# sp-uhh/sgmse

Measured on AMD Instinct MI355X. Metric: utterances/sec, SGMSE+ NCSN++ PC N=30 (reverse_diffusion + ALD, 60 NFE), 16 kHz 4 s utterances, higher is better.
Workload: dtype f32 (fp16x2-split products, fp32 accumulate); 1 GPU; BASELINE configs[1]: ncsnpp (65.6M params) PC sampler N=30, batch=32 x 4 s @16 kHz per GPU, hipGraph-captured step; batch_per_gpu=32, F=256, T=512, nfe=60, sampler=pc, parallelism=utterance-sharded x1 (weights broadcast once over RCCL)

## Files before the change

sgmse_amd/csrc/conv_launch.h:

```cpp
#pragma once
#include "conv_route.h"
#include "kernels_conv.h"
#include "kernels_conv_pipe.h"
#include "kernels_conv1x1.h"
#include "kernels_conv_split.h"
#include "kernels_conv_wino.h"
#include "kernels_conv_wino43.h"
#include "kernels_conv_wino2d.h"
#include "kernels_conv_thin.h"

#ifndef SGMSE_CONV_SPLIT_DEFAULT
#define SGMSE_CONV_SPLIT_DEFAULT 2
#endif
#ifndef SGMSE_CONV_PIPE_DEFAULT
#define SGMSE_CONV_PIPE_DEFAULT 1
#endif

namespace sgmse {

inline int conv_variant() {
  static int v = [] { const char* e = getenv("SGMSE_CONV_VARIANT"); return e ? atoi(e) : 0; }();
  return v;
}

inline int conv_grid_tiles(const ConvArgs& a, int rows) {
  const int ty = (a.H + rows - 1) / rows;
  return a.rag_cols ? ty * a.rag_ncols : a.B * ty * ((a.W + 31) / 32);
}

template <int KS, int WC, int FC, int FP>
inline void launch_conv_mfma_t(const ConvArgs& a, drt::stream_t st, int variant, int ksplit = 1) {
  using T = ConvTile<KS, WC, FC, FP>;
  const int tiles = conv_grid_tiles(a, T::ROWS);
  dim3 grid(tiles, (a.Cout + T::CO_T - 1) / T::CO_T, ksplit);
  if (variant < 0) variant = conv_variant();
  const bool vec = (a.rag_w ? a.rag_vec_ok != 0 : a.W % 4 == 0) && !(variant & 2) && (reinterpret_cast<uintptr_t>(a.src1) % 16 == 0) &&
                   (a.src2 == nullptr || reinterpret_cast<uintptr_t>(a.src2) % 16 == 0);
  const bool pref = !(variant & 1);
  if constexpr (FC * FP == 8) {
    const bool pipe = ((variant & 4) != 0) != (SGMSE_CONV_PIPE_DEFAULT != 0);
    if (vec && pipe) { DRT_LAUNCH((conv_mfma_pipe_kernel<KS, WC, FC, FP>), grid, dim3(256), st, a); return; }
  }
  if constexpr (KS == 1 && FC * FP == 8) {
    if (!vec) { launch_conv_mfma_t<KS, WC, FC, FP / 2>(a, st, variant, ksplit); return; }
    if (pref) DRT_LAUNCH((conv_mfma_kernel<KS, WC, FC, FP, 1, 1>), grid, dim3(256), st, a);
    else DRT_LAUNCH((conv_mfma_kernel<KS, WC, FC, FP, 0, 1>), grid, dim3(256), st, a);
  } else {
    if (vec && pref) DRT_LAUNCH((conv_mfma_kernel<KS, WC, FC, FP, 1, 1>), grid, dim3(256), st, a);
    else if (vec) DRT_LAUNCH((conv_mfma_kernel<KS, WC, FC, FP, 0, 1>), grid, dim3(256), st, a);
    else if (pref) DRT_LAUNCH((conv_mfma_kernel<KS, WC, FC, FP, 1, 0>), grid, dim3(256), st, a);
    else DRT_LAUNCH((conv_mfma_kernel<KS, WC, FC, FP, 0, 0>), grid, dim3(256), st, a);
  }
  if constexpr (FC * FP <= 2) {
    if (ksplit > 1) DRT_LAUNCH((conv_splitk_reduce_kernel<KS, WC, FC, FP>), dim3(grid.x, grid.y, 1), dim3(256), st, a, ksplit);
  }
}

inline void launch_conv_mfma(const ConvArgs& a, int ks, const ConvPlan& pl, drt::stream_t st, int variant = -1, int ksplit = 1) {
  const int v = variant < 0 ? conv_variant() : variant;
  if (ks == 1 && pl.co_t == 128 && (v & 8)) {
    const int kc = (v & 16) ? 64 : 32;
    const int Cin = a.C1 + a.C2;
    if (Cin % kc == 0 && (a.src2 == nullptr || a.C1 % kc == 0)) {
      const int tiles = conv_grid_tiles(a, 4);
      dim3 grid(tiles, a.Cout / 128, 1);
      if (kc == 64) DRT_LAUNCH((conv1x1_stream_kernel<1, 64>), grid, dim3(256), st, a);
      else DRT_LAUNCH((conv1x1_stream_kernel<1, 32>), grid, dim3(256), st, a);
      return;
    }
  }
#define SGMSE_CONV_CASE(KS_, CO_, ROWS_, WC_, FC_, FP_) \
  if (ks == KS_ && pl.co_t == CO_ && pl.rows == ROWS_) { launch_conv_mfma_t<KS_, WC_, FC_, FP_>(a, st, variant, ksplit); return; }
  SGMSE_CONV_CASE(3, 128, 8, 2, 2, 4)
  SGMSE_CONV_CASE(3, 64, 8, 2, 1, 4)
  SGMSE_CONV_CASE(3, 32, 8, 1, 1, 2)
  SGMSE_CONV_CASE(3, 128, 4, 2, 2, 2)
  SGMSE_CONV_CASE(3, 64, 4, 2, 1, 2)
  SGMSE_CONV_CASE(3, 32, 4, 1, 1, 1)
  SGMSE_CONV_CASE(1, 128, 8, 2, 2, 4)
  SGMSE_CONV_CASE(1, 64, 8, 2, 1, 4)
  SGMSE_CONV_CASE(1, 32, 8, 1, 1, 2)
  SGMSE_CONV_CASE(1, 128, 4, 2, 2, 2)
  SGMSE_CONV_CASE(1, 64, 4, 2, 1, 2)
  SGMSE_CONV_CASE(1, 32, 4, 1, 1, 1)
#undef SGMSE_CONV_CASE
}

static_assert(ConvThinGeom::KC == kConvThinKC, "conv_thin_eligible (conv_route.h) assumes the thin kernel's stage depth");

template <class S, int SHAPE>
inline void launch_conv3x3_split_t(const ConvArgs& a, dim3 grid, drt::stream_t st) {
  const bool act = a.in_scale && a.in_act;
  if constexpr (SHAPE != 1 && S::SCALED) {
    if (a.sc_w) {
      DRT_LAUNCH((conv3x3_split_kernel<S, SHAPE, 1, 0, 1>), grid, dim3(256), st, a);
      return;
    }
  }
  if (act) DRT_LAUNCH((conv3x3_split_kernel<S, SHAPE, 1>), grid, dim3(256), st, a);
  else DRT_LAUNCH((conv3x3_split_kernel<S, SHAPE, 0>), grid, dim3(256), st, a);
}
#ifndef SGMSE_CONV1X1_RAW_VEC
#define SGMSE_CONV1X1_RAW_VEC 1
#endif
template <class S>
inline void launch_conv1x1_split_t(const ConvArgs& a, dim3 grid, drt::stream_t st) {
  if (a.in_scale) { DRT_LAUNCH((conv1x1_split_kernel<S, 1, 0>), grid, dim3(256), st, a); return; }
  const bool vec = SGMSE_CONV1X1_RAW_VEC && (a.rag_w ? a.rag_vec_ok != 0 : a.W % 4 == 0) && reinterpret_cast<uintptr_t>(a.src1) % 16 == 0 &&
                   (a.src2 == nullptr || reinterpret_cast<uintptr_t>(a.src2) % 16 == 0);
  if (vec) DRT_LAUNCH((conv1x1_split_kernel<S, 0, 1>), grid, dim3(256), st, a);
  else DRT_LAUNCH((conv1x1_split_kernel<S, 0, 0>), grid, dim3(256), st, a);
}
inline void launch_conv_split(const ConvArgs& a, int ks, int mode, drt::stream_t st, bool rows4 = false, int abl = 0, int ksplit = 1) {
  const int tiles = conv_grid_tiles(a, 8);
  if (ks == 3 && a.Cout > 32 && rows4 && a.kchunk_stages > 0 && mode == 2) {
    const dim3 grid(conv_grid_tiles(a, 4), a.Cout / 128, ksplit);
    if (a.in_scale && a.in_act) DRT_LAUNCH((conv3x3_split_kernel<SplitH2, 2, 1, 0, 0, 1>), grid, dim3(256), st, a);
    else DRT_LAUNCH((conv3x3_split_kernel<SplitH2, 2, 0, 0, 0, 1>), grid, dim3(256), st, a);
    if (ksplit > 1) DRT_LAUNCH((conv_splitk_reduce_kernel<3, 4, 1, 4, true>), dim3(grid.x, grid.y, 1), dim3(256), st, a, ksplit);
    return;
  }
  if (ks == 3 && a.Cout > 32 && rows4) {
    const dim3 grid(conv_grid_tiles(a, 4), a.Cout / 128, 1);
    if (mode == 2) launch_conv3x3_split_t<SplitH2, 2>(a, grid, st); else launch_conv3x3_split_t<SplitB3, 2>(a, grid, st);
    return;
  }
  if (ks == 3 && a.Cout <= 32) {
    if (mode == 2) launch_conv3x3_split_t<SplitH2, 1>(a, dim3(tiles, 1, 1), st); else launch_conv3x3_split_t<SplitB3, 1>(a, dim3(tiles, 1, 1), st);
    return;
  }
  if (ks == 1) {
    if (mode == 2) launch_conv1x1_split_t<SplitH2>(a, dim3(tiles, a.Cout / 128, 1), st);
    else launch_conv1x1_split_t<SplitB3>(a, dim3(tiles, a.Cout / 128, 1), st);
    return;
  }
  const dim3 grid(tiles, a.Cout / 128, 1);
  if (abl && mode == 2) {
#define SGMSE_ABL_CASE(V) if (abl == V) { DRT_LAUNCH((conv3x3_split_kernel<SplitH2, 0, 1, V>), grid, dim3(256), st, a); return; }
#ifdef SGMSE_ABLATION_FULL
    SGMSE_ABL_CASE(8) SGMSE_ABL_CASE(59) SGMSE_ABL_CASE(64)
    SGMSE_ABL_CASE(3) SGMSE_ABL_CASE(4) SGMSE_ABL_CASE(24) SGMSE_ABL_CASE(56)
    SGMSE_ABL_CASE(1) SGMSE_ABL_CASE(2) SGMSE_ABL_CASE(67) SGMSE_ABL_CASE(72) SGMSE_ABL_CASE(128) SGMSE_ABL_CASE(256) SGMSE_ABL_CASE(512)
#endif
#undef SGMSE_ABL_CASE
  }
  if (mode == 2) launch_conv3x3_split_t<SplitH2, 0>(a, grid, st); else launch_conv3x3_split_t<SplitB3, 0>(a, grid, st);
}

inline bool conv_wino43_aligned(const ConvArgs& a) {
  return reinterpret_cast<uintptr_t>(a.src1) % 16 == 0 && (a.src2 == nullptr || reinterpret_cast<uintptr_t>(a.src2) % 16 == 0);
}
template <int ROWS>
inline void launch_conv_wino_rows(WinoForm form, const ConvArgs& a, drt::stream_t st) {
  const dim3 grid(conv_grid_tiles(a, ROWS), a.Cout / 128, 1);
  const bool act = a.in_scale && a.in_act;
  if (form == WinoForm::F43) {
    if (act) DRT_LAUNCH((conv3x3_wino43_kernel<ROWS, 1>), grid, dim3(512), st, a);
    else DRT_LAUNCH((conv3x3_wino43_kernel<ROWS, 0>), grid, dim3(512), st, a);
  } else {
    if (a.sc_w) DRT_LAUNCH((conv3x3_wino_kernel<ROWS, 1, 1>), grid, dim3(512), st, a);
    else if (act) DRT_LAUNCH((conv3x3_wino_kernel<ROWS, 1, 0>), grid, dim3(512), st, a);
    else DRT_LAUNCH((conv3x3_wino_kernel<ROWS, 0, 0>), grid, dim3(512), st, a);
  }
}
inline void launch_conv_wino(WinoForm form, const ConvArgs& a, drt::stream_t st, bool rows4, bool trace = false, int abl = 0) {
  if (form == WinoForm::F2x2) {
    const dim3 grid(conv_grid_tiles(a, 4), a.Cout / 128, 1);
    if (abl == 8) DRT_LAUNCH((conv3x3_wino2d_kernel<1, 8>), grid, dim3(512), st, a);
    else if (abl == 16) DRT_LAUNCH((conv3x3_wino2d_kernel<1, 16>), grid, dim3(512), st, a);
    else if (a.in_scale && a.in_act) DRT_LAUNCH((conv3x3_wino2d_kernel<1>), grid, dim3(512), st, a);
    else DRT_LAUNCH((conv3x3_wino2d_kernel<0>), grid, dim3(512), st, a);
    return;
  }
#ifdef SGMSE_ABLATION_FULL
  const dim3 grid8(conv_grid_tiles(a, 8), a.Cout / 128, 1);
  if (form == WinoForm::F43) {
    if (trace) { DRT_LAUNCH((conv3x3_wino43_kernel<8, 1, 1>), grid8, dim3(512), st, a); return; }
  } else {
#define SGMSE_WABL_CASE(V) if (abl == V) { DRT_LAUNCH((conv3x3_wino_kernel<8, 1, 0, 0, V>), grid8, dim3(512), st, a); return; }
    SGMSE_WABL_CASE(1) SGMSE_WABL_CASE(2) SGMSE_WABL_CASE(4) SGMSE_WABL_CASE(8) SGMSE_WABL_CASE(16) SGMSE_WABL_CASE(24) SGMSE_WABL_CASE(3) SGMSE_WABL_CASE(32) SGMSE_WABL_CASE(20)
#undef SGMSE_WABL_CASE
    if (trace) { DRT_LAUNCH((conv3x3_wino_kernel<8, 1, 0, 1>), grid8, dim3(512), st, a); return; }
  }
#endif
  (void)abl; (void)trace;
  if (rows4) launch_conv_wino_rows<4>(form, a, st); else launch_conv_wino_rows<8>(form, a, st);
}

inline void launch_conv_thin(const ConvArgs& a, drt::stream_t st) {
  const dim3 grid(conv_thin_grid_tiles(a, (a.W + ConvThinGeom::TW - 1) / ConvThinGeom::TW), 1, 1);
  if (a.in_scale && a.in_act) DRT_LAUNCH((conv3x3_thin_kernel<1>), grid, dim3(256), st, a);
  else DRT_LAUNCH((conv3x3_thin_kernel<0>), grid, dim3(256), st, a);
}

inline void launch_conv_direct(const ConvArgs& a, int ks, drt::stream_t st) {
  const int HW = a.H * a.W;
  if (a.Cout <= 4) {
    dim3 grid((HW + 255) / 256, 1, a.B);
    if (ks == 3) DRT_LAUNCH((conv_direct_kernel<3, 4>), grid, dim3(256), st, a);
    else DRT_LAUNCH((conv_direct_kernel<1, 4>), grid, dim3(256), st, a);
  } else {
    dim3 grid((HW + 255) / 256, (a.Cout + 15) / 16, a.B);
    if (ks == 3) DRT_LAUNCH((conv_direct_kernel<3, 16>), grid, dim3(256), st, a);
    else DRT_LAUNCH((conv_direct_kernel<1, 16>), grid, dim3(256), st, a);
  }
}

}
```

sgmse_amd/csrc/engine.h:

```cpp
#pragma once
#include <algorithm>
#include <map>
#include <string>
#include <vector>
#include <cstdio>
#include <stdexcept>

#include <deque>
#include <sgmse_devrt.h>
#include "dev_memory.h"
#include "kernels_conv.h"
#include "conv_launch.h"
#include "kernels_norm_fir.h"
#include "kernels_attn_misc.h"
#include "kernels_ode.h"
#include "ode_control.h"
#include "kernels_stft.h"
#include "../../include/sgmse_hip.h"

namespace sgmse {

struct NetCfg {
  int variant = 0;
  int nf = 128;
// ... 661 lines not shown
    frames_next_.insert(frames_next_.end(), total, total + n);
  }
  void take_noise_frames(const std::string& who, int B, int T, const float2* noise) {
    std::vector<int> g;
    g.swap(frames_next_);
    geom_call_.clear();
    if ((int)g.size() != 2 * B) return;
    std::string bad;
    if (noise) bad = who + ": a noise geometry (sgmse_set_noise_frames) applies to in-kernel noise, not to replayed noise";
    for (int b = 0; b < B && bad.empty(); ++b) {
      const int Tb = ragged() ? rag_T_[b] : T;
      const long long first = g[b], total = g[B + b];
      if (first < 0 || first + Tb > total)
        bad = who + ": utterance " + std::to_string(b) + ": noise frames [" + std::to_string(first) + ", " + std::to_string(first + Tb) +
              ") do not lie inside the recording's [0, " + std::to_string(total) + ")";
      geom_call_.insert(geom_call_.end(), {g[b], g[B + b], Tb});
    }
    if (!bad.empty()) { geom_call_.clear(); streams_next_.clear(); throw EngineArgError(bad); }
  }
  void set_ragged_frames(const int* frames, int n) { set_frames(frames, n); }
  int last_nfe() const { return nfe_; }
  int graph_captures() const { return graph_captures_; }
  int graph_updates() const { return graph_updates_; }
  int split_mode() const { return split_mode_; }
  bool winograd() const { return split_mode_ == 2 && wino_; }
  size_t arena_bytes() const { return arena_buf_.capacity(); }

  DevBuf input_bounds(const float* x1, int C1, const float* x2, int C2, int B, int HW) {
    const size_t per = (size_t)B * kAmaxSpread;
    DevBuf buf = fresh(2 * per * 4);
    float* out = buf.as<float>();
    SG_CHECK(drt::memset_dev(out, 0, 2 * per * 4, stream_));
    for (int b = 0; b < B; ++b) {
      const size_t n1 = (size_t)C1 * HW;
      DRT_LAUNCH(absmax_kernel, dim3((unsigned)std::min<size_t>((n1 + 255) / 256, 1024)), dim3(256), stream_, x1 + b * n1, n1,
                 out + (size_t)b * kAmaxSpread);
      if (x2) {
        const size_t n2 = (size_t)C2 * HW;
        DRT_LAUNCH(absmax_kernel, dim3((unsigned)std::min<size_t>((n2 + 255) / 256, 1024)), dim3(256), stream_, x2 + b * n2, n2,
                   out + per + (size_t)b * kAmaxSpread);
      }
    }
    return buf;
  }

  DevBuf producer_bound(const float* in_scale, const float* in_shift, int C, const float* amax1, const float* amax2, int B) {
    DevBuf buf = fresh((size_t)B * kAmaxSpread * 4);
    float* out = buf.as<float>();
    DRT_LAUNCH(xform_bound_kernel, dim3(B), dim3(64), stream_, in_scale, in_shift, C, amax1, amax2, out);
    return buf;
  }

  struct ConvPack { enum Kind { Mfma, Thin, Split, Wino } kind; int smode = 0; WinoForm form = WinoForm::F23; int co_t = 0; };
  struct StandaloneConv { ConvArgs a{}; DevBuf packed, bounds, xbound; };
  StandaloneConv standalone_conv(const ConvArgs& a0, const ConvPack& f, const float* w_oihw, int ks) {
    StandaloneConv s;
    ConvArgs& a = s.a = a0;
    const int Cin = a.C1 + a.C2;
    switch (f.kind) {
      case ConvPack::Mfma: s.packed = pack_mfma(oihw_sources(w_oihw, ks, Cin, a.Cout), f.co_t); break;
      case ConvPack::Thin: s.packed = pack_thin(w_oihw, Cin, a.Cout); break;
      case ConvPack::Split: s.packed = pack_split(w_oihw, ks, Cin, a.Cout, f.smode, &a.co_scale); break;
      case ConvPack::Wino: s.packed = pack_wino(f.form, w_oihw, Cin, a.Cout, &a.co_scale); break;
    }
    a.w = s.packed.as<float>();
    if (f.kind == ConvPack::Wino || (f.kind == ConvPack::Split && f.smode == 2)) {
      s.bounds = input_bounds(a.src1, a.C1, a.src2, a.C2, a.B, a.H * a.W);
      const float* am1 = s.bounds.as<float>();
      const float* am2 = a.src2 ? am1 + (size_t)a.B * kAmaxSpread : nullptr;
      if (ks == 1 && a.in_scale == nullptr) bind_bounds(a, 1, nullptr, am1, am2);
      else {
        s.xbound = producer_bound(a.in_scale, a.in_shift, Cin, am1, am2, a.B);
        bind_bounds(a, ks, s.xbound.as<float>(), s.xbound.as<float>(), nullptr);
      }
    }
    return s;
  }
  static void bind_bounds(ConvArgs& ca, int ks, const float* xbound, const float* amax1, const float* amax2) {
    if (ks == 3) ca.xbound = xbound;
    else { ca.amax1 = amax1; ca.amax2 = amax2; }
  }

  enum ForceConv { FC_AUTO = 0, FC_DIRECT = 1, FC_SPLIT_B3 = 2, FC_SPLIT_H2 = 3, FC_WINO = 4, FC_WINO_4ROW = 5, FC_THIN = 6, FC_WINO2D = 7,
                   FC_WINO43 = 8, FC_WINO43_4ROW = 9 };
  void op_conv2d(const float* x, const float* w_oihw, const float* bias, const float* res, float* out, int B, int Cin,
                 int Cout, int H, int W, int ks, float out_scale, int force_direct, const float* in_scale,
                 const float* in_shift, int in_act, const float* x2, int C2) {
    ConvArgs a{};
    a.src1 = x; a.src2 = x2; a.C1 = Cin - C2; a.C2 = C2; a.bias = bias; a.res = res; a.out_scale = out_scale; a.out = out;
    a.Cout = Cout; a.B = B; a.H = H; a.W = W; a.in_scale = in_scale; a.in_shift = in_shift; a.in_act = in_act;
    ConvPlan pl = choose_conv_plan(ks, Cin, Cout, H, W);
    const bool wino = force_direct == FC_WINO || force_direct == FC_WINO_4ROW || force_direct == FC_WINO2D || force_direct == FC_WINO43 || force_direct == FC_WINO43_4ROW;
    StandaloneConv s;
    if (force_direct == FC_THIN) {
      SG_REQUIRE(conv_thin_eligible(ks, a.C1, C2, Cout), "op_conv2d: shape is not eligible for the thin-output kernel");
      s = standalone_conv(a, ConvPack{ConvPack::Thin}, w_oihw, ks);
      launch_conv_thin(s.a, stream_);
      SG_CHECK(drt::stream_sync(stream_));
    } else if (wino || force_direct == FC_SPLIT_B3 || force_direct == FC_SPLIT_H2) {
      const WinoForm form = force_direct == FC_WINO2D ? WinoForm::F2x2 : force_direct >= FC_WINO43 ? WinoForm::F43 : WinoForm::F23;
      const int smode = wino ? 2 : force_direct - 1;
      if (!wino) SG_REQUIRE(conv_split_eligible(ks, a.C1, C2, Cout) || conv_thin_split_eligible(ks, a.C1, C2, Cout), "op_conv2d: shape is not eligible for the split kernels");
      else if (form == WinoForm::F43) SG_REQUIRE(ks == 3 && conv_wino43_eligible(a.C1, C2, Cout, W) && conv_wino43_aligned(a), "op_conv2d: shape is not eligible for the Winograd F(4,3) kernel");
      else SG_REQUIRE(ks == 3 && conv_wino_eligible(a.C1, C2, Cout, W), form == WinoForm::F2x2 ? "op_conv2d: shape is not eligible for the 2-D Winograd kernel" : "op_conv2d: shape is not eligible for the Winograd kernel");
      s = standalone_conv(a, wino ? ConvPack{ConvPack::Wino, smode, form} : ConvPack{ConvPack::Split, smode}, w_oihw, ks);
      if (wino) launch_conv_wino(form, s.a, stream_, force_direct == FC_WINO_4ROW || force_direct == FC_WINO43_4ROW);
      else launch_conv_split(s.a, ks, smode, stream_);
      SG_CHECK(drt::stream_sync(stream_));
    } else if (pl.mfma && !force_direct && (C2 == 0 || a.C1 % ((ks == 3) ? 8 : 32) == 0)) {
      s = standalone_conv(a, ConvPack{ConvPack::Mfma, 0, WinoForm::F23, pl.co_t}, w_oihw, ks);
      launch_conv_mfma(s.a, ks, pl, stream_);
      SG_CHECK(drt::stream_sync(stream_));
    } else {
      a.w = w_oihw;
      launch_conv_direct(a, ks, stream_);
    }
    check_launch();
  }

  void op_groupnorm(const float* x, const float* gamma, const float* beta, float* out, int B, int C, int H, int W, int act,
                    const float* x2, int C2) {
    const int HW = H * W, C1 = C - C2;
    const DevBuf stats_buf = fresh((size_t)B * C * 2 * 4), sc_buf = fresh((size_t)B * C * 4), sh_buf = fresh((size_t)B * C * 4);
    float *stats = stats_buf.as<float>(), *sc = sc_buf.as<float>(), *sh = sh_buf.as<float>();
    float* stats2 = stats + (size_t)B * C1 * 2;
    DRT_LAUNCH(gn_chan_stats_kernel, dim3(B * C1), dim3(256), stream_, x, (const float*)nullptr, C1, 0, HW, stats, Rag{nullptr, nullptr, nullptr}, 0);
    if (C2) DRT_LAUNCH(gn_chan_stats_kernel, dim3(B * C2), dim3(256), stream_, x2, (const float*)nullptr, C2, 0, HW, stats2, Rag{nullptr, nullptr, nullptr}, 0);
    const int G = std::min(C / 4, 32);
    const GnFin f{stats, stats2, nullptr, nullptr, gamma, beta, sc, sh, nullptr, Rag{nullptr, nullptr, nullptr}, C1, 1, 1, C2, 1, 1, G, HW, 0, 1e-6f};
    DRT_LAUNCH(gn_finalize_kernel, dim3(G, B), dim3(256), stream_, f);
    DRT_LAUNCH(gn_apply_kernel, dim3((HW + 1023) / 1024, B * C), dim3(256), stream_, x, x2, C1, C2, HW, (const float*)sc,
               (const float*)sh, act, out);
    SG_CHECK(drt::stream_sync(stream_));
    check_launch();
  }

  void op_fir(const float* x, float* out, int BC, int H, int W, int up, const float* in_scale, const float* in_shift, int in_act,
              float* out_raw) {
    FirArgs fa{x, out, in_scale, in_shift, in_act, BC, H, W, out_raw, 1, Rag{nullptr, nullptr, nullptr}};
    launch_fir(fa, up);
    check_launch();
  }

  void op_upfirdn2d(int dtype, const void* x, const void* kern, void* out, int BC, int H, int W, int kh, int kw, int up_x, int up_y,
                    int down_x, int down_y, int px0, int px1, int py0, int py1) {
    UpfirdnArgs a{x, kern, out, BC, H, W, kh, kw, up_x, up_y, down_x, down_y, px0, px1, py0, py1, 0, 0};
    a.Ho = (H * up_y + py0 + py1 - kh) / down_y + 1;
    a.Wo = (W * up_x + px0 + px1 - kw) / down_x + 1;
    SG_REQUIRE(a.Ho > 0 && a.Wo > 0, "upfirdn2d: empty output");
    const dim3 grid((a.Ho * a.Wo + 255) / 256, BC);
    if (dtype == 0) DRT_LAUNCH(upfirdn2d_generic_kernel<UpfirdnF32>, grid, dim3(256), stream_, a);
    else if (dtype == 1) DRT_LAUNCH(upfirdn2d_generic_kernel<UpfirdnF64>, grid, dim3(256), stream_, a);
    else DRT_LAUNCH(upfirdn2d_generic_kernel<UpfirdnF16>, grid, dim3(256), stream_, a);
    check_launch();
  }

  void op_attention(const float* qkv, float* out, int B, int C, int S) {
    AttnArgs a{qkv, out, B, C, S, 1.0f / sqrtf((float)C), Rag{nullptr, nullptr, nullptr}, 0};
    SG_REQUIRE(launch_attn_core(a, stream_), "attention: C must be one of " + attn_widths_text());
    check_launch();
  }

  void op_stft(const float* sig, const float* window, float2* spec, int B, int L, int n_fft, int hop) {
    SG_REQUIRE(n_fft <= kMaxNfft && n_fft >= 2 && hop >= 1 && L > n_fft / 2, "stft: unsupported geometry");
    const float2* tw = twiddle(n_fft);
    StftArgs a{sig, window, tw, spec, L, n_fft, hop, n_fft / 2 + 1, (L + 2 * (n_fft / 2) - n_fft) / hop + 1};
    DRT_LAUNCH(stft_kernel, dim3(a.K, B), dim3(256), stream_, a);
    check_launch();
  }

  void op_istft(const float2* spec, const float* window, float* out, int B, int K, int n_fft, int hop, int length) {
    SG_REQUIRE(n_fft <= kMaxNfft && n_fft >= 2 && hop >= 1, "istft: unsupported geometry");
    SG_REQUIRE(K >= 1 && length >= 1 && length + n_fft / 2 <= n_fft + hop * (K - 1), "istft: length exceeds the overlap-add span");
    const float2* tw = twiddle(n_fft);
    IstftArgs a{spec, window, tw, out, n_fft, hop, n_fft / 2 + 1, K, length};
    DRT_LAUNCH(istft_kernel, dim3((length + 255) / 256, B), dim3(256), stream_, a);
    check_launch();
  }

  void op_spec_xform(const float2* in, float2* out, size_t n, int type, float factor, float exponent, int inverse) {
    SpecXformArgs a{in, out, n, type, factor, exponent, inverse};
    DRT_LAUNCH(spec_xform_kernel, dim3((unsigned)((n + 255) / 256)), dim3(256), stream_, a);
    check_launch();
  }

  const int* upload_windows(const int* start, const int* frames, int n) {
    const size_t nb = (size_t)3 * n * sizeof(int);
    grow(win_tab_, nb);
    int* h = reinterpret_cast<int*>(stage_.acquire(nb));
    int col = 0;
    for (int j = 0; j < n; ++j) { h[j] = start[j]; h[n + j] = frames[j]; h[2 * n + j] = col; col += frames[j]; }
    SG_CHECK(drt::memcpy_h2d(win_tab_, h, nb, stream_));
    stage_.commit(stream_);
    return win_tab_.get();
  }

  void op_spec_split(const float2* spec, float2* windows, int F, int K, const int* start, const int* frames, int n, int type, float factor,
                     float exponent) {
    SG_REQUIRE(n <= 65535 && F <= 65535, "spec_split: more than 65535 windows or rows");
    SpecWinArgs a{spec, windows, upload_windows(start, frames, n), F, K, n, type, factor, exponent};
    const int tmax = *std::max_element(frames, frames + n);
    DRT_LAUNCH(spec_split_kernel, dim3((tmax + 255) / 256, F, n), dim3(256), stream_, a);
    check_launch();
  }

  void op_spec_merge(const float2* windows, float2* spec, int F, int K, const int* start, const int* frames, int n, int type, float factor,
                     float exponent) {
    SG_REQUIRE(F <= 65535, "spec_merge: more than 65535 rows");
    SpecWinArgs a{windows, spec, upload_windows(start, frames, n), F, K, n, type, factor, exponent};
    DRT_LAUNCH(spec_merge_kernel, dim3((K + 255) / 256, F), dim3(256), stream_, a);
    check_launch();
  }

  void sync() { SG_CHECK(drt::stream_sync(stream_)); }

  float bench_conv(int ks, int B, int Cin, int Cout, int H, int W, int variant, int iters, int fused) {
    ConvPlan pl = choose_conv_plan(ks, Cin, Cout, H, W);
    SG_REQUIRE(pl.mfma, "bench_conv: shape is not MFMA-eligible");
    if (variant >= 0 && (variant & 512)) { pl.rows = 4; variant &= ~512; }
    int ablate = 0, abl_split = 0;
    bool split_rows4 = false, wino43 = false;
    if (variant >= 0) {
      split_rows4 = (variant >> 23) & 1;
      wino43 = (variant >> 22) & 1;
      abl_split = (variant >> 12) & 1023;
      if (!(variant & (64 | 128))) { ablate = abl_split & 15; abl_split = 0; }
      variant &= 4095;
    }
    const bool wino = variant >= 0 && (variant & 1024);
    const bool wino2d = variant >= 0 && (variant & 2048) && !wino;
    const int smode = variant < 0 ? 0 : ((variant & 128) ? 2 : ((variant & 64) ? 1 : 0));
    const bool b3 = smode != 0 && !wino && !wino2d;
    SG_REQUIRE(!(wino || wino2d) || (ks == 3 && conv_wino_eligible(Cin, 0, Cout, W)), "bench_conv: shape is not eligible for the Winograd kernel");
    SG_REQUIRE(!b3 || conv_split_eligible(ks, Cin, 0, Cout), "bench_conv: shape is not eligible for the split kernels");
    wino43 = wino43 && wino;
    SG_REQUIRE(!wino43 || conv_wino43_eligible(Cin, 0, Cout, W), "bench_conv: shape is not eligible for the Winograd F(4,3) kernel");
    const WinoForm wform = wino2d ? WinoForm::F2x2 : wino43 ? WinoForm::F43 : WinoForm::F23;
    const size_t nx = (size_t)B * Cin * H * W, no = (size_t)B * Cout * H * W, nw = (size_t)Cout * Cin * ks * ks;
    const DevBuf x_buf = fresh(nx * 4), o_buf = fresh(no * 4), r_buf = fresh(no * 4), w_buf = fresh(nw * 4), sc_buf = fresh((size_t)B * Cin * 8);
    float *x = x_buf.as<float>(), *o = o_buf.as<float>(), *r = r_buf.as<float>(), *w = w_buf.as<float>(), *sc = sc_buf.as<float>();
    auto fill = [&](float* d, size_t n, uint32_t seed) {
      DRT_LAUNCH(fill_random_kernel, dim3((unsigned)((n + 255) / 256)), dim3(256), stream_, d, n, seed);
    };
    fill(x, nx, 1); fill(r, no, 2); fill(w, nw, 3); fill(sc, (size_t)B * Cin * 2, 4);
    ConvArgs a0{};
    a0.src1 = x; a0.C1 = Cin; a0.out = o; a0.Cout = Cout; a0.B = B; a0.H = H; a0.W = W; a0.out_scale = 1.f;
    a0.ablate = ablate;
    if (fused) { a0.in_scale = sc; a0.in_shift = sc + (size_t)B * Cin; a0.in_act = 1; a0.res = r; a0.bias = w; a0.out_scale = 0.70710678f; }
    if (b3 && smode == 2 && ks == 1) { a0.in_scale = nullptr; a0.in_shift = nullptr; a0.in_act = 0; }
    EventTimer timer;
    StandaloneConv s = standalone_conv(a0, b3 ? ConvPack{ConvPack::Split, smode} : (wino || wino2d) ? ConvPack{ConvPack::Wino, 2, wform}
                                                                               : ConvPack{ConvPack::Mfma, 0, WinoForm::F23, pl.co_t}, w, ks);
    ConvArgs& a = s.a;
    DevBuf trace_buf;
    unsigned long long* trace_dev = nullptr;
    const size_t n_wg = (size_t)B * ((H + 7) / 8) * ((W + 31) / 32) * ((Cout + 127) / 128);
    if (abl_split & 64) {
      trace_buf = fresh(n_wg * 256);
      trace_dev = trace_buf.as<unsigned long long>();
      SG_CHECK(drt::memset_dev(trace_dev, 0, n_wg * 256, stream_));
      a.trace = trace_dev;
    }
    auto go = [&]() {
      if (wino || wino2d) launch_conv_wino(wform, a, stream_, split_rows4, (abl_split & 64) != 0, abl_split & 63);
      else if (b3) launch_conv_split(a, ks, smode, stream_, split_rows4, abl_split);
      else launch_conv_mfma(a, ks, pl, stream_, variant);
    };
    for (int i = 0; i < 2; ++i) go();
    timer.start(stream_);
    for (int i = 0; i < iters; ++i) go();
    const float ms = timer.stop_ms(stream_) / (float)iters;
    check_launch();
    if (trace_dev) {
      const size_t words = wino ? 32 : 16;
      std::vector<unsigned long long> h(n_wg * words);
      SG_CHECK(drt::memcpy_d2h(h.data(), trace_dev, n_wg * words * 8, stream_));
      SG_CHECK(drt::stream_sync(stream_));
      if (const char* path = getenv("SGMSE_TRACE_OUT")) { if (FILE* f = fopen(path, "wb")) { fwrite(h.data(), 8, h.size(), f); fclose(f); } }
    }
    return ms;
  }

  float calib_stream(int mode, int bytes_per_lane, size_t total_bytes) {
    SG_REQUIRE((bytes_per_lane == 8 || bytes_per_lane == 16) && (mode == 0 || mode == 1) && total_bytes >= 4096, "calib_stream: bad arguments");
    const DevBuf scratch = fresh(total_bytes + 256);
    float* buf = scratch.as<float>();
    SG_CHECK(drt::memset_dev(buf, 0, total_bytes + 256, stream_));
    const size_t nvec = total_bytes / (size_t)bytes_per_lane;
    EventTimer timer;
    timer.start(stream_);
    const dim3 g(256 * 16), b(256);
    float* sink = buf + total_bytes / 4;
    if (bytes_per_lane == 8) { if (mode) DRT_LAUNCH((calib_stream_kernel<2, 1>), g, b, stream_, buf, nvec, sink); else DRT_LAUNCH((calib_stream_kernel<2, 0>), g, b, stream_, buf, nvec, sink); }
    else { if (mode) DRT_LAUNCH((calib_stream_kernel<4, 1>), g, b, stream_, buf, nvec, sink); else DRT_LAUNCH((calib_stream_kernel<4, 0>), g, b, stream_, buf, nvec, sink); }
    const float ms = timer.stop_ms(stream_);
    check_launch();
    return ms;
  }

  enum { TC_CONV3_BIG = 0, TC_CONV3, TC_CONV1, TC_DIRECT, TC_GN, TC_FIR, TC_ATTN, TC_MISC, TC_COUNT };
  void profile_forward(const float2* xy, const float* t_dev, float2* out, int B, int F, int T, float* ms_out, double* work_out,
                       int* launches_out) {
    prof_ = true;
    for (int i = 0; i < TC_COUNT; ++i) { prof_ms_[i] = 0.f; prof_flops_[i] = 0.0; prof_n_[i] = 0; }
    prof_used_ = 0;
    forward_xy(xy, t_dev, out, B, F, T);
    prof_ = false;
    SG_CHECK(drt::stream_sync(stream_));
    for (size_t i = 0; i < prof_used_; ++i) {
      ProfRec& r = prof_recs_[i];
      if (r.cls < 0) continue;
      const float ms = drt::event_elapsed_ms(*r.a.get(), *r.b.get());
      prof_ms_[r.cls] += ms;
      prof_flops_[r.cls] += r.work;
      prof_n_[r.cls] += r.launches;
      if (prof_dump_ && r.note[0]) fprintf(stderr, "[sgmse-prof] %s %.4f ms %.1f Gwork/s\n", r.note, ms, r.work / ms * 1e-6);
    }
    for (int i = 0; i < TC_COUNT; ++i) { ms_out[i] = prof_ms_[i]; work_out[i] = prof_flops_[i]; launches_out[i] = prof_n_[i]; }
  }

 private:
  bool grow(DevBuf& b, size_t bytes) { return b.ensure(bytes, stream_, poison_); }
  void renew(DevBuf& b, size_t bytes) { b.renew(bytes, stream_, poison_); }
  DevBuf fresh(size_t bytes) { DevBuf b; grow(b, bytes); return b; }
  template <class T = float> T* keep(DevBuf b) { wset_.push_back(std::move(b)); return wset_.back().as<T>(); }
  void release_weights() {
    if (wset_.empty()) return;
    drt::stream_sync(stream_);
    wset_.clear();
  }
// ... 333 lines not shown
    SG_REQUIRE(tmax == T, "ragged batch: T must be the largest frame count");
    rag_.clear();
    for (int l = 0; l < L; ++l) {
      const int H = F >> l;
      std::vector<int> w(B), cols(B + 1, 0);
      std::vector<long long> off(B + 1, 0), soff(B + 1, 0);
      for (int b = 0; b < B; ++b) {
        w[b] = rag_T_[b] >> l;
        off[b + 1] = off[b] + (long long)H * w[b];
        soff[b + 1] = soff[b] + (long long)H * ((w[b] + 31) / 32);
        cols[b + 1] = cols[b] + (w[b] + 31) / 32;
      }
      RagLevel r;
      r.pix = (size_t)off[B]; r.ncols = cols[B];
      grow(r.w, (size_t)B * 4); grow(r.off, (size_t)(B + 1) * 8); grow(r.soff, (size_t)(B + 1) * 8); grow(r.cols, (size_t)(B + 1) * 4);
      SG_CHECK(drt::memcpy_h2d(r.w, w.data(), (size_t)B * 4, stream_));
      SG_CHECK(drt::memcpy_h2d(r.off, off.data(), (size_t)(B + 1) * 8, stream_));
      SG_CHECK(drt::memcpy_h2d(r.soff, soff.data(), (size_t)(B + 1) * 8, stream_));
      SG_CHECK(drt::memcpy_h2d(r.cols, cols.data(), (size_t)(B + 1) * 4, stream_));
      SG_CHECK(drt::stream_sync(stream_));
      rag_.push_back(std::move(r));
    }
    rag_built_ = true;
  }
  std::vector<int> rag_T_;
  struct RagLevel { DevArray<int> w; DevArray<long long> off, soff; DevArray<int> cols; size_t pix = 0; int ncols = 0; };
  std::vector<RagLevel> rag_;
  bool rag_built_ = false;
  int cur_F_ = 0;
  void drop(Tensor& t) { arena_.release(t.p); t.p = nullptr; if (t.st) { arena_.release(t.st); t.st = nullptr; } }

  void gn_coeffs(const Tensor& a, const Tensor* b, const float* gamma, const float* beta, float** sc, float** sh,
                 const float** bound = nullptr) {
    const int C = a.C + (b ? b->C : 0), HW = a.H * a.W;
    float* bslot = bound ? next_amax() : nullptr;
    if (bound) *bound = bslot;
    const float* st[2] = {a.st, b ? b->st : nullptr};
    int nsub[2] = {a.nsub, b ? b->nsub : 0};
    int srows[2] = {a.srows, b ? b->srows : 1};
    float* tmp[2] = {nullptr, nullptr};
    const Tensor* src[2] = {&a, b};
    for (int k = 0; k < 2; ++k) {
      if (!src[k] || st[k]) continue;
      tmp[k] = arena_.alloc((size_t)B_ * src[k]->C * 2);
      st[k] = tmp[k]; nsub[k] = 1; srows[k] = 1;
      if (!dry_) {
        tock();
        DRT_LAUNCH(gn_chan_stats_kernel, dim3(B_ * src[k]->C), dim3(256), stream_, (const float*)src[k]->p, (const float*)nullptr,
                   src[k]->C, 0, HW, tmp[k], rag_of(a.H), a.H);
        if (noting()) snprintf(prof_note_, sizeof prof_note_, "gn_chan_stats C=%d @%dx%dx%d", src[k]->C, B_, a.H, a.W);
        tick(TC_GN, 4.0 * B_ * (double)src[k]->C * HW, 1);
      }
    }
    *sc = arena_.alloc((size_t)B_ * C);
    *sh = arena_.alloc((size_t)B_ * C);
    if (!dry_) {
      tock();
      const int G = std::min(C / 4, 32);
      const GnFin f{st[0], st[1], a.amax, b ? b->amax : nullptr, gamma, beta, *sc, *sh, bslot, rag_of(a.H),
                    a.C, nsub[0], srows[0], b ? b->C : 0, nsub[1], srows[1], G, HW, a.H, 1e-6f};
      DRT_LAUNCH(gn_finalize_kernel, dim3(G, B_), dim3(256), stream_, f);
      if (noting()) snprintf(prof_note_, sizeof prof_note_, "gn_finalize C=%d nsub=%d @%dx%dx%d", C, nsub[0], B_, a.H, a.W);
      tick(TC_GN, 8.0 * B_ * ((double)a.C * nsub[0] + (b ? (double)b->C * nsub[1] : 0.0)), 1);
    }
    for (int k = 0; k < 2; ++k) if (tmp[k]) arena_.release(tmp[k]);
  }

  struct Shortcut { const ConvW* w; const Tensor* a; const Tensor* b; };
  bool shortcut_foldable(const ConvW& c2, const Tensor& a, const Tensor* b) const {
    return fold_shortcut_ && c2.packed_split && c2.split_mode == 2 && c2.ks == 1 && conv_split_eligible(1, a.C, b ? b->C : 0, c2.cout) &&
           a.amax && (!b || b->amax);
  }

  ConvRoute route_of(const ConvW& w, int C1, int C2, int H, int W, const ConvCall& call) const {
    const ConvLayer layer{w.ks, C1, C2, w.cout, w.co_t, w.packed != nullptr, w.packed32 != nullptr, w.packed_thin != nullptr,
                          w.packed_split != nullptr, w.packed_wino != nullptr, w.split_mode, w.wino_form};
    const ConvKnobs knobs{tile_min_blocks_, split_min_tiles_, wino_min_tiles_, wino_, fuse_gn_stats_, chunk_max_tiles_, coarse_splitk_div_,
                          coarse_chunked_, coarse_split_};
    return conv_route(layer, ConvLevel{H, W, dec_W(H), level_of(H)}, call, B_, knobs);
  }

  Tensor conv(const ConvW& w, const Tensor& a, const Tensor* b, const Xform& xf, const float* bias, const float* bias2,
              const float* res, float out_scale, const FwdCtl& ctl, bool emit_stats = false, const Shortcut* sc = nullptr) {
    const int C2 = b ? b->C : 0, Cin = a.C + C2;
    SG_REQUIRE(Cin == w.cin, "conv: channel mismatch");
    Tensor o = new_tensor(w.cout, a.H, a.W);
    const ConvRoute rt = route_of(w, a.C, C2, a.H, a.W, ConvCall{xf.bound != nullptr, a.amax && (!b || b->amax), xf.scale != nullptr, emit_stats,
                                                                 bias2 != nullptr, sc != nullptr});
    const ConvFamily fam = rt.family;
    SG_REQUIRE(fam != ConvFamily::Wino23 || (a.W % 2 == 0 && rag_all_mult(a.H, 2)), "conv: odd width on a Winograd level");
    SG_REQUIRE(fam != ConvFamily::Wino43 || (a.W % 4 == 0 && rag_all_mult(a.H, 4)), "conv: width not a multiple of 4 on a Winograd F(4,3) level");
    SG_REQUIRE(!sc || (rt.accepts_shortcut && xf.act && !res), "conv: shortcut fold on an ineligible launch");
    float* partial = rt.ksplit > 1 ? arena_.alloc((size_t)rt.ksplit * w.cout * pix_total(a.H, a.W)) : nullptr;
    if (emit_stats && fuse_gn_stats_ && fam != ConvFamily::Direct) {
      o.srows = rt.srows;
      SG_REQUIRE(o.srows == 1 || !ragged() || a.H % 4 == 0, "ragged batch: 4-row statistics sub-tiles need H % 4 == 0");
      o.nsub = conv_plan_nsub(a.H, a.W, o.srows);
      o.st = arena_.alloc((size_t)B_ * w.cout * o.nsub * 2);
    } else if (emit_stats && fuse_gn_stats_) {
      o.nsub = 1;
      o.st = arena_.alloc((size_t)B_ * w.cout * 2);
    }
    o.amax = next_amax();
    if (dry_) { if (partial) arena_.release(partial); return o; }
    ConvArgs ca{};
    ca.xcd_map = conv_xcd_map_ ? 1 : 0;
    ca.stats_out = o.st; ca.stats_nsub = o.nsub; ca.stats_rows = o.srows;
    ca.amax_out = o.amax;
    ca.src1 = a.p; ca.src2 = b ? b->p : nullptr; ca.C1 = a.C; ca.C2 = C2;
    ca.bias = bias; ca.bias2 = bias2; ca.bias2_bstride = ctl.bias_bstride; ca.bias2_sstride = ctl.bias_sstride;
    ca.step_ptr = bias2 ? ctl.bias_step : nullptr;
    ca.in_scale = xf.scale; ca.in_shift = xf.shift; ca.in_act = xf.act;
    ca.res = res; ca.out_scale = out_scale; ca.out = o.p; ca.Cout = w.cout; ca.B = B_; ca.H = a.H; ca.W = a.W;
    ca.kchunk_stages = rt.kchunk; ca.partial = partial;
    if (ragged()) {
      const Rag rg = rag_of(a.H);
      ca.rag_w = rg.w; ca.rag_off = rg.off; ca.rag_soff = rg.soff; ca.rag_slab = (long long)w.cout * (long long)pix_total(a.H, a.W);
      ca.rag_vec_ok = rag_all_mult(a.H, 4) ? 1 : 0;
      if (rag_prefix_) { const RagLevel& r = rag_.at(level_of(a.H)); ca.rag_cols = r.cols; ca.rag_ncols = r.ncols; }
    }
    double fl = 2.0 * B_ * (double)w.cout * Cin * w.ks * w.ks * a.H * a.W;
    if (sc) {
      const int Cs = sc->a->C + (sc->b ? sc->b->C : 0);
      SG_REQUIRE(Cs == sc->w->cin && sc->w->cout == w.cout && sc->a->H == a.H && sc->a->W == a.W, "conv: shortcut shape mismatch");
      ca.sc_src1 = sc->a->p; ca.sc_src2 = sc->b ? sc->b->p : nullptr; ca.sc_C1 = sc->a->C; ca.sc_C2 = sc->b ? sc->b->C : 0;
      ca.sc_w = sc->w->packed_split; ca.sc_scale = sc->w->split_scale; ca.sc_bias = sc->w->bias;
      ca.sc_amax1 = sc->a->amax; ca.sc_amax2 = sc->b ? sc->b->amax : nullptr;
      fl += 2.0 * B_ * (double)w.cout * Cs * a.H * a.W;
    }
    tock();
    const char* gn = xf.scale ? " +gn" : "";
    const char* rs = res ? " +res" : "";
    const char* ex = ca.rag_cols ? " existing-tiles" : "";
    auto note_split = [&](const char* name) {
      if (!noting()) return;
      char scn[24] = "";
      if (sc) snprintf(scn, sizeof scn, " +shortcut(%d)", ca.sc_C1 + ca.sc_C2);
      snprintf(prof_note_, sizeof prof_note_, "conv3x3-%s %d->%d @%dx%dx%d%s%s%s%s", name, Cin, w.cout, B_, a.H, a.W, rs, gn, scn, ex);
    };
    int cls = w.ks == 3 ? (w.cout >= 128 ? TC_CONV3_BIG : TC_CONV3) : TC_CONV1;
    switch (fam) {
      case ConvFamily::Thin:
        ca.w = w.packed_thin; ca.stats_out = nullptr;
        launch_conv_thin(ca, stream_);
        if (noting()) snprintf(prof_note_, sizeof prof_note_, "conv3x3-thin %d->%d @%dx%dx%d%s%s", Cin, w.cout, B_, a.H, a.W, rs, gn);
        cls = TC_CONV3;
        break;
      case ConvFamily::Wino43:
        SG_REQUIRE(conv_wino43_aligned(ca), "conv: unaligned source on a Winograd F(4,3) level");
        [[fallthrough]];
      case ConvFamily::Wino23:
        ca.w = w.packed_wino; ca.co_scale = w.wino_scale;
        bind_bounds(ca, w.ks, xf.bound, a.amax, b ? b->amax : nullptr);
        launch_conv_wino(w.wino_form, ca, stream_, rt.rows4);
        note_split(fam == ConvFamily::Wino43 ? "wino43" : "wino");
        break;
      case ConvFamily::Split:
      case ConvFamily::SplitCoarse:
        ca.w = w.packed_split; ca.co_scale = w.split_scale;
        if (w.split_mode == 2) bind_bounds(ca, w.ks, xf.bound, a.amax, b ? b->amax : nullptr);
        launch_conv_split(ca, w.ks, w.split_mode, stream_, rt.rows4, 0, rt.ksplit);
        note_split("split");
        break;
      case ConvFamily::Mfma:
        ca.w = (rt.co_t == w.co_t) ? w.packed : w.packed32;
        launch_conv_mfma(ca, w.ks, ConvPlan{rt.co_t, rt.rows, true}, stream_, -1, rt.ksplit);
        if (noting())
          snprintf(prof_note_, sizeof prof_note_, "conv%dx%d %d->%d @%dx%dx%d tile %dco x %drows%s%s%s%s", w.ks, w.ks, Cin, w.cout, B_, a.H, a.W,
                   rt.co_t, rt.rows, rs, gn, rt.ksplit > 1 ? " split-K" : "", ex);
        cls = w.ks == 3 ? ((split_mode_ == 0 && rt.co_t == 128 && rt.rows == 8) ? TC_CONV3_BIG : TC_CONV3) : TC_CONV1;
        break;
      case ConvFamily::Direct:
        ca.w = w.oihw; ca.stats_out = nullptr;
        launch_conv_direct(ca, w.ks, stream_);
        if (noting()) snprintf(prof_note_, sizeof prof_note_, "conv-direct%dx%d %d->%d @%dx%dx%d", w.ks, w.ks, Cin, w.cout, B_, a.H, a.W);
        cls = TC_DIRECT;
        break;
    }
    tick(cls, fl);
    if (partial) arena_.release(partial);
    if (fam == ConvFamily::Direct && o.st) {
      tock();
      DRT_LAUNCH(gn_chan_stats_kernel, dim3(B_ * w.cout), dim3(256), stream_, (const float*)o.p, (const float*)nullptr, w.cout, 0,
                 a.H * a.W, o.st, rag_of(a.H), a.H);
      if (noting()) snprintf(prof_note_, sizeof prof_note_, "gn_chan_stats(direct) C=%d @%dx%dx%d", w.cout, B_, a.H, a.W);
      tick(TC_GN, 4.0 * B_ * (double)w.cout * a.H * a.W, 1);
    }
    return o;
  }

  void launch_fir(const FirArgs& fa, bool up, bool by_level = false) {
    const int H = fa.H, W = fa.W, BC = fa.BC;
// ... 99 lines not shown
    Tensor out = conv(w.proj, o, nullptr, Xform{}, w.proj.bias, nullptr, x.p, 0.70710678118654752440f, ctl, true);
    drop(o);
    return out;
  }

  bool side_enabled() const { return side_stream_on_ && B_ <= side_max_batch_; }
  bool side_active() const { return side_enabled() && !prof_ && !dry_ && !drt::is_emulator(); }
  drt::event_t* side_event() {
    if (side_ev_next_ == side_ev_.size()) side_ev_.emplace_back(Event::Order);
    return side_ev_[side_ev_next_++].get();
  }
  void side_begin() {
    SG_REQUIRE(!side_open_, "side stream: nested section");
    side_open_ = true;
    if (!side_enabled()) return;
    if (!side_pending_) arena_.defer_begin();
    if (!side_active()) return;
    if (!side_stream_ready_) { SG_CHECK(drt::stream_create(&side_stream_)); side_stream_ready_ = true; }
    drt::event_t* e = side_event();
    SG_CHECK(drt::event_record(e, stream_));
    SG_CHECK(drt::stream_wait_event(side_stream_, e));
    std::swap(stream_, side_stream_);
    side_swapped_ = true;
  }
  void side_end() {
    SG_REQUIRE(side_open_, "side stream: end without begin");
    side_open_ = false;
    if (!side_enabled()) return;
    side_pending_ = true;
    if (!side_swapped_) return;
    drt::event_t* e = side_event();
    SG_CHECK(drt::event_record(e, stream_));
    std::swap(stream_, side_stream_);
    side_swapped_ = false;
    side_join_ev_ = e;
  }
  void side_join() {
    if (!side_pending_) return;
    side_pending_ = false;
    if (side_join_ev_) { SG_CHECK(drt::stream_wait_event(stream_, side_join_ev_)); side_join_ev_ = nullptr; }
    arena_.defer_end();
  }
  drt::stream_t side_stream_{}; bool side_stream_ready_ = false, side_open_ = false, side_pending_ = false, side_swapped_ = false;
  std::deque<Event> side_ev_; size_t side_ev_next_ = 0; drt::event_t* side_join_ev_ = nullptr;
  bool side_stream_on_ = true; int side_max_batch_ = 8;

  void run_forward(const float2* x, long long xbs, const float2* y, long long ybs, float2* out, int B, int F, int T,
                   const FwdCtl& ctl_in) {
    side_ev_next_ = 0; side_open_ = side_pending_ = false; side_join_ev_ = nullptr;
    try { run_forward_main(x, xbs, y, ybs, out, B, F, T, ctl_in); }
    catch (...) {
      if (side_swapped_) { std::swap(stream_, side_stream_); side_swapped_ = false; }
      side_open_ = side_pending_ = false; side_join_ev_ = nullptr;
      arena_.reset();
      throw;
    }
  }
  void run_forward_main(const float2* x, long long xbs, const float2* y, long long ybs, float2* out, int B, int F, int T,
                        const FwdCtl& ctl_in) {
    FwdCtl ctl = ctl_in;
    ctl.bias_step = ctl.step_ptr;
    if (!dry_ && ctl.step_ptr && ctl.bias_table && ctl.bias_bstride == 0 && tot_temb_ > 0) {
      DRT_LAUNCH(bias_select_kernel, dim3((tot_temb_ + 255) / 256), dim3(256), stream_, ctl.bias_table, ctl.bias_sstride, ctl.step_ptr,
                 bias_cur_.get(), tot_temb_);
      ctl.bias_table = bias_cur_; ctl.bias_sstride = 0; ctl.bias_step = nullptr;
    }
    B_ = B;
    cur_F_ = F;
    amax_next_ = 0;
    lds_poison_count_ = 0;
    if (!dry_ && poison_ && arena_buf_.capacity()) SG_CHECK(drt::memset_dev(arena_buf_.as<char>(), 0xFF, arena_buf_.capacity(), stream_));
    if (!dry_ && amax_pool_) {
      const int n = amax_slots_ * B * kAmaxSpread;
      DRT_LAUNCH(zero_floats_kernel, dim3((n + 255) / 256), dim3(256), stream_, amax_pool_.get(), n);
    }
    const NetCfg& c = cfg_;
    const int L = c.n_levels;
    size_t mi = 3;
    auto next = [&]() -> const Mod& { SG_REQUIRE(mi < layout_.size(), "layout exhausted"); return layout_[mi++]; };
    const int FT = F * T;
    std::vector<Tensor> hs;
    Tensor xr = new_tensor(4, F, T);
    const bool entry8 = entry_mfma_ && entry8_.packed && layout_[mi].idx == entry8_idx_;
    Tensor xr8{};
    if (entry8) xr8 = new_tensor(entry8_.cin, F, T);
    if (!dry_) { tock(); const WrapCoef wc{ctl.coef, ctl.coef_bstride, ctl.coef_sstride, ctl.step_ptr, ctl.sign};
      DRT_LAUNCH(entry_kernel, dim3((FT + 255) / 256, B), dim3(256), stream_, x, xbs, y, ybs, xr.p, entry8 ? xr8.p : (float*)nullptr,
                 entry8 ? entry8_.cin : 0, FT, wc, rag_of(F), F, ctl.y_plane);
      tick(TC_MISC, (32.0 + (entry8 ? 4.0 * entry8_.cin : 0.0)) * B * FT); }
    {
      const Mod& m = next();
      const ConvW& w = entry8 ? entry8_ : conv_.at(m.idx);
      hs.push_back(conv(w, entry8 ? xr8 : xr, nullptr, Xform{}, w.bias, nullptr, nullptr, 1.f, ctl, true));
      if (entry8) drop(xr8);
    }
    Tensor pyr_in = xr;
    bool pyr_in_is_xr = true;
    for (int l = 0; l < L; ++l) {
      for (int rb = 0; rb < c.num_res_blocks; ++rb) {
        const Mod& m = next();
        Tensor h = res_block(m, hs.back(), nullptr, ctl);
        SG_REQUIRE(cfg_has_attn(c, h.H) == cfg_has_attn(c, c.image_size >> l),
                   "input height does not match the image_size the network was built for (attention placement, ncsnpp.py:308)");
        if (cfg_has_attn(c, h.H)) {
          const Mod& ma = next();
          Tensor h2 = attn_block(ma, h, ctl);
          drop(h);
          h = h2;
        }
        hs.push_back(h);
      }
      if (l != L - 1) {
        const Mod& m = next();
        Tensor h = res_block(m, hs.back(), nullptr, ctl);
        if (c.progressive_input == 1) {
          const Mod& mc = next();
          Tensor np = fir(pyr_in, false, Xform{});
          if (!pyr_in_is_xr) drop(pyr_in);
          pyr_in = np; pyr_in_is_xr = false;
          const ConvW& w = conv_.at(mc.idx);
          Tensor h2 = conv(w, pyr_in, nullptr, Xform{}, w.bias, nullptr, h.p, 1.f, ctl, true);
          drop(h);
          h = h2;
        }
        hs.push_back(h);
      }
    }
    if (!pyr_in_is_xr) drop(pyr_in);
    drop(xr);

    Tensor h = hs.back();
    {
      const Mod& m1 = next(); Tensor a = res_block(m1, h, nullptr, ctl);
      const Mod& m2 = next(); Tensor b2 = attn_block(m2, a, ctl); drop(a);
      const Mod& m3 = next(); h = res_block(m3, b2, nullptr, ctl); drop(b2);
    }
    Tensor pyramid; bool have_pyr = false;
    for (int l = L - 1; l >= 0; --l) {
      for (int rb = 0; rb < c.num_res_blocks + 1; ++rb) {
        const Mod& m = next();
        Tensor skip = hs.back(); hs.pop_back();
        Tensor o = res_block(m, h, &skip, ctl);
        drop(h); drop(skip);
        h = o;
      }
      SG_REQUIRE(cfg_has_attn(c, h.H) == cfg_has_attn(c, c.image_size >> l),
                 "input height does not match the image_size the network was built for (attention placement, ncsnpp.py:354)");
      if (cfg_has_attn(c, h.H)) {
        const Mod& ma = next();
        Tensor h2 = attn_block(ma, h, ctl);
        drop(h); h = h2;
      }
      if (c.progressive == 1) {
        const Mod& mg = next(); const Mod& mc = next();
        side_begin();
        float *sc, *sh;
        const float* bd;
        gn_coeffs(h, nullptr, gn_.at(mg.idx).first, gn_.at(mg.idx).second, &sc, &sh, &bd);
        const ConvW& w = conv_.at(mc.idx);
        Tensor up; bool have_up = false;
        if (have_pyr) { up = fir(pyramid, true, Xform{}); have_up = true; drop(pyramid); }
        pyramid = conv(w, h, nullptr, Xform{sc, sh, 1, bd}, w.bias, nullptr, have_up ? up.p : nullptr, 1.f, ctl);
        have_pyr = true;
        if (have_up) drop(up);
        arena_.release(sc); arena_.release(sh);
        side_end();
      }
      if (l != 0) {
        const Mod& m = next();
        Tensor o = res_block(m, h, nullptr, ctl);
        side_join();
        drop(h); h = o;
      }
    }
    side_join();
    SG_REQUIRE(hs.empty(), "skip stack not empty");
    Tensor h4;
// ... 12 lines not shown
    if (!dry_) {
      ExitArgs ea{h4.p, Wp("output_layer.weight"), Wp("output_layer.bias"), ctl.tvals, ctl.t_bstride, ctl.t_sstride, ctl.step_ptr,
                  c.variant == 1 ? 1 : 0, c.scale_by_sigma,
                  WrapCoef{ctl.coef, ctl.coef_bstride, ctl.coef_sstride, ctl.step_ptr, ctl.sign}, x, xbs, out, FT, rag_of(F), F};
      tock();
      DRT_LAUNCH(exit_kernel, dim3((FT + 255) / 256, B), dim3(256), stream_, ea);
      tick(TC_MISC, 24.0 * B * FT);
      check_launch();
    }
    drop(h4);
  }

  struct HostStage {
    PinnedArray<char> buf_; Event ev_; bool pending_ = false;
    char* acquire(size_t n) {
      if (pending_) { SG_CHECK(drt::event_sync(ev_.get())); pending_ = false; }
      buf_.ensure(std::max(n, size_t(1) << 16));
      return buf_;
    }
    void commit(drt::stream_t stream) {
      ev_.create();
      SG_CHECK(drt::event_record(ev_.get(), stream));
      pending_ = true;
    }
  } stage_;
  const unsigned long long* upload_tables(const std::vector<float>& tab, const std::vector<float>& tv, const std::vector<float>& cf,
                                          unsigned long long seed, int B) {
    SG_REQUIRE(B + 1 <= kMaxStreams, "batch too large for the noise-stream table");
    grow(seed_dev_, (size_t)kMaxStreams * (8 + 12) + 8);
    const size_t nb_geom = geom_call_.empty() ? 0 : ((size_t)3 * B * 4 + 7) / 8 * 8;
    const size_t nb_seed = ((size_t)B + 2) * 8 + nb_geom, nb_tab = tab.size() * 4, nb_tv = tv.size() * 4, nb_cf = cf.size() * 4;
    char* q = stage_.acquire(nb_seed + nb_tab + nb_tv + nb_cf);
    unsigned long long* hs = reinterpret_cast<unsigned long long*>(q);
    hs[0] = seed;
    const bool given = (int)streams_next_.size() == B;
    for (int b = 0; b < B; ++b) hs[1 + b] = given ? streams_next_[b] : (unsigned long long)b;
    streams_next_.clear();
    hs[1 + B] = nb_geom ? 1ull : 0ull;
    if (nb_geom) { hs[1 + B + nb_geom / 8] = 0; memcpy(hs + 2 + B, geom_call_.data(), (size_t)3 * B * 4); }
    geom_call_.clear();
    q += nb_seed;
    memcpy(q, tab.data(), nb_tab); memcpy(q + nb_tab, tv.data(), nb_tv);
    if (nb_cf) memcpy(q + nb_tab + nb_tv, cf.data(), nb_cf);
    SG_CHECK(drt::memcpy_h2d(seed_dev_, hs, nb_seed, stream_));
    SG_CHECK(drt::memcpy_h2d(step_table_, q, nb_tab, stream_));
    SG_CHECK(drt::memcpy_h2d(tsteps_, q + nb_tab, nb_tv, stream_));
    if (nb_cf) SG_CHECK(drt::memcpy_h2d(coef_table_, q + nb_tab + nb_tv, nb_cf, stream_));
    stage_.commit(stream_);
    return seed_dev_.get();
  }
  static constexpr int kMaxStreams = 4096;
  std::vector<unsigned long long> streams_next_;
  std::vector<int> frames_next_;
  std::vector<int> geom_call_;
  DevArray<unsigned long long> seed_dev_;
  DevArray<int> win_tab_;
  int graph_captures_ = 0;

  int device_;
  drt::stream_t stream_;
  NetCfg cfg_;
  std::vector<Mod> layout_;
  std::map<std::string, const float*> W_;
  std::map<int, ResW> res_;
  std::map<int, AttnW> attn_;
  std::map<int, ConvW> conv_;
  std::map<int, std::pair<const float*, const float*>> gn_;
  DenseDesc* dense_descs_ = nullptr; int n_dense_ = 0; int tot_temb_ = 0;
  bool weights_ready_ = false;
  std::vector<DevBuf> wset_;
  std::map<int, DevArray<float2>> twiddles_;

  Arena arena_; DevBuf arena_buf_;
  bool dry_ = false;
  void read_knobs() {
    auto flag = [](const char* name, bool dflt) { const char* e = getenv(name); return e ? e[0] == '1' : dflt; };
    const char* e = getenv("SGMSE_CONV_SPLIT");
    split_mode_ = e ? atoi(e) : SGMSE_CONV_SPLIT_DEFAULT;
    SG_REQUIRE(split_mode_ >= 0 && split_mode_ <= 2, "SGMSE_CONV_SPLIT must be 0, 1 or 2");
    wino_ = flag("SGMSE_WINO", true);
    wino43_ = flag("SGMSE_WINO43", true);
    rag_prefix_ = flag("SGMSE_RAGGED_PREFIX", true);
    conv_xcd_map_ = flag("SGMSE_CONV_XCD_MAP", true);
    debug_sync_ = flag("SGMSE_DEBUG_SYNC", false);
    prof_dump_ = flag("SGMSE_PROFILE_DUMP", false);
    e = getenv("SGMSE_TILE_MIN_BLOCKS");
    tile_min_blocks_ = e ? atol(e) : 512L;
    e = getenv("SGMSE_SPLIT_MIN_TILES");
    split_min_tiles_ = e ? atol(e) : 8L;
    e = getenv("SGMSE_WINO_MIN_TILES");
    wino_min_tiles_ = e ? atol(e) : 32L;
    fuse_gn_stats_ = flag("SGMSE_FUSE_GN_STATS", true);
    lds_poison_ = flag("SGMSE_POISON_LDS", false);
    e = getenv("SGMSE_POISON_LDS_AT");
    lds_poison_at_ = e ? atoi(e) : -1;
    lds_poison_upto_ = flag("SGMSE_POISON_LDS_UPTO", false);
    side_stream_on_ = flag("SGMSE_SIDE_STREAM", true);
    e = getenv("SGMSE_SIDE_MAX_BATCH");
    side_max_batch_ = e ? atoi(e) : 8;
    e = getenv("SGMSE_NOFOLD_LEVELS");
    nofold_levels_ = e ? atoi(e) : 0;
    poison_ = flag("SGMSE_POISON", false);
  }
  DevArray<float> amax_pool_; int amax_slots_ = 0, amax_next_ = 0;
  float* next_amax() {
    const int i = amax_next_++;
    if (dry_) return reinterpret_cast<float*>(uintptr_t(1) << 43) + (size_t)i * kAmaxSpread;
    SG_REQUIRE(amax_pool_ && i < amax_slots_, "range-bound pool smaller than the forward needs");
    return amax_pool_ + (size_t)i * B_ * kAmaxSpread;
  }
  long tile_min_blocks_ = 512, split_min_tiles_ = 8;
  static constexpr bool coarse_chunked_ = true, fold_shortcut_ = true, coarse_split_ = true, entry_mfma_ = true;
  ConvW entry8_{}; int entry8_idx_ = -1;
  bool poison_ = false, debug_sync_ = false, conv_xcd_map_ = true, rag_prefix_ = true, wino_ = true, wino43_ = true;
  long wino_min_tiles_ = 32;
  int nofold_levels_ = 0;
  bool lds_poison_ = false, lds_poison_upto_ = false; int lds_poison_at_ = -1, lds_poison_count_ = 0; DevArray<unsigned> lds_sink_;
  static constexpr long coarse_splitk_div_ = 4, chunk_max_tiles_ = 8;
  int split_mode_ = SGMSE_CONV_SPLIT_DEFAULT;
  bool prof_dump_ = false;
  char prof_note_[160] = {0};
  static constexpr bool fir_scalar_ = false;
  bool fuse_gn_stats_ = true;
  int B_ = 0, shape_B_ = 0, shape_F_ = 0, shape_T_ = 0;
  DevArray<float2> sx_, sxm_, sscore_, sy_;
  DevArray<int> step_ctr_;
  DevArray<float> lang_partial_, lang_scal_;
  DevArray<float> bias_cur_, temb_act_, bias_table_, step_table_, tsteps_, coef_table_; int temb_rows_ = 0;
  drt::graph_t graph_{}; bool graph_valid_ = false; GraphKey graph_key_{};
  int nfe_ = 0;
  DevArray<float2> ode_k_[7], ode_xs_;
  static constexpr int kOdeEachMaxB = 1024;
  DevArray<double> ode_table_, ode_partial_, ode_result_; PinnedArray<double> ode_host_;
  std::vector<OdeControl> ode_ctl_; int ode_rounds_ = 0, ode_wasted_ = 0;
  bool prof_ = false; std::vector<ProfRec> prof_recs_; size_t prof_used_ = 0; float prof_ms_[TC_COUNT]; double prof_flops_[TC_COUNT]; int prof_n_[TC_COUNT];
};

}
```

sgmse_amd/csrc/kernels_attn_misc.h:

```cpp
#pragma once
#include <string>
#include <sgmse_devrt.h>
#include "kernels_conv.h"
#include "kernels_norm_fir.h"

namespace sgmse {

struct AttnArgs { const float* qkv; float* out; int B, C, S; float scale; Rag rag; int H; };

template <int CF>
__global__ __launch_bounds__(256, 2) void attn_core_kernel(AttnArgs p) {
  constexpr int C = CF * 32;
  constexpr int FH = CF < 2 ? CF : 2;
  constexpr int NH = CF / FH;
  constexpr int VS = 33;
  __shared__ float s_q[C * 32];
  __shared__ float s_v[4][FH * 32 * VS];
  __shared__ float s_m[4][32];
  __shared__ float s_l[4][32];
  __shared__ float s_lt[32];
  const int tid = threadIdx.x, wave = tid >> 6, lane = tid & 63, l31 = lane & 31, kh = lane >> 5;
  const int b = blockIdx.y, s0 = blockIdx.x * 32;
  const int S = p.rag.w ? p.H * p.rag.w[b] : p.S;
  if (s0 >= S) return;
// ... 146 lines not shown
  return false;
}

inline std::string attn_widths_text() {
  std::string s;
#define SGMSE_ATTN_TXT(CF) s += (s.empty() ? "" : ", ") + std::to_string((CF) * 32);
  SGMSE_ATTN_WIDTHS(SGMSE_ATTN_TXT)
#undef SGMSE_ATTN_TXT
  return s;
}

inline bool launch_attn_core(const AttnArgs& a, drt::stream_t st) {
  dim3 grid((a.S + 31) / 32, a.B, 1);
  switch (a.C) {
#define SGMSE_ATTN_CASE(CF) case (CF) * 32: DRT_LAUNCH((attn_core_kernel<CF>), grid, dim3(256), st, a); return true;
    SGMSE_ATTN_WIDTHS(SGMSE_ATTN_CASE)
#undef SGMSE_ATTN_CASE
    default: return false;
  }
}

struct TembArgs {
  const float* t; int nt;
  const float* Wf; const float* w1; const float* b1; const float* w2; const float* b2;
  int nf;
  float* act_out;
};

__global__ __launch_bounds__(256) void temb_mlp_kernel(TembArgs p) {
  __shared__ float s_emb[512];
  __shared__ float s_h[1024];
  const int row = blockIdx.x, nf = p.nf, ne = 2 * nf, nh = 4 * nf;
  const float logt = (float)log((double)p.t[row]);
  for (int i = threadIdx.x; i < nf; i += 256) {
    float pr = logt * p.Wf[i];
    pr = pr * 2.0f;
    pr = pr * 3.14159265358979323846f;
    s_emb[i] = (float)sin((double)pr);
    s_emb[nf + i] = (float)cos((double)pr);
  }
  __syncthreads();
  for (int o = threadIdx.x; o < nh; o += 256) {
    float acc = 0.f;
    const float* wr = p.w1 + (size_t)o * ne;
    for (int i = 0; i < ne; ++i) acc = fmaf(wr[i], s_emb[i], acc);
    s_h[o] = silu_precise_f(acc + p.b1[o]);
  }
  __syncthreads();
  for (int o = threadIdx.x; o < nh; o += 256) {
    float acc = 0.f;
    const float* wr = p.w2 + (size_t)o * nh;
    for (int i = 0; i < nh; ++i) acc = fmaf(wr[i], s_h[i], acc);
    p.act_out[(size_t)row * nh + o] = silu_precise_f(acc + p.b2[o]);
  }
}

struct DenseDesc { const float* W; const float* b; const float* cb; int cout; int off; };

__global__ __launch_bounds__(256) void temb_dense_kernel(const DenseDesc* descs, const float* act, int nh, float* table,
                                                         int row_stride) {
  __shared__ float s_a[1024];
  const DenseDesc d = descs[blockIdx.x];
  const int row = blockIdx.y;
  for (int i = threadIdx.x; i < nh; i += 256) s_a[i] = act[(size_t)row * nh + i];
  __syncthreads();
  for (int co = threadIdx.x; co < d.cout; co += 256) {
    float acc = 0.f;
    const float* wr = d.W + (size_t)co * nh;
    for (int i = 0; i < nh; ++i) acc = fmaf(wr[i], s_a[i], acc);
    table[(size_t)row * row_stride + d.off + co] = acc + d.b[co] + d.cb[co];
  }
}

struct WrapCoef { const float* coef; int bstride, sstride; const int* step_ptr; float sign; };

__device__ __forceinline__ void wrap_coef(const WrapCoef& w, int b, float* gamma, float* alpha, float* beta) {
  if (!w.coef) { *gamma = 1.f; *alpha = 0.f; *beta = w.sign; return; }
  const int step = w.step_ptr ? *w.step_ptr : 0;
  const float* r = w.coef + ((size_t)step * w.sstride + (size_t)b * w.bstride) * 4;
  *gamma = r[0]; *alpha = r[1]; *beta = r[2];
}

__global__ __launch_bounds__(256) void entry_kernel(const float2* x, long long xbs, const float2* y, long long ybs,
                                                    float* xr, float* xr8, int C8, int FT, WrapCoef w, Rag rag, int F, int y_plane) {
  const int i = blockIdx.x * 256 + threadIdx.x;
  const int b = blockIdx.y;
  size_t xo = (size_t)b * xbs, yo = (size_t)b * ybs, po = (size_t)b * FT;
  if (rag.w) {
    FT = F * rag.w[b];
    xo = (size_t)rag.off[b] * xbs; yo = (size_t)rag.off[b] * ybs + (size_t)y_plane * FT; po = (size_t)rag.off[b];
  }
  if (i >= FT) return;
  float g, al, be;
  wrap_coef(w, b, &g, &al, &be);
  const float2 xv = x[xo + i], yv = y[yo + i];
  float* o = xr + po * 4 + i;
  const float v0 = g * xv.x, v1 = g * xv.y, v2 = g * yv.x, v3 = g * yv.y;
  o[0] = v0; o[FT] = v1; o[2 * (size_t)FT] = v2; o[3 * (size_t)FT] = v3;
  if (xr8) {
    float* q = xr8 + po * C8 + i;
    q[0] = v0; q[FT] = v1; q[2 * (size_t)FT] = v2; q[3 * (size_t)FT] = v3;
    for (int k = 4; k < C8; ++k) q[(size_t)k * FT] = 0.f;
  }
}

struct ExitArgs {
  const float* h4; const float* ow; const float* ob;
  const float* tvals; int t_bstride, t_sstride; const int* step_ptr;
  int conv_first, scale_by_t;
  WrapCoef w; const float2* xt; long long xt_bs;
  float2* out; int FT;
  Rag rag; int F;
};

__global__ __launch_bounds__(256) void exit_kernel(ExitArgs p) {
  const int i = blockIdx.x * 256 + threadIdx.x;
  const int b = blockIdx.y;
  int FT = p.FT;
  size_t po = (size_t)b * FT, xo = (size_t)b * p.xt_bs;
  if (p.rag.w) { FT = p.F * p.rag.w[b]; po = (size_t)p.rag.off[b]; xo = po * p.xt_bs; }
  if (i >= FT) return;
  const int step = p.step_ptr ? *p.step_ptr : 0;
  const float t = p.scale_by_t ? p.tvals[(size_t)step * p.t_sstride + (size_t)b * p.t_bstride] : 1.f;
  const float* h = p.h4 + po * 4 + i;
  float hv[4];
#pragma unroll
  for (int c = 0; c < 4; ++c) hv[c] = h[(size_t)c * FT];
  if (p.scale_by_t && !p.conv_first) {
#pragma unroll
    for (int c = 0; c < 4; ++c) hv[c] = hv[c] / t;
  }
  float o[2];
#pragma unroll
  for (int k = 0; k < 2; ++k) {
    float acc = 0.f;
#pragma unroll
    for (int c = 0; c < 4; ++c) acc = fmaf(p.ow[k * 4 + c], hv[c], acc);
    o[k] = acc + p.ob[k];
  }
  if (p.scale_by_t && p.conv_first) { o[0] = o[0] / t; o[1] = o[1] / t; }
  float g, al, be;
  wrap_coef(p.w, b, &g, &al, &be);
  float2 r = make_float2(be * o[0], be * o[1]);
  if (al != 0.f) { const float2 xv = p.xt[xo + i]; r.x += al * xv.x; r.y += al * xv.y; }
  p.out[po + i] = r;
}

enum { SC_T = 0, SC_DT = 1, SC_ALD_EPS = 2, SC_ALD_NOISE = 3, SC_G = 4, SC_G2 = 5, SC_STRIDE = 8 };

__device__ __forceinline__ void philox_round(uint32_t& c0, uint32_t& c1, uint32_t& c2, uint32_t& c3, uint32_t k0, uint32_t k1) {
  const uint64_t p0 = (uint64_t)0xD2511F53u * c0, p1 = (uint64_t)0xCD9E8D57u * c2;
  const uint32_t n0 = (uint32_t)(p1 >> 32) ^ c1 ^ k0, n1 = (uint32_t)p1;
  const uint32_t n2 = (uint32_t)(p0 >> 32) ^ c3 ^ k1, n3 = (uint32_t)p0;
  c0 = n0; c1 = n1; c2 = n2; c3 = n3;
}

__device__ __forceinline__ float2 philox_cnormal(unsigned long long seed, unsigned long long idx, uint32_t draw, unsigned long long stream64 = 0) {
  const uint32_t stream = (uint32_t)stream64, shi = (uint32_t)(stream64 >> 32);
  uint32_t c0 = (uint32_t)idx, c1 = (uint32_t)(idx >> 32) ^ (stream * 0x9E3779B9u), c2 = draw, c3 = 0x5367534du ^ stream;
  uint32_t k0 = (uint32_t)seed ^ (shi * 0x85EBCA6Bu), k1 = (uint32_t)(seed >> 32) ^ shi;
#pragma unroll
  for (int r = 0; r < 10; ++r) { philox_round(c0, c1, c2, c3, k0, k1); k0 += 0x9E3779B9u; k1 += 0xBB67AE85u; }
  const float u1 = ((float)(c0 >> 8) + 0.5f) * (1.0f / 16777216.0f);
  const float u2 = ((float)(c1 >> 8) + 0.5f) * (1.0f / 16777216.0f);
  const float rad = sqrtf(-logf(u1));
  float sn, cs;
  sincosf(6.283185307179586f * u2, &sn, &cs);
  return make_float2(rad * cs, rad * sn);
}

struct SamplerArgs {
  float2* x; float2* x_mean; const float2* y; const float2* score;
  const float2* noise;
  const unsigned long long* seed;
  const float* table; const int* step_ptr;
  int draw_base, draw_per_step;
  float theta, score_w;
  int add_noise;
  float std1;
  int n;
  float snr; int B; int per;
  float* partial;
  float* lang;
  const long long* rag_off;
};

// ... 186 lines not shown
```

sgmse_amd/csrc/kernels_conv.h:

```cpp
#pragma once
#include <sgmse_devrt.h>
#include <type_traits>

namespace sgmse {

struct Rag { const int* w; const long long* off; const long long* soff; };

struct ConvArgs {
  const float* src1; const float* src2;
  int C1, C2;
  const float* w;
  const float* bias;
  const float* bias2;
  int bias2_bstride, bias2_sstride;
  const int* step_ptr;
  const float* in_scale; const float* in_shift;
  int in_act;
  const float* res;
  const float* acc_scale;
  const float* co_scale;
  float out_scale;
  float* out;
  int Cout, B, H, W;
  float* stats_out;
  int stats_nsub;
  int stats_rows;
  float* amax_out;
  const float* amax1; const float* amax2;
  const float* xbound;
  int ablate;
  const float* sc_src1; const float* sc_src2; int sc_C1, sc_C2;
  const float* sc_w; const float* sc_scale; const float* sc_bias; const float* sc_amax1; const float* sc_amax2;
  int kchunk_stages;
  float* partial;
  const int* rag_w; const long long* rag_off; const long long* rag_soff; long long rag_slab;
  int rag_vec_ok;
  unsigned long long* trace;
  int xcd_map;
  const int* rag_cols; int rag_ncols;
};
__device__ __forceinline__ int conv_xcd_tile(int t, int nt, int on) { return (on && (nt & 7) == 0) ? (t & 7) * (nt >> 3) + (t >> 3) : t; }
__device__ __forceinline__ void conv_tile_of(const ConvArgs& p, int t, int nt, int tiles_xg, int tiles_y, int& b, int& ty, int& tx) {
  int bid = conv_xcd_tile(t, nt, p.xcd_map);
  if (p.rag_cols) {
    int lo = 0, hi = p.B;
    while (hi - lo > 1) { const int mid = (lo + hi) >> 1; if (p.rag_cols[mid] * tiles_y <= bid) lo = mid; else hi = mid; }
    const int c0 = p.rag_cols[lo], nx = p.rag_cols[lo + 1] - c0, r = bid - c0 * tiles_y;
    b = lo; ty = r / nx; tx = r - ty * nx;
  } else {
    tx = bid % tiles_xg; bid /= tiles_xg;
    ty = bid % tiles_y;
    b = bid / tiles_y;
  }
}

#ifndef SGMSE_SPLITK_FRAGMENT_MAJOR
#define SGMSE_SPLITK_FRAGMENT_MAJOR 1
#endif
constexpr int kAmaxSpread = 64;

__device__ __forceinline__ bool conv_ragged_adjust(ConvArgs& p, int b, int tx) {
  const int Wb = p.rag_w[b];
  if (tx * 32 >= Wb) return false;
  const long long d = p.rag_off[b] - (long long)b * p.H * Wb;
  p.W = Wb;
  p.src1 += d * p.C1;
  if (p.src2) p.src2 += d * p.C2;
  p.out += d * p.Cout;
  if (p.res) p.res += d * p.Cout;
  if (p.sc_src1) p.sc_src1 += d * p.sc_C1;
  if (p.sc_src2) p.sc_src2 += d * p.sc_C2;
  if (p.partial) p.partial += d * p.Cout;
  if (p.stats_out) {
    const int rps = p.stats_rows == 4 ? 4 : 1;
    const int nsub = (p.H / rps) * ((Wb + 31) >> 5);
    p.stats_out += (p.rag_soff[b] / rps - (long long)b * nsub) * p.Cout * 2;
    p.stats_nsub = nsub;
  }
  return true;
}
__device__ __forceinline__ size_t conv_partial_slab(const ConvArgs& p, int H, int W) {
  return p.rag_w ? (size_t)p.rag_slab : (size_t)p.B * p.Cout * H * W;
}

__device__ __forceinline__ float amax_read(const float* amax, int b) {
  float m = amax[b * kAmaxSpread + (threadIdx.x & (kAmaxSpread - 1))];
#pragma unroll
  for (int o = 32; o >= 1; o >>= 1) m = fmaxf(m, __shfl_xor(m, o));
  return m;
}

__device__ __forceinline__ float h2_weight_scale(float absmax) {
  if (!(absmax > 0.f)) return 1.f;
  const int e = (int)((__builtin_bit_cast(uint32_t, absmax) >> 23) & 0xff) - 127;
  int k = 13 - e;
  k = k > 100 ? 100 : (k < -100 ? -100 : k);
  return __builtin_bit_cast(float, (uint32_t)(k + 127) << 23);
}

struct GnFin {
  const float* st1; const float* st2; const float* amax1; const float* amax2;
  const float* gamma; const float* beta; float* scale; float* shift; float* bound_out;
  Rag rag;
  int C1, nsub1, rps1, C2, nsub2, rps2, G, HW, H;
  float eps;
};

__device__ __forceinline__ void gn_sum_pairs(const float* base, int n, int slot, double& s, double& q) {
  if ((reinterpret_cast<uintptr_t>(base) & 15) == 0 && (n & 1) == 0) {
    const float4* b4 = reinterpret_cast<const float4*>(base);
#pragma unroll 4
    for (int i = slot; i < n / 2; i += 256) {
      const float4 v = b4[i];
      s += (double)v.x + (double)v.z; q += (double)v.y + (double)v.w;
    }
  } else {
    for (int i = slot; i < n; i += 256) { s += (double)base[2 * i]; q += (double)base[2 * i + 1]; }
  }
}

struct GnGroupSpan { const float* p1; int n1; const float* p2; int n2; int HW; };
__device__ __forceinline__ GnGroupSpan gn_group_span(const GnFin& f, int b, int g) {
  const int cpg = (f.C1 + f.C2) / f.G;
  const int c_lo = g * cpg, c_hi = c_lo + cpg;
  int nsub1 = f.nsub1, nsub2 = f.nsub2, HW = f.HW;
  size_t sb1 = (size_t)b * nsub1, sb2 = (size_t)b * nsub2;
  if (f.rag.w) {
    const int w = f.rag.w[b], ns = f.H * ((w + 31) >> 5);
    HW = f.H * w;
    if (nsub1 > 1) { nsub1 = ns / f.rps1; sb1 = (size_t)(f.rag.soff[b] / f.rps1); }
    if (nsub2 > 1) { nsub2 = ns / f.rps2; sb2 = (size_t)(f.rag.soff[b] / f.rps2); }
  }
  GnGroupSpan sp{nullptr, 0, nullptr, 0, HW};
  const int a_hi = c_hi < f.C1 ? c_hi : f.C1;
  if (c_lo < a_hi) { sp.p1 = f.st1 + (sb1 * f.C1 + (size_t)c_lo * nsub1) * 2; sp.n1 = (a_hi - c_lo) * nsub1; }
  const int b_lo = c_lo > f.C1 ? c_lo : f.C1;
  if (b_lo < c_hi) { sp.p2 = f.st2 + (sb2 * f.C2 + (size_t)(b_lo - f.C1) * nsub2) * 2; sp.n2 = (c_hi - b_lo) * nsub2; }
  return sp;
}

__device__ __forceinline__ void gn_group_coeffs(const GnFin& f, int b, int g, int lane, double s_tot, double q_tot, int HW) {
  const int C = f.C1 + f.C2, cpg = C / f.G, c_lo = g * cpg;
  float am = -1.f;
  if (f.bound_out && f.amax1 && (f.C2 == 0 || f.amax2)) {
    am = amax_read(f.amax1, b);
    if (f.C2) am = fmaxf(am, amax_read(f.amax2, b));
  }
  float bnd = 0.f;
  if (lane < cpg) {
// ... 242 lines not shown
    for (int i = 0; i < FC; ++i)
#pragma unroll
      for (int j = 0; j < FP; ++j) {
        const int y = ty * ROWS + wp * FP + j;
        unsigned off[16];
#pragma unroll
        for (int r = 0; r < 16; ++r) {
          const int co = co_blk * CO_T + (wc * FC + i) * 32 + 4 * kh + (r & 3) + 8 * (r >> 2);
          const bool ok = co < p.Cout && y < H && x < W;
          off[r] = ok ? (unsigned)((((size_t)b * p.Cout + co) * H + y) * W + x) : 0u;
        }
        f32x16 v[8];
#pragma unroll
        for (int z = 0; z < 8; ++z) {
          const float* pz = p.partial + (size_t)(z < nchunks ? z : 0) * slab;
#pragma unroll
          for (int r = 0; r < 16; ++r) v[z][r] = pz[off[r]];
        }
        __builtin_amdgcn_sched_barrier(0);
#pragma unroll
        for (int r = 0; r < 16; ++r) acc[i][j][r] = v[0][r];
#pragma unroll
        for (int z = 1; z < 8; ++z) {
          if (z < nchunks) {
#pragma unroll
            for (int r = 0; r < 16; ++r) acc[i][j][r] = acc[i][j][r] + v[z][r];
          }
        }
        __builtin_amdgcn_sched_barrier(0);
      }
  } else
  for (int z = 0; z < nchunks; ++z) {
    const float* pz = p.partial + (size_t)z * slab;
    f32x16 v[FC][FP];
#pragma unroll
    for (int i = 0; i < FC; ++i)
#pragma unroll
      for (int j = 0; j < FP; ++j) {
        const int y = ty * ROWS + wp * FP + j;
#pragma unroll
        for (int r = 0; r < 16; ++r) {
          const int co = co_blk * CO_T + (wc * FC + i) * 32 + 4 * kh + (r & 3) + 8 * (r >> 2);
          const bool ok = co < p.Cout && y < H && x < W;
          v[i][j][r] = pz[ok ? ((size_t)(b * p.Cout + co) * H + y) * W + x : 0];
        }
      }
    __builtin_amdgcn_sched_barrier(0);
#pragma unroll
    for (int i = 0; i < FC; ++i)
#pragma unroll
      for (int j = 0; j < FP; ++j)
#pragma unroll
        for (int r = 0; r < 16; ++r) acc[i][j][r] = z == 0 ? v[i][j][r] : acc[i][j][r] + v[i][j][r];
    __builtin_amdgcn_sched_barrier(0);
  }
#pragma unroll
  for (int i = 0; i < FC; ++i)
#pragma unroll
    for (int j = 0; j < FP; ++j) {
      const int y = ty * ROWS + wp * FP + j;
#pragma unroll
      for (int r = 0; r < 16; ++r) {
        const int co = co_blk * CO_T + (wc * FC + i) * 32 + 4 * kh + (r & 3) + 8 * (r >> 2);
        if (!(co < p.Cout && y < H && x < W)) acc[i][j][r] = 0.f;
      }
    }
}

template <int KS, int WC, int FC, int FP, int PREF, int VEC>
__global__ __launch_bounds__(256, 2) void conv_mfma_kernel(ConvArgs p) {
  using T = ConvTile<KS, WC, FC, FP, VEC>;
  constexpr int CO_T = T::CO_T, ROWS = T::ROWS, KC = T::KC, HALO = T::HALO, RS = T::RS, PLANE = T::PLANE,
                TAPS = T::TAPS, NI = VEC ? 1 : T::NI, NW4 = T::NW4, NV = VEC ? T::NV : 1, TROWS = T::TROWS;
  __shared__ float s_in[T::IN_ELEMS];
  __shared__ float s_w[T::W_ELEMS];
  __shared__ float s_sc[512];
  __shared__ float s_sh[512];

  const int tid = threadIdx.x;
  const int Cin = p.C1 + p.C2;
  const int tiles_xg = (p.W + 31) >> 5;
  const int tiles_y = (p.H + ROWS - 1) / ROWS;
  int b, ty, tx;
  conv_tile_of(p, (int)blockIdx.x, (int)gridDim.x, tiles_xg, tiles_y, b, ty, tx);
  if (p.rag_w) { if (!conv_ragged_adjust(p, b, tx)) return; }
  const int tiles_x = (p.W + 31) >> 5;
  const int x0 = tx * 32, y0 = ty * ROWS;
  const int co_blk = blockIdx.y;
  const int H = p.H, W = p.W;
  const bool xform = p.in_scale != nullptr;

  for (int c = tid; c < Cin; c += 256) {
    s_sc[c] = xform ? p.in_scale[b * Cin + c] : 1.f;
    s_sh[c] = xform ? p.in_shift[b * Cin + c] : 0.f;
  }
  const bool act = xform && p.in_act;

  const int wave = tid >> 6, lane = tid & 63, l31 = lane & 31, kh = lane >> 5;
  const int wc = wave % WC, wp = wave / WC;
  const int a_off = kh * TAPS * CO_T + wc * FC * 32 + l31;
  const int b_off = kh * PLANE + (wp * FP) * RS + l31 + T::XOFF;

  f32x16 acc[FC][FP];
#pragma unroll
  for (int i = 0; i < FC; ++i)
#pragma unroll
    for (int j = 0; j < FP; ++j)
#pragma unroll
      for (int r = 0; r < 16; ++r) acc[i][j][r] = 0.f;

  float rin[NI];
  f32x4 rv[NV];
  f32x4 rw[NW4];
  unsigned okmask = 0;
  int goff[NI];
  int goff_v[NV];
  int loff_v[NV];
  int loff_h = 0;

  const float* wbase = p.w + (size_t)co_blk * Cin * TAPS * CO_T;
  const size_t HW = (size_t)H * W;

  if constexpr (!VEC) {
#pragma unroll
    for (int i = 0; i < NI; ++i) {
      int e = tid + 256 * i;
      e = e < T::IN_ELEMS ? e : T::IN_ELEMS - 1;
      const int c = e / PLANE;
      const int rem = e - c * PLANE;
      const int r = rem / RS;
      const int x = rem - r * RS;
      const int gy = y0 - HALO + r, gx = x0 - HALO + x;
      const bool ok = gy >= 0 && gy < H && gx >= 0 && gx < W;
      okmask |= (ok ? 1u : 0u) << i;
      goff[i] = ok ? gy * W + gx : 0;
    }
  } else {
#pragma unroll
    for (int i = 0; i < NV; ++i) {
      int it = tid + 256 * i;
      it = it < T::NVI ? it : T::NVI - 1;
      const int c = it / (TROWS * 8);
      const int rem = it - c * (TROWS * 8);
      const int r = rem >> 3, q = rem & 7;
      const int gy = y0 - HALO + r, gx = x0 + 4 * q;
      const bool ok = gy >= 0 && gy < H && gx < W;
      okmask |= (ok ? 1u : 0u) << i;
      goff_v[i] = ok ? gy * W + gx : 0;
      loff_v[i] = c * PLANE + r * RS + (HALO ? 4 : 0) + 4 * q;
    }
    if (HALO) {
      const int it = tid < T::NHI ? tid : T::NHI - 1;
      const int c = it / (TROWS * 2);
      const int rem = it - c * (TROWS * 2);
      const int r = rem >> 1, side = rem & 1;
      const int gy = y0 - HALO + r, gx = side ? x0 + 32 : x0 - 1;
      const bool ok = gy >= 0 && gy < H && gx >= 0 && gx < W;
      okmask |= (ok ? 1u : 0u) << 31;
      goff[0] = ok ? gy * W + gx : 0;
      loff_h = c * PLANE + r * RS + (side ? 36 : 3);
    }
  }

  auto plane_of = [&](int cg) -> const float* {
    return (cg < p.C1) ? p.src1 + (size_t)(b * p.C1 + cg) * HW : p.src2 + (size_t)(b * p.C2 + (cg - p.C1)) * HW;
  };

  auto load_stage = [&](int c0) {
    if constexpr (!VEC) {
#pragma unroll
      for (int i = 0; i < NI; ++i) {
        int e = tid + 256 * i;
        e = e < T::IN_ELEMS ? e : T::IN_ELEMS - 1;
        rin[i] = plane_of(c0 + e / PLANE)[goff[i]];
      }
    } else {
#pragma unroll
      for (int i = 0; i < NV; ++i) {
        int it = tid + 256 * i;
        it = it < T::NVI ? it : T::NVI - 1;
        rv[i] = *reinterpret_cast<const f32x4*>(plane_of(c0 + it / (TROWS * 8)) + goff_v[i]);
      }
      if (HALO) {
        const int it = tid < T::NHI ? tid : T::NHI - 1;
        rin[0] = plane_of(c0 + it / (TROWS * 2))[goff[0]];
      }
    }
    const f32x4* wsrc = reinterpret_cast<const f32x4*>(wbase + (size_t)c0 * TAPS * CO_T);
#pragma unroll
    for (int i = 0; i < NW4; ++i) {
      int idx = tid + 256 * i;
      idx = idx < T::W_ELEMS / 4 ? idx : T::W_ELEMS / 4 - 1;
      rw[i] = wsrc[idx];
    }
  };

  auto xf1 = [&](float v, float sc, float sh, bool ok) -> float {
    v = v * sc + sh;
    const float sv = silu_f(v);
    v = act ? sv : v;
    return ok ? v : 0.f;
  };

  auto store_stage = [&](int c0) {
    if constexpr (!VEC) {
#pragma unroll
      for (int i = 0; i < NI; ++i) {
        int e = tid + 256 * i;
        e = e < T::IN_ELEMS ? e : T::IN_ELEMS - 1;
        const int cg = c0 + e / PLANE;
        s_in[e] = xf1(rin[i], s_sc[cg], s_sh[cg], (okmask >> i) & 1u);
      }
    } else {
#pragma unroll
      for (int i = 0; i < NV; ++i) {
        int it = tid + 256 * i;
        it = it < T::NVI ? it : T::NVI - 1;
        const int cg = c0 + it / (TROWS * 8);
        const float sc = s_sc[cg], sh = s_sh[cg];
        const bool ok = (okmask >> i) & 1u;
        f32x4 o;
        o[0] = xf1(rv[i][0], sc, sh, ok); o[1] = xf1(rv[i][1], sc, sh, ok);
        o[2] = xf1(rv[i][2], sc, sh, ok); o[3] = xf1(rv[i][3], sc, sh, ok);
        *reinterpret_cast<f32x4*>(s_in + loff_v[i]) = o;
      }
      if (HALO) {
        const int it = tid < T::NHI ? tid : T::NHI - 1;
        const int cg = c0 + it / (TROWS * 2);
        s_in[loff_h] = xf1(rin[0], s_sc[cg], s_sh[cg], (okmask >> 31) & 1u);
      }
    }
    f32x4* wdst = reinterpret_cast<f32x4*>(s_w);
#pragma unroll
    for (int i = 0; i < NW4; ++i) {
      int idx = tid + 256 * i;
      idx = idx < T::W_ELEMS / 4 ? idx : T::W_ELEMS / 4 - 1;
      wdst[idx] = rw[i];
    }
  };

  auto compute = [&]() {
    const float* sw = s_w + a_off;
    const float* si = s_in + b_off;
    if constexpr (PREF) {
      constexpr int NS = (KC / 2) * TAPS;
      float a[2][FC], bb[2][FP];
      auto ld = [&](int s2, int slot) {
        const int cp = s2 / TAPS, tap = s2 % TAPS, dy = tap / KS, dx = tap % KS;
// ... 22 lines not shown
#pragma unroll 1
      for (int cp = 0; cp < KC / 2; ++cp) {
#pragma unroll
        for (int tap = 0; tap < TAPS; ++tap) {
          const int dy = tap / KS, dx = tap % KS;
          float a[FC], bb[FP];
#pragma unroll
          for (int i = 0; i < FC; ++i) a[i] = sw[i * 32 + (cp * 2 * TAPS + tap) * CO_T];
#pragma unroll
          for (int j = 0; j < FP; ++j) bb[j] = si[j * RS + cp * 2 * PLANE + dy * RS + dx];
#pragma unroll
          for (int i = 0; i < FC; ++i)
#pragma unroll
            for (int j = 0; j < FP; ++j)
              acc[i][j] = __builtin_amdgcn_mfma_f32_32x32x2f32(a[i], bb[j], acc[i][j], 0, 0, 0);
        }
      }
    }
  };

  const int nstages = Cin / KC;
  const bool abl_stage = p.ablate & 4, abl_bar = p.ablate & 8;
  if constexpr (FC * FP <= 2) {
    const int cs = p.kchunk_stages > 0 ? p.kchunk_stages : nstages;
    const bool splitk = gridDim.z > 1;
    const int ci0 = splitk ? (int)blockIdx.z * cs : 0;
    const int ci1 = splitk ? (ci0 + cs < nstages ? ci0 + cs : nstages) : nstages;
    f32x16 tot[FC][FP];
    bool first = true;
    load_stage(ci0 * KC);
    __syncthreads();
    for (int ci = ci0; ci < ci1; ++ci) {
      store_stage(ci * KC);
      __syncthreads();
      if (ci + 1 < ci1) load_stage((ci + 1) * KC);
      compute();
      __syncthreads();
      if (p.kchunk_stages > 0 && !splitk && ((ci + 1) % cs == 0 || ci + 1 == ci1)) {
#pragma unroll
        for (int i = 0; i < FC; ++i)
#pragma unroll
          for (int j = 0; j < FP; ++j)
#pragma unroll
            for (int r = 0; r < 16; ++r) { tot[i][j][r] = first ? acc[i][j][r] : tot[i][j][r] + acc[i][j][r]; acc[i][j][r] = 0.f; }
        first = false;
      }
    }
    if (p.kchunk_stages > 0 && !splitk) {
#pragma unroll
      for (int i = 0; i < FC; ++i)
#pragma unroll
        for (int j = 0; j < FP; ++j) acc[i][j] = tot[i][j];
    }
    if (splitk) {
      ConvArgs q = p;
      q.out = p.partial + (size_t)blockIdx.z * conv_partial_slab(p, H, W);
      q.bias = nullptr; q.bias2 = nullptr; q.res = nullptr; q.acc_scale = nullptr; q.out_scale = 1.f; q.stats_out = nullptr; q.amax_out = nullptr;
      conv_epilogue<T, FC, FP, WC>(q, acc, b, co_blk, tx, ty, tiles_x, wc, wp, l31, kh);
      return;
    }
  } else {
    load_stage(0);
    __syncthreads();
    for (int ci = 0; ci < nstages; ++ci) {
      if (!abl_stage || ci == 0) store_stage(ci * KC);
      if (!abl_bar) __syncthreads();
      if (ci + 1 < nstages && !abl_stage) load_stage((ci + 1) * KC);
      compute();
      if (!abl_bar) __syncthreads();
    }
  }

  conv_epilogue<T, FC, FP, WC>(p, acc, b, co_blk, tx, ty, tiles_x, wc, wp, l31, kh);
}

template <int KS, int WC, int FC, int FP, bool STAT4 = false>
__global__ __launch_bounds__(256) void conv_splitk_reduce_kernel(ConvArgs p, int nchunks) {
  using T = ConvTile<KS, WC, FC, FP, 1>;
  constexpr int ROWS = T::ROWS, CO_T = T::CO_T;
  const int tid = threadIdx.x;
  const int tiles_xg = (p.W + 31) >> 5;
  const int tiles_y = (p.H + ROWS - 1) / ROWS;
  int b, ty, tx;
  conv_tile_of(p, (int)blockIdx.x, (int)gridDim.x, tiles_xg, tiles_y, b, ty, tx);
  if (p.rag_w) { if (!conv_ragged_adjust(p, b, tx)) return; }
  const int H = p.H, W = p.W;
  const int tiles_x = (W + 31) >> 5;
  const int co_blk = blockIdx.y;
  const int wave = tid >> 6, lane = tid & 63, l31 = lane & 31, kh = lane >> 5;
  const int wc = wave % WC, wp = wave / WC;
  f32x16 acc[FC][FP];
  conv_splitk_sum<T, FC, FP, WC>(p, nchunks, b, co_blk, tx, ty, wc, wp, l31, kh, acc);
  float as_mul = 1.0f;
  if (p.xbound) as_mul = 1.0f / h2_weight_scale(amax_read(p.xbound, b));
  conv_epilogue<T, FC, FP, WC, 0, false, STAT4, STAT4>(p, acc, b, co_blk, tx, ty, tiles_x, wc, wp, l31, kh, as_mul);
}

template <int KS, int CG>
__global__ __launch_bounds__(256) void conv_direct_kernel(ConvArgs p) {
  constexpr int TAPS = KS * KS, HALO = KS / 2;
  const int b = blockIdx.z;
  if (p.rag_w) conv_ragged_adjust(p, b, 0);
  const int H = p.H, W = p.W, HW = H * W;
  const int pix = blockIdx.x * 256 + threadIdx.x;
  const int co0 = blockIdx.y * CG;
  const int Cin = p.C1 + p.C2;
  const bool inb = pix < HW;
  const int y = inb ? pix / W : 0, x = inb ? pix - (pix / W) * W : 0;
  float acc[CG];
#pragma unroll
  for (int g = 0; g < CG; ++g) acc[g] = 0.f;
  const bool xform = p.in_scale != nullptr;
  constexpr int CB = 4;
  int offs[TAPS];
  bool oks[TAPS];
#pragma unroll
  for (int t = 0; t < TAPS; ++t) {
    const int gy = y + t / KS - HALO, gx = x + t % KS - HALO;
    oks[t] = inb && gy >= 0 && gy < H && gx >= 0 && gx < W;
    const int gyc = gy < 0 ? 0 : (gy >= H ? H - 1 : gy), gxc = gx < 0 ? 0 : (gx >= W ? W - 1 : gx);
    offs[t] = gyc * W + gxc;
  }
  for (int c0 = 0; c0 < Cin; c0 += CB) {
    float v[CB][TAPS];
#pragma unroll
    for (int cc = 0; cc < CB; ++cc) {
      const int c = c0 + cc < Cin ? c0 + cc : Cin - 1;
      const float* plane = (c < p.C1) ? p.src1 + (size_t)(b * p.C1 + c) * HW : p.src2 + (size_t)(b * p.C2 + (c - p.C1)) * HW;
#pragma unroll
      for (int t = 0; t < TAPS; ++t) v[cc][t] = plane[offs[t]];
    }
    __builtin_amdgcn_sched_barrier(0);
#pragma unroll
    for (int cc = 0; cc < CB; ++cc) {
      const int c = c0 + cc;
      if (c < Cin) {
        if (xform) {
          const float sc = p.in_scale[b * Cin + c], sh = p.in_shift[b * Cin + c];
#pragma unroll
          for (int t = 0; t < TAPS; ++t) { float u = v[cc][t] * sc + sh; if (p.in_act) u = silu_f(u); v[cc][t] = u; }
        }
#pragma unroll
        for (int t = 0; t < TAPS; ++t) v[cc][t] = oks[t] ? v[cc][t] : 0.f;
#pragma unroll
        for (int g = 0; g < CG; ++g) {
          const int co = co0 + g;
          if (co < p.Cout) {
            const float* wr = p.w + ((size_t)co * Cin + c) * TAPS;
#pragma unroll
            for (int t = 0; t < TAPS; ++t) acc[g] = fmaf(wr[t], v[cc][t], acc[g]);
          }
        }
      }
    }
  }
  const float* b2 = nullptr;
  if (p.bias2) {
    const int step = p.step_ptr ? *p.step_ptr : 0;
    b2 = p.bias2 + (size_t)step * p.bias2_sstride + (size_t)b * p.bias2_bstride;
  }
  float vmax = 0.f;
  float rr[CG];
  if (p.res) {
#pragma unroll
    for (int g = 0; g < CG; ++g) {
      const int co = co0 + g < p.Cout ? co0 + g : p.Cout - 1;
      rr[g] = p.res[(size_t)(b * p.Cout + co) * HW + (inb ? pix : 0)];
    }
  } else {
#pragma unroll
    for (int g = 0; g < CG; ++g) rr[g] = 0.f;
// ... 49 lines not shown
```

sgmse_amd/csrc/kernels_conv1x1.h:

```cpp
#pragma once
#include "kernels_conv.h"

namespace sgmse {

template <int FP, int KC>
__global__ __launch_bounds__(256, 2) void conv1x1_stream_kernel(ConvArgs p) {
  constexpr int FC = 4, NSTEP = KC / 2, CO_T = 128;
  using T = ConvTile<1, 1, FC, FP, 1>;
  static_assert(T::CO_T == CO_T && T::ROWS == 4 * FP, "tile");
  __shared__ float s_w0[KC * CO_T];
  __shared__ float s_w1[KC * CO_T];
  __shared__ float s_sc[512];
  __shared__ float s_sh[512];

  const int tid = threadIdx.x;
  const int Cin = p.C1 + p.C2;
  const int tiles_xg = (p.W + 31) >> 5;
  const int tiles_y = (p.H + T::ROWS - 1) / T::ROWS;
  int b, ty, tx;
  conv_tile_of(p, (int)blockIdx.x, (int)gridDim.x, tiles_xg, tiles_y, b, ty, tx);
  if (p.rag_w) { if (!conv_ragged_adjust(p, b, tx)) return; }
  const int H = p.H, W = p.W;
  const int tiles_x = (W + 31) >> 5;
  const int co_blk = blockIdx.y;
  const bool xform = p.in_scale != nullptr;
  for (int c = tid; c < Cin; c += 256) {
    s_sc[c] = xform ? p.in_scale[b * Cin + c] : 1.f;
    s_sh[c] = xform ? p.in_shift[b * Cin + c] : 0.f;
  }
  const bool act = xform && p.in_act;

  const int wave = tid >> 6, lane = tid & 63, l31 = lane & 31, kh = lane >> 5;
  const size_t HW = (size_t)H * W;
  int poff[FP];
#pragma unroll
  for (int j = 0; j < FP; ++j) {
    int y = ty * T::ROWS + wave * FP + j, x = tx * 32 + l31;
    y = y < H ? y : H - 1;
    x = x < W ? x : W - 1;
    poff[j] = y * W + x;
  }

  f32x16 acc[FC][FP];
#pragma unroll
  for (int i = 0; i < FC; ++i)
#pragma unroll
    for (int j = 0; j < FP; ++j)
#pragma unroll
      for (int r = 0; r < 16; ++r) acc[i][j][r] = 0.f;

  const float* wbase = p.w + (size_t)co_blk * Cin * CO_T;
  constexpr int NW4 = KC * CO_T / 4 / 256;
  float xb[NSTEP][FP], xn[NSTEP][FP];
  f32x4 rw[NW4];

  auto load_x = [&](int c0, float (&dst)[NSTEP][FP]) {
    const bool first = c0 < p.C1;
    const float* base = first ? p.src1 + ((size_t)b * p.C1 + c0 + kh) * HW : p.src2 + ((size_t)b * p.C2 + (c0 - p.C1) + kh) * HW;
#pragma unroll
    for (int s = 0; s < NSTEP; ++s)
#pragma unroll
      for (int j = 0; j < FP; ++j) dst[s][j] = base[(size_t)(2 * s) * HW + poff[j]];
  };
  auto load_w = [&](int c0) {
#pragma unroll
    for (int i = 0; i < NW4; ++i) rw[i] = *reinterpret_cast<const f32x4*>(wbase + (size_t)c0 * CO_T + 4 * (tid + 256 * i));
  };
  auto store_w = [&](float* sw) {
#pragma unroll
    for (int i = 0; i < NW4; ++i) *reinterpret_cast<f32x4*>(sw + 4 * (tid + 256 * i)) = rw[i];
  };
  auto compute = [&](const float* sw, int c0) {
    float a[2][FC];
    auto lda = [&](int s, int slot) {
#pragma unroll
      for (int i = 0; i < FC; ++i) a[slot][i] = sw[(2 * s + kh) * CO_T + i * 32 + l31];
    };
    lda(0, 0);
#pragma unroll
    for (int s = 0; s < NSTEP; ++s) {
      if (s + 1 < NSTEP) lda(s + 1, (s + 1) & 1);
      const float sc = s_sc[c0 + 2 * s + kh], sh = s_sh[c0 + 2 * s + kh];
      float bb[FP];
#pragma unroll
      for (int j = 0; j < FP; ++j) {
        float t = xb[s][j] * sc + sh;
        bb[j] = act ? silu_f(t) : t;
      }
#pragma unroll
      for (int i = 0; i < FC; ++i)
#pragma unroll
        for (int j = 0; j < FP; ++j)
          acc[i][j] = __builtin_amdgcn_mfma_f32_32x32x2f32(a[s & 1][i], bb[j], acc[i][j], 0, 0, 0);
    }
  };

  const int nchunk = Cin / KC;
  load_x(0, xb);
  load_w(0);
  store_w(s_w0);
  __syncthreads();
#pragma unroll 1
  for (int ci = 0; ci < nchunk; ci += 2) {
    const int cn = (ci + 1 < nchunk ? ci + 1 : ci) * KC;
    load_x(cn, xn);
    load_w(cn);
    compute(s_w0, ci * KC);
// ... 24 lines not shown
```

sgmse_amd/csrc/kernels_conv_pipe.h:

```cpp
#pragma once
#include "kernels_conv.h"

namespace sgmse {

template <int KS, int WC, int FC, int FP>
__global__ __launch_bounds__(256, 2) void conv_mfma_pipe_kernel(ConvArgs p) {
  using T = ConvTile<KS, WC, FC, FP, 1>;
  constexpr int CO_T = T::CO_T, ROWS = T::ROWS, HALO = T::HALO, RS = T::RS, PLANE = T::PLANE, TAPS = T::TAPS, TROWS = T::TROWS;
  constexpr int KH = T::KC / 2;
  constexpr int IN_ELEMS = KH * PLANE, W_ELEMS = KH * TAPS * CO_T;
  constexpr int NVI = KH * TROWS * 8, NV = (NVI + 255) / 256;
  constexpr int NHI = KH * TROWS * 2 * HALO;
  constexpr int NW4 = (W_ELEMS / 4 + 255) / 256;
  constexpr int NTASK = NV + (HALO ? 1 : 0) + NW4;
  constexpr int NS = (KH / 2) * TAPS;
  static_assert(NTASK <= NS - 1, "not enough MFMA groups to hide the staging tasks");
  static_assert(NHI <= 256, "halo items must fit one per thread");

  __shared__ float s_in0[IN_ELEMS];
  __shared__ float s_in1[IN_ELEMS];
  __shared__ float s_w0[W_ELEMS];
  __shared__ float s_w1[W_ELEMS];
  __shared__ float s_sc[512];
  __shared__ float s_sh[512];

  const int tid = threadIdx.x;
  const int Cin = p.C1 + p.C2;
  const int tiles_xg = (p.W + 31) >> 5;
  const int tiles_y = (p.H + ROWS - 1) / ROWS;
  int b, ty, tx;
  conv_tile_of(p, (int)blockIdx.x, (int)gridDim.x, tiles_xg, tiles_y, b, ty, tx);
  if (p.rag_w) { if (!conv_ragged_adjust(p, b, tx)) return; }
  const int tiles_x = (p.W + 31) >> 5;
  const int x0 = tx * 32, y0 = ty * ROWS;
  const int co_blk = blockIdx.y;
  const int H = p.H, W = p.W;
  const bool xform = p.in_scale != nullptr;
  for (int c = tid; c < Cin; c += 256) {
    s_sc[c] = xform ? p.in_scale[b * Cin + c] : 1.f;
    s_sh[c] = xform ? p.in_shift[b * Cin + c] : 0.f;
  }
  const bool act = xform && p.in_act;

  const int wave = tid >> 6, lane = tid & 63, l31 = lane & 31, kh = lane >> 5;
  const int wc = wave % WC, wp = wave / WC;
  const int a_off = kh * TAPS * CO_T + wc * FC * 32 + l31;
  const int b_off = kh * PLANE + (wp * FP) * RS + l31 + T::XOFF;

  f32x16 acc[FC][FP];
#pragma unroll
  for (int i = 0; i < FC; ++i)
#pragma unroll
    for (int j = 0; j < FP; ++j)
#pragma unroll
      for (int r = 0; r < 16; ++r) acc[i][j][r] = 0.f;

  f32x4 rv[NV];
  f32x4 rw[NW4];
  float rh = 0.f;
  unsigned okmask = 0;
  int goff_v[NV], loff_v[NV], cv[NV];
  int goff_h = 0, loff_h = 0, ch = 0;
#pragma unroll
  for (int i = 0; i < NV; ++i) {
    int it = tid + 256 * i;
    it = it < NVI ? it : NVI - 1;
    const int c = it / (TROWS * 8);
    const int rem = it - c * (TROWS * 8);
    const int r = rem >> 3, q = rem & 7;
    const int gy = y0 - HALO + r, gx = x0 + 4 * q;
    const bool ok = gy >= 0 && gy < H && gx < W;
    okmask |= (ok ? 1u : 0u) << i;
    goff_v[i] = ok ? gy * W + gx : 0;
    loff_v[i] = c * PLANE + r * RS + (HALO ? 4 : 0) + 4 * q;
    cv[i] = c;
  }
  if (HALO) {
    const int it = tid < NHI ? tid : NHI - 1;
    const int c = it / (TROWS * 2);
    const int rem = it - c * (TROWS * 2);
    const int r = rem >> 1, side = rem & 1;
    const int gy = y0 - HALO + r, gx = side ? x0 + 32 : x0 - 1;
    const bool ok = gy >= 0 && gy < H && gx >= 0 && gx < W;
    okmask |= (ok ? 1u : 0u) << 31;
    goff_h = ok ? gy * W + gx : 0;
    loff_h = c * PLANE + r * RS + (side ? 36 : 3);
    ch = c;
  }
  const float* wbase = p.w + (size_t)co_blk * Cin * TAPS * CO_T;
  const size_t HW = (size_t)H * W;
  const int nst = Cin / KH;

  auto plane_of = [&](int cg) -> const float* {
    return (cg < p.C1) ? p.src1 + (size_t)(b * p.C1 + cg) * HW : p.src2 + (size_t)(b * p.C2 + (cg - p.C1)) * HW;
  };
  auto xf1 = [&](float v, float sc, float sh, bool ok) -> float {
    v = v * sc + sh;
    const float sv = silu_f(v);
    v = act ? sv : v;
    return ok ? v : 0.f;
  };

  constexpr int NPART = 4;
  f32x4 tmp_o;
  auto task_part = [&](auto itc, auto partc, auto nbc, int st_store, int st_load) {
    constexpr int IT = decltype(itc)::value, PART = decltype(partc)::value, NB = decltype(nbc)::value;
    float* din = NB ? s_in1 : s_in0;
    float* dw = NB ? s_w1 : s_w0;
    if constexpr (IT < NV) {
      const int cg = st_store * KH + cv[IT];
      const bool ok = (okmask >> IT) & 1u;
      if constexpr (PART == 0) { const float sc = s_sc[cg], sh = s_sh[cg]; tmp_o[0] = xf1(rv[IT][0], sc, sh, ok); tmp_o[1] = xf1(rv[IT][1], sc, sh, ok); }
      if constexpr (PART == 1) { const float sc = s_sc[cg], sh = s_sh[cg]; tmp_o[2] = xf1(rv[IT][2], sc, sh, ok); tmp_o[3] = xf1(rv[IT][3], sc, sh, ok); }
      if constexpr (PART == 2) *reinterpret_cast<f32x4*>(din + loff_v[IT]) = tmp_o;
      if constexpr (PART == 3) rv[IT] = *reinterpret_cast<const f32x4*>(plane_of(st_load * KH + cv[IT]) + goff_v[IT]);
    } else if constexpr (HALO && IT == NV) {
      const int cg = st_store * KH + ch;
      if constexpr (PART == 0) din[loff_h] = xf1(rh, s_sc[cg], s_sh[cg], (okmask >> 31) & 1u);
      if constexpr (PART == 2) rh = plane_of(st_load * KH + ch)[goff_h];
    } else {
      constexpr int WI = IT - NV - (HALO ? 1 : 0);
      int idx = tid + 256 * WI;
      idx = idx < W_ELEMS / 4 ? idx : W_ELEMS / 4 - 1;
      if constexpr (PART == 0) reinterpret_cast<f32x4*>(dw)[idx] = rw[WI];
      if constexpr (PART == 2) rw[WI] = reinterpret_cast<const f32x4*>(wbase + (size_t)st_load * KH * TAPS * CO_T)[idx];
    }
  };
  auto task = [&](auto itc, auto nbc, int st_store, int st_load) {
    task_part(itc, std::integral_constant<int, 0>{}, nbc, st_store, st_load);
    task_part(itc, std::integral_constant<int, 1>{}, nbc, st_store, st_load);
    task_part(itc, std::integral_constant<int, 2>{}, nbc, st_store, st_load);
    task_part(itc, std::integral_constant<int, 3>{}, nbc, st_store, st_load);
  };

  auto stage = [&](auto cbc, int st_store, int st_load) {
    constexpr int CB = decltype(cbc)::value;
    using NBc = std::integral_constant<int, CB ^ 1>;
    const float* sw = (CB ? s_w1 : s_w0) + a_off;
    const float* si = (CB ? s_in1 : s_in0) + b_off;
    float a[2][FC], bb[2][FP];
    auto ld = [&](int s2, int slot) {
      const int cp = s2 / TAPS, tap = s2 % TAPS, dy = tap / KS, dx = tap % KS;
#pragma unroll
      for (int i = 0; i < FC; ++i) a[slot][i] = sw[i * 32 + (cp * 2 * TAPS + tap) * CO_T];
#pragma unroll
      for (int j = 0; j < FP; ++j) bb[slot][j] = si[j * RS + cp * 2 * PLANE + dy * RS + dx];
    };
    ld(0, 0);
    constexpr int NM = FC * FP, SL = (NM + NPART - 1) / NPART;
    auto group = [&](auto sc2) {
      constexpr int S2 = decltype(sc2)::value;
      if (S2 + 1 < NS) ld(S2 + 1, (S2 + 1) & 1);
      auto slice = [&](auto qc) {
        constexpr int Q = decltype(qc)::value;
#pragma unroll
        for (int m = Q * SL; m < (Q + 1) * SL && m < NM; ++m) {
          const int i = m / FP, j = m % FP;
          acc[i][j] = __builtin_amdgcn_mfma_f32_32x32x2f32(a[S2 & 1][i], bb[S2 & 1][j], acc[i][j], 0, 0, 0);
        }
        if constexpr (S2 >= 1 && S2 - 1 < NTASK) task_part(std::integral_constant<int, S2 - 1>{}, qc, NBc{}, st_store, st_load);
        __builtin_amdgcn_sched_barrier(0);
      };
      slice(std::integral_constant<int, 0>{});
      slice(std::integral_constant<int, 1>{});
      slice(std::integral_constant<int, 2>{});
      slice(std::integral_constant<int, 3>{});
    };
    auto run = [&](auto self, auto sc2) -> void {
      constexpr int S2 = decltype(sc2)::value;
      if constexpr (S2 < NS) { group(sc2); self(self, std::integral_constant<int, S2 + 1>{}); }
    };
    run(run, std::integral_constant<int, 0>{});
  };

  using B0 = std::integral_constant<int, 0>;
  using B1 = std::integral_constant<int, 1>;
  auto clampst = [&](int s) { return s < nst ? s : nst - 1; };
// ... 37 lines not shown
```

sgmse_amd/csrc/kernels_conv_split.h:

```cpp
#pragma once
#include "kernels_conv.h"

#ifndef SGMSE_SPLIT_FENCE
#define SGMSE_SPLIT_FENCE 0
#endif

namespace sgmse {

struct SplitB3 {
  static constexpr int NS = 3;
  static constexpr int NP = 6;
  static constexpr int PX_V = 7;
  static constexpr bool SCALED = false;
  __device__ static constexpr int pa(int k) { return k == 0 ? 2 : (k == 2 || k == 3) ? 1 : 0; }
  __device__ static constexpr int pb(int k) { return k == 1 ? 2 : (k == 2 || k == 4) ? 1 : 0; }
  __device__ static __forceinline__ void split(float x, uint32_t (&t)[3]) {
    const uint32_t xb = __builtin_bit_cast(uint32_t, x);
    const uint32_t hi = xb & 0xffff0000u;
    const float r1 = x - __builtin_bit_cast(float, hi);
    const uint32_t mid = __builtin_bit_cast(uint32_t, r1) & 0xffff0000u;
    const float r2 = r1 - __builtin_bit_cast(float, mid);
    t[0] = hi >> 16; t[1] = mid >> 16; t[2] = __builtin_bit_cast(uint32_t, r2) >> 16;
  }
  __device__ static __forceinline__ void split2(float x0, float x1, uint32_t (&d)[3]) {
// ... 46 lines not shown
  for (size_t i = (size_t)blockIdx.x * 256 + threadIdx.x; i < n; i += (size_t)gridDim.x * 256) m = fmaxf(m, fabsf(x[i]));
#pragma unroll
  for (int o = 32; o >= 1; o >>= 1) m = fmaxf(m, __shfl_xor(m, o));
  if ((threadIdx.x & 63) == 0) drt_atomic_max_nonneg(out, m);
}

template <class S>
__global__ __launch_bounds__(256) void pack_weights_split_kernel(PackSplitArgs p) {
  const size_t e = (size_t)blockIdx.x * 256 + threadIdx.x;
  if (e >= p.total) return;
  const int lane = (int)(e & 63);
  size_t r = e >> 6;
  const int w = (int)(r & 3); r >>= 2;
  const int split = (int)(r % S::NS); r /= S::NS;
  const int tap = (int)(r % p.taps); r /= p.taps;
  const int nst = p.cin / 16;
  const int st = (int)(r % nst);
  const int blk = (int)(r / nst);
  const int co = blk * 128 + w * 32 + (lane & 31);
  const int c0 = st * 16 + 8 * (lane >> 5);
  const float wscale = (S::SCALED && co < p.cout) ? p.co_scale[co] : 1.f;
  u32x4 o;
#pragma unroll
  for (int q = 0; q < 4; ++q) {
    uint32_t part[2];
#pragma unroll
    for (int h = 0; h < 2; ++h) {
      const int c = c0 + 2 * q + h;
      const float v = (co < p.cout ? p.src[((size_t)co * p.cin + c) * p.taps + tap] : 0.f) * wscale;
      uint32_t t[S::NS];
      S::split(v, t);
      uint32_t sel = t[0];
#pragma unroll
      for (int s = 1; s < S::NS; ++s) sel = split == s ? t[s] : sel;
      part[h] = sel;
    }
    o[q] = part[0] | (part[1] << 16);
  }
  reinterpret_cast<u32x4*>(p.dst)[e] = o;
}

template <class S>
inline size_t packed_split_frags(int cin, int cout, int taps = 9) { return (size_t)((cout + 127) / 128) * (cin / 16) * taps * S::NS * 4 * 64; }
template <class S>
inline size_t packed_split_bytes(int cin, int cout, int taps = 9) { return packed_split_frags<S>(cin, cout, taps) * 16 + (size_t)((cout + 127) / 128) * 128 * 8; }

template <class S, int SHAPE = 0, int ACT = 1, int ABL = 0, int SC = 0, int CHK = 0>
__global__ __launch_bounds__(256, 2) void conv3x3_split_kernel(ConvArgs p) {
  static_assert(!CHK || (SHAPE == 2 && !SC), "chunked accumulation exists for the plain 4-row shape");
  constexpr bool THIN = SHAPE == 1;
  constexpr int ROWS = SHAPE == 2 ? 4 : 8;
  using C = ConvSplitGeom<ROWS>;
  constexpr int WCW = THIN ? 1 : 4;
  constexpr int FCW = THIN ? 1 : 4 / WCW;
  constexpr int FPW = THIN ? 2 : ROWS / (4 / WCW);
  using T = ConvTile<3, WCW, FCW, FPW, 1>;
  static_assert(T::CO_T == (THIN ? 32 : 128) && T::ROWS == ROWS, "tile");
  constexpr int NS = S::NS, PX_V = S::PX_V;
  constexpr int EPJ = 8 / FPW;
  constexpr int STAGE_V = C::TROWS * C::TCOLS * PX_V;
  constexpr int DUMMY_V = STAGE_V;
  __shared__ u32x4 s_in0[STAGE_V + NS];
  __shared__ u32x4 s_in1[STAGE_V + NS];
  constexpr int NCO = S::SCALED ? 4 : 2;
  __shared__ float s_co[512 * NCO];

  const int tid = threadIdx.x;
  if constexpr (ABL & 512) {
    __shared__ u32x4 s_pad[3072];
    if (p.ablate == 12345) s_pad[tid] = u32x4{0u, 0u, 0u, 0u};
  }
  unsigned long long* trace = nullptr;
  if constexpr (ABL & 64) {
    if (tid == 0 && p.trace) {
      trace = p.trace + 16 * (size_t)(blockIdx.y * gridDim.x + blockIdx.x);
      trace[0] = (unsigned long long)drt_hw_id() | ((unsigned long long)drt_xcc_id() << 32);
      trace[1] = drt_clock();
    }
  }
  const int Cin = p.C1 + p.C2;
  const int tiles_xg = (p.W + 31) >> 5;
  const int tiles_y = (p.H + ROWS - 1) / ROWS;
  int b, ty, tx;
  conv_tile_of(p, (int)blockIdx.x, (int)gridDim.x, tiles_xg, tiles_y, b, ty, tx);
  if (p.rag_w) { if (!conv_ragged_adjust(p, b, tx)) return; }
  const int H = p.H, W = p.W;
  const int tiles_x = (W + 31) >> 5;
  const int co_blk = blockIdx.y;
  const int x0 = tx * 32, y0 = ty * ROWS;
  float xb_raw = 0.f;
  if constexpr (S::SCALED) { if (p.xbound) xb_raw = p.xbound[b * kAmaxSpread + (tid & (kAmaxSpread - 1))]; }
  float csc[2], csh[2];
#pragma unroll
  for (int k = 0; k < 2; ++k) {
    const int c = tid + 256 * k;
    const bool ld = p.in_scale != nullptr && c < Cin;
    csc[k] = ld ? p.in_scale[b * Cin + (c < Cin ? c : 0)] : 1.f;
    csh[k] = ld ? p.in_shift[b * Cin + (c < Cin ? c : 0)] : 0.f;
  }
  const unsigned HW = (unsigned)H * (unsigned)W;

  const int wave = tid >> 6, lane = tid & 63, l31 = lane & 31, kg = lane >> 5;

  unsigned it_boff[C::NIT];
  int it_loff[C::NIT], it_g[C::NIT];
#pragma unroll
  for (int i = 0; i < C::NIT; ++i) {
    int it = tid + 256 * i;
    it = it < C::NITEM ? it : C::NITEM - 1;
    const int g = it / (C::TROWS * C::TCOLS);
    const int rem = it - g * (C::TROWS * C::TCOLS);
    const int r = rem / C::TCOLS, c = rem - r * C::TCOLS;
    const int gy = y0 - 1 + r, gx = x0 - 1 + c;
    const bool ok = gy >= 0 && gy < H && gx >= 0 && gx < W;
    const int loff = (r * C::TCOLS + c) * PX_V + g * NS;
    if (!ok) {
#pragma unroll
      for (int s = 0; s < NS; ++s) { s_in0[loff + s] = u32x4{0u, 0u, 0u, 0u}; s_in1[loff + s] = u32x4{0u, 0u, 0u, 0u}; }
    }
    it_boff[i] = ((unsigned)(8 * g) * HW + (ok ? (unsigned)(gy * W + gx) : 0u)) * 4u;
    it_loff[i] = ok ? loff : DUMMY_V;
    it_g[i] = g;
  }

  float rin[C::NIT][8];
  auto load_item = [&](int i, int c0) {
    const bool first = c0 < p.C1;
    const float* base = first ? p.src1 + ((size_t)b * p.C1 + c0) * HW : p.src2 + ((size_t)b * p.C2 + (c0 - p.C1)) * HW;
#pragma unroll
    for (int e = 0; e < 8; ++e)
      rin[i][e] = *reinterpret_cast<const float*>(reinterpret_cast<const char*>(base + (size_t)e * HW) + it_boff[i]);
  };
  auto produce = [&](float x, int ch) -> float {
    float o, u;
    if constexpr (NCO == 4) {
      const f32x4 co = reinterpret_cast<const f32x4*>(s_co)[ch];
      o = x * co[0] + co[1];
      u = x * co[2] + co[3];
    } else {
      o = x * s_co[2 * ch] + s_co[2 * ch + 1];
      u = o * -1.4426950408889634f;
    }
    if constexpr (ACT == 1) {
      if constexpr (ABL & 4) o = o * u;
      else o = o * __builtin_amdgcn_rcpf(1.0f + drt_exp2(u));
    }
    if (S::SCALED) o = fminf(fmaxf(o, -65504.f), 65504.f);
    return o;
  };
  auto store_item = [&](int i, int c0, u32x4* sbuf) {
    u32x4 v[NS];
#pragma unroll
    for (int q = 0; q < 4; ++q) {
      const int ch = c0 + 8 * it_g[i] + 2 * q;
      uint32_t d[NS];
      S::split2(produce(rin[i][2 * q], ch), produce(rin[i][2 * q + 1], ch + 1), d);
#pragma unroll
      for (int s = 0; s < NS; ++s) v[s][q] = d[s];
    }
#pragma unroll
    for (int s = 0; s < NS; ++s) sbuf[it_loff[i] + s] = v[s];
  };

  u32x4 pk[NS];
  float ev = 0.f;
  auto stage_elem = [&](int i, int e, int c0, const float (&raw)[C::NIT][8]) {
    const float o = produce(raw[i][e], c0 + 8 * it_g[i] + e);
    if ((e & 1) == 0) { ev = o; return; }
    uint32_t d[NS];
    S::split2(ev, o, d);
#pragma unroll
// ... 255 lines not shown
  }
  if constexpr (ABL & 32) load_a(0, 2, ar[2]);
#pragma unroll 1
  for (int st = st0; st < st1; ++st) {
    const int stn = st + 1 < st1 ? st + 1 : st;
    const u32x4* cur = ((st - st0) & 1) ? s_in1 : s_in0;
    u32x4* nxt = ((st - st0) & 1) ? s_in0 : s_in1;
#pragma unroll
    for (int tap = 0; tap < 9; ++tap) {
      unsigned long long tc0 = 0;
      if constexpr (ABL & 64) tc0 = drt_clock();
      const int ntap = (tap + AD) % 9;
      const int nstg = tap + AD < 9 ? st : stn;
      if constexpr (!(ABL & 32)) load_a(nstg, ntap, ar[(tap + AD) % AR]);
      if constexpr (!(ABL & 8)) { if (tap < C::NIT) load_item(tap, stn * C::KC); }
      __builtin_amdgcn_sched_barrier(0);
      int item = (tap >= 4 && (tap & 1) == 0 && (tap - 4) / 2 < C::NIT) ? (tap - 4) / 2 : -1;
      if constexpr (ABL & 8) item = -1;
      compute_tap(cur, tap, ar[tap % AR], item, stn * C::KC, nxt, rin);
      if constexpr (ABL & 64) { __builtin_amdgcn_sched_barrier(0); tsum[tap] += drt_clock() - tc0; }
    }
    if constexpr (ABL & 64) {
      const unsigned long long tb = drt_clock();
      __syncthreads();
      tsum[9] += drt_clock() - tb;
    } else {
      __syncthreads();
    }
    if constexpr (CHK) {
      if (gridDim.z == 1 && ((st + 1) % p.kchunk_stages == 0 || st + 1 == st1)) {
#pragma unroll
        for (int i = 0; i < FCW; ++i)
#pragma unroll
          for (int j = 0; j < FPW; ++j)
#pragma unroll
            for (int r = 0; r < 16; ++r) { tot[i][j][r] = first_chunk ? acc[i][j][r] : tot[i][j][r] + acc[i][j][r]; acc[i][j][r] = 0.f; }
        first_chunk = false;
      }
    }
  }
  if constexpr (CHK) {
    if (gridDim.z == 1) {
#pragma unroll
      for (int i = 0; i < FCW; ++i)
#pragma unroll
        for (int j = 0; j < FPW; ++j) acc[i][j] = tot[i][j];
    } else {
      ConvArgs q = p;
      q.out = p.partial + (size_t)blockIdx.z * conv_partial_slab(p, H, W);
      q.bias = nullptr; q.bias2 = nullptr; q.res = nullptr; q.acc_scale = nullptr; q.co_scale = nullptr; q.out_scale = 1.f; q.stats_out = nullptr; q.amax_out = nullptr;
      conv_epilogue<T, FCW, FPW, WCW, 0, true>(q, acc, b, co_blk, tx, ty, tiles_x, wc, wp, l31, kg);
      return;
    }
  }
  if constexpr (ABL & 64) {
    if (trace) {
#pragma unroll
      for (int i = 0; i < 10; ++i) trace[5 + i] = tsum[i];
    }
  }

  if constexpr (ABL & 64) { if (trace) trace[3] = drt_clock(); }
  conv_epilogue<T, FCW, FPW, WCW, ABL & (3 | 128 | 256), !CHK, FPW % 4 == 0, S::SCALED>(p, acc, b, co_blk, tx, ty, tiles_x, wc, wp, l31, kg, inv_kx);
  if constexpr (ABL & 64) { if (trace) trace[4] = drt_clock(); }
}

template <class S, int XF = 1, int VEC = 0>
__global__ __launch_bounds__(256, 2) void conv1x1_split_kernel(ConvArgs p) {
  using T = ConvTile<1, 4, 1, 8, 1>;
  static_assert(T::CO_T == 128 && T::ROWS == 8, "tile");
  static_assert(!VEC || !XF, "16-byte staging exists for raw inputs only");
  constexpr int NS = S::NS, PX_V = S::PX_V, KC = 16, NIT = 2;
  constexpr int STAGE_V = 256 * PX_V;
  __shared__ u32x4 s_in0[STAGE_V];
  __shared__ u32x4 s_in1[STAGE_V];
  __shared__ float s_sc[XF ? 512 : 1];
  __shared__ float s_sh[XF ? 512 : 1];

  const int tid = threadIdx.x;
  const int Cin = p.C1 + p.C2;
  const int tiles_xg = (p.W + 31) >> 5;
  const int tiles_y = (p.H + 7) >> 3;
  int b, ty, tx;
  conv_tile_of(p, (int)blockIdx.x, (int)gridDim.x, tiles_xg, tiles_y, b, ty, tx);
  if (p.rag_w) { if (!conv_ragged_adjust(p, b, tx)) return; }
  const int H = p.H, W = p.W;
  const int tiles_x = (W + 31) >> 5;
  const int co_blk = blockIdx.y;
  const int x0 = tx * 32, y0 = ty * 8;
  float actf = 0.f;
  if constexpr (XF) {
    const bool xform = p.in_scale != nullptr;
    for (int c = tid; c < Cin; c += 256) {
      s_sc[c] = xform ? p.in_scale[b * Cin + c] : 1.f;
      s_sh[c] = xform ? p.in_shift[b * Cin + c] : 0.f;
    }
    actf = (xform && p.in_act) ? 1.f : 0.f;
  }
  const size_t HW = (size_t)H * W;
  const int wave = tid >> 6, lane = tid & 63, l31 = lane & 31, kg = lane >> 5;
  float xs = 1.f;
  if (S::SCALED) {
    float m = p.amax1 ? amax_read(p.amax1, b) : 0.f;
    if (p.amax2) m = fmaxf(m, amax_read(p.amax2, b));
    xs = h2_weight_scale(m);
  }

  int it_goff[NIT], it_loff[NIT], it_g[NIT];
  if constexpr (VEC) {
    const int cq = tid & 7, h = (tid >> 3) & 1, g = (tid >> 4) & 1, r = tid >> 5;
    int gy = y0 + r, gx = x0 + 4 * cq;
    gy = gy < H ? gy : H - 1; gx = gx < W ? gx : W - 4;
    it_goff[0] = gy * W + gx;
    it_loff[0] = ((r * 32 + 4 * cq) * PX_V + g * NS) * 2 + h;
    it_g[0] = 8 * g + 4 * h;
    it_goff[1] = it_loff[1] = it_g[1] = 0;
  } else {
#pragma unroll
    for (int i = 0; i < NIT; ++i) {
      const int it = tid + 256 * i;
      const int g = it >> 8, r = (it >> 5) & 7, c = it & 31;
      int gy = y0 + r, gx = x0 + c;
      gy = gy < H ? gy : H - 1; gx = gx < W ? gx : W - 1;
      it_goff[i] = gy * W + gx;
      it_loff[i] = (r * 32 + c) * PX_V + g * NS;
      it_g[i] = g;
    }
  }
  float rinA[NIT][8], rinB[NIT][8];
  auto load_items = [&](int c0, float (&dst)[NIT][8]) {
    const bool first = c0 < p.C1;
    const float* base = first ? p.src1 + ((size_t)b * p.C1 + c0) * HW : p.src2 + ((size_t)b * p.C2 + (c0 - p.C1)) * HW;
    if constexpr (VEC) {
#pragma unroll
      for (int e = 0; e < 4; ++e) {
        const f32x4 v = *reinterpret_cast<const f32x4*>(base + (size_t)(it_g[0] + e) * HW + it_goff[0]);
#pragma unroll
        for (int q = 0; q < 4; ++q) dst[e >> 1][4 * (e & 1) + q] = v[q];
      }
    } else {
#pragma unroll
      for (int i = 0; i < NIT; ++i)
#pragma unroll
        for (int e = 0; e < 8; ++e) dst[i][e] = base[(size_t)(8 * it_g[i] + e) * HW + it_goff[i]];
    }
  };
  u32x4 pk[NS];
  uint32_t ev[NS];
  auto stage_elem = [&](int i, int e, int c0, const float (&src)[NIT][8]) {
    float t = src[i][e];
    if constexpr (XF) {
      const int ch = c0 + 8 * it_g[i] + e;
      t = t * s_sc[ch] + s_sh[ch];
      const float sig = __builtin_amdgcn_rcpf(1.0f + __expf(-t));
      t *= actf * (sig - 1.0f) + 1.0f;
    }
    if (S::SCALED) t = fminf(fmaxf(t * xs, -65504.f), 65504.f);
    uint32_t t16[NS];
    S::split(t, t16);
#pragma unroll
    for (int s = 0; s < NS; ++s) {
      if ((e & 1) == 0) ev[s] = t16[s]; else pk[s][e >> 1] = ev[s] | (t16[s] << 16);
    }
  };
  auto flush_item = [&](int i, u32x4* sbuf) {
#pragma unroll
    for (int s = 0; s < NS; ++s) sbuf[it_loff[i] + s] = pk[s];
  };
  uint32_t hv[NS];
  auto stage_quad = [&](int k, const float (&src)[NIT][8], u32x4* sbuf) {
    const int q = k >> 1, cp = k & 1;
// ... 95 lines not shown
```

sgmse_amd/csrc/kernels_conv_wino.h:

```cpp
#pragma once
#include "kernels_conv_split.h"

#ifndef SGMSE_WINO_TAIL_STAGING
#define SGMSE_WINO_TAIL_STAGING 0
#endif

namespace sgmse {

template <int ROWS_>
struct WinoGeom {
  static constexpr int KC = 16, ROWS = ROWS_, TROWS = ROWS_ + 2, NF = ROWS_ / 2;
  static constexpr int PV = 17;
  static constexpr int ROW_V = 16 * PV;
  static constexpr int STAGE_V = TROWS * ROW_V;
  static constexpr int NSROW = 4 * TROWS;
  static constexpr int NPASS = (NSROW + 2) / 3;
  static constexpr int NIT = (NPASS + 7) / 8;
  static constexpr int CO_V = 512;
  static constexpr int NDIR = ROWS_ == 4 ? 1 : 2;
  static constexpr int XCH_V = 4 * NDIR * 2 * 16 * 64 / 2;
  static constexpr int LDS_V = (2 * STAGE_V + CO_V) > XCH_V ? (2 * STAGE_V + CO_V) : XCH_V;
};
template <int ROWS_>
struct WinoTile { static constexpr int CO_T = 128, ROWS = ROWS_; };
// ... 1 lines not shown
struct PackWinoArgs { const float* src; uint32_t* dst; int cin, cout; size_t total; };
inline size_t packed_wino_frags(int cin, int cout) { return (size_t)((cout + 127) / 128) * (cin / 16) * 12 * 2 * 4 * 64; }
inline size_t packed_wino_bytes(int cin, int cout) { return packed_wino_frags(cin, cout) * 16 + (size_t)((cout + 127) / 128) * 128 * 4; }

__device__ __forceinline__ float wino_co_absmax(const float* src, int cin, int co) {
  float m = 0.f;
  for (int i = 0; i < cin * 3; ++i) {
    const float* g = src + ((size_t)co * cin * 3 + i) * 3;
    const float g0 = g[0], g1 = g[1], g2 = g[2];
    m = fmaxf(m, fmaxf(fmaxf(fabsf(g0), fabsf(g2)), fmaxf(fabsf(0.5f * (g0 + g1 + g2)), fabsf(0.5f * (g0 - g1 + g2)))));
  }
  return m;
}
__global__ __launch_bounds__(256) void wino_co_scale_kernel(const float* src, int cin, int cout, int cout_pad, float* inv_scale, float* scale) {
  const int co = blockIdx.x * 256 + threadIdx.x;
  if (co >= cout_pad) return;
  const float s = co < cout ? h2_weight_scale(wino_co_absmax(src, cin, co)) : 1.f;
  scale[co] = s; inv_scale[co] = 1.f / s;
}
__global__ __launch_bounds__(256) void pack_weights_wino_kernel(PackWinoArgs p, const float* co_scale) {
  const size_t e = (size_t)blockIdx.x * 256 + threadIdx.x;
  if (e >= p.total) return;
  const int lane = (int)(e & 63);
  size_t r = e >> 6;
  const int cf = (int)(r & 3); r >>= 2;
  const int split = (int)(r & 1); r >>= 1;
  const int k = (int)(r & 3); r >>= 2;
  const int dy = (int)(r % 3); r /= 3;
  const int nst = p.cin / 16;
  const int st = (int)(r % nst);
  const int blk = (int)(r / nst);
  const int co = blk * 128 + cf * 32 + (lane & 31);
  const int c0 = st * 16 + 8 * (lane >> 5);
  const double ws = co < p.cout ? (double)co_scale[co] : 1.0;
  u32x4 o;
#pragma unroll
  for (int q = 0; q < 4; ++q) {
    uint32_t part[2];
#pragma unroll
    for (int h = 0; h < 2; ++h) {
      const int c = c0 + 2 * q + h;
      double u = 0.0;
      if (co < p.cout) {
        const float* g = p.src + (((size_t)co * p.cin + c) * 3 + dy) * 3;
        const double g0 = g[0], g1 = g[1], g2 = g[2];
        u = k == 0 ? g0 : k == 1 ? 0.5 * (g0 + g1 + g2) : k == 2 ? 0.5 * (g0 - g1 + g2) : g2;
      }
      u *= ws;
      const uint32_t hi = drt_f32_to_f16((float)u);
      const uint32_t lo = drt_f32_to_f16((float)(u - (double)drt_f16_to_f32(hi)));
      part[h] = split ? lo : hi;
    }
    o[q] = part[0] | (part[1] << 16);
  }
  reinterpret_cast<u32x4*>(p.dst)[e] = o;
}

template <int ROWS, int ACT, int SC, int TRACE = 0, int ABL = 0>
__global__ __launch_bounds__(512, 1) void conv3x3_wino_kernel(ConvArgs p) {
  using G = WinoGeom<ROWS>;
  using T = WinoTile<ROWS>;
  using S = SplitH2;
  constexpr int NF = G::NF, NIT = G::NIT, PV = G::PV, NS = 2;
  __shared__ u32x4 s_all[G::LDS_V];
  u32x4* const s_in0 = s_all;
  u32x4* const s_in1 = s_all + G::STAGE_V;
  f32x4* const s_co = reinterpret_cast<f32x4*>(s_all + 2 * G::STAGE_V);

  const int tid = threadIdx.x;
  const int wave = drt_uniform(tid >> 6), lane = tid & 63, l31 = lane & 31, kg = lane >> 5;
  const int cf = wave & 3, kh = wave >> 2;
  unsigned long long* trace = nullptr;
  if constexpr (TRACE) {
    if (tid == 0 && p.trace) {
      trace = p.trace + 32 * (size_t)(blockIdx.y * gridDim.x + blockIdx.x);
      trace[0] = (unsigned long long)drt_hw_id() | ((unsigned long long)drt_xcc_id() << 32);
      trace[1] = drt_clock();
    }
  }
  const int Cin = p.C1 + p.C2;
  const int tiles_xg = (p.W + 31) >> 5;
  const int tiles_y = (p.H + ROWS - 1) / ROWS;
  int b, ty, tx;
  conv_tile_of(p, (int)blockIdx.x, (int)gridDim.x, tiles_xg, tiles_y, b, ty, tx);
  if (p.rag_w) { if (!conv_ragged_adjust(p, b, tx)) return; }
  const int H = p.H, W = p.W;
  const int tiles_x = (W + 31) >> 5;
  const int co_blk = blockIdx.y;
  const int x0 = tx * 32, y0 = ty * ROWS;
  const unsigned HW = (unsigned)H * (unsigned)W;

  float xb_raw = 0.f;
  if (p.xbound) xb_raw = p.xbound[b * kAmaxSpread + (tid & (kAmaxSpread - 1))];
  const bool cld = p.in_scale != nullptr && tid < Cin;
  const float csc = cld ? p.in_scale[b * Cin + (tid < Cin ? tid : 0)] : 1.f;
  const float csh = cld ? p.in_shift[b * Cin + (tid < Cin ? tid : 0)] : 0.f;

  unsigned it_boff[NIT];
  int it_woff[NIT], it_q[NIT];
  bool it_ok[NIT], it_wr[NIT], it_run[NIT];
#pragma unroll
  for (int i = 0; i < NIT; ++i) {
    const int pass = wave + 8 * i;
    const int sub = lane / 18, j = lane - 18 * sub;
    const int rr = 3 * pass + sub;
    const bool live = sub < 3 && rr < G::NSROW;
    const int q = rr & 3, r = live ? rr >> 2 : 0;
    const int gy = y0 - 1 + r, gx = x0 - 2 + 2 * j;
    const bool ok = live && gy >= 0 && gy < H && gx >= 0 && gx < W;
    it_boff[i] = ((unsigned)(4 * q) * HW + (ok ? (unsigned)(gy * W + gx) : 0u)) * 4u;
    it_woff[i] = ((r * 16 + (j - 1)) * PV + (q >> 1) * NS) * 2 + (q & 1);
    it_q[i] = q; it_ok[i] = ok; it_wr[i] = live && j >= 1 && j <= 16;
    it_run[i] = 3 * pass < G::NSROW;
  }
  float rin[NIT][8];
  auto load_item = [&](int i, int c0) {
    const bool first = c0 < p.C1;
    const float* base = first ? p.src1 + ((size_t)b * p.C1 + c0) * HW : p.src2 + ((size_t)b * p.C2 + (c0 - p.C1)) * HW;
#pragma unroll
    for (int c = 0; c < 4; ++c) {
      const float2 v = *reinterpret_cast<const float2*>(reinterpret_cast<const char*>(base + (size_t)c * HW) + it_boff[i]);
      rin[i][2 * c] = v.x; rin[i][2 * c + 1] = v.y;
    }
  };
  float V[4][4];
  auto produce_co = [&](float x, const f32x4& co, bool ok) -> float {
    float o = x * co[0] + co[1];
    if constexpr (ACT == 1) {
      const float u = x * co[2] + co[3];
      if constexpr (ABL & 1) o = o * u; else o = o * __builtin_amdgcn_rcpf(1.0f + drt_exp2(u));
    }
    return ok ? o : 0.f;
  };
  auto stage_chan_co = [&](int i, int c, const f32x4& co) {
    const float e = produce_co(rin[i][2 * c], co, it_ok[i]), o = produce_co(rin[i][2 * c + 1], co, it_ok[i]);
    const float ol = (ABL & 2) ? e : drt_wave_shr1(o), er = (ABL & 2) ? o : drt_wave_shl1(e);
    V[0][c] = ol - o; V[1][c] = e + o; V[2][c] = o - e; V[3][c] = e - er;
  };
  auto stage_chan = [&](int i, int c, int c0) { stage_chan_co(i, c, s_co[c0 + 4 * it_q[i] + c]); };
  auto flush_k = [&](int i, int k, u32x4* sbuf) {
    if (it_wr[i] && (!(ABL & 4) || V[k][0] == 12345.678f)) {
      uint2* w = reinterpret_cast<uint2*>(sbuf) + it_woff[i];
      uint32_t d01[2], d23[2];
      S::split2(V[k][0], V[k][1], d01);
      S::split2(V[k][2], V[k][3], d23);
      if constexpr (ABL & 32) {
        if ((d01[0] ^ d23[1]) == 0x12345678u) w[k * 8] = make_uint2(d01[0] ^ d01[1], d23[0] ^ d23[1]);
      } else {
        w[k * 8] = make_uint2(d01[0], d23[0]);
        w[k * 8 + 2] = make_uint2(d01[1], d23[1]);
      }
    }
  };
  auto flush_item = [&](int i, u32x4* sbuf) {
#pragma unroll
    for (int k = 0; k < 4; ++k) flush_k(i, k, sbuf);
  };

  const int nst = Cin / G::KC;
  const float* cs_tab = p.co_scale + (size_t)co_blk * 128;
  float acc_raw[16];
  if constexpr (!SC) conv_acc_raw<T>(p, b, co_blk, cf, kg, acc_raw);
  auto load_cs = [&](float (&cs)[16]) {
#pragma unroll
    for (int r = 0; r < 16; ++r) cs[r] = cs_tab[cf * 32 + 4 * kg + (r & 3) + 8 * (r >> 2)];
  };
  float sc_m1 = 0.f, sc_m2 = 0.f;
  if constexpr (SC) {
    sc_m1 = p.sc_amax1[b * kAmaxSpread + (tid & (kAmaxSpread - 1))];
    if (p.sc_amax2) sc_m2 = p.sc_amax2[b * kAmaxSpread + (tid & (kAmaxSpread - 1))];
  } else {
// ... 370 lines not shown
```

sgmse_amd/csrc/kernels_conv_wino2d.h:

```cpp
#pragma once
#include "kernels_conv_wino.h"

namespace sgmse {

struct Wino2Geom {
  static constexpr int KC = 16, ROWS = 4, TROWS = 6;
  static constexpr int PV = 65;
  static constexpr int STAGE_V = 32 * PV;
  static constexpr int SCR_E = 68;
  static constexpr int SCR_F = TROWS * 16 * SCR_E;
  static constexpr int SCR_V = SCR_F / 4;
  static constexpr int CO_V = 512;
  static constexpr int XCH_V = 4 * 2 * 16 * 64 / 2;
  static constexpr int LDS_V = 2 * STAGE_V + 2 * SCR_V + CO_V;
  static_assert(XCH_V <= 2 * STAGE_V, "exchange buffer must fit the stage buffers");
};
struct Wino2Tile { static constexpr int CO_T = 128, ROWS = 4; };

__device__ __forceinline__ double wino2d_u(const float* g, int i, int j) {
  const double G[4][3] = {{1.0, 0.0, 0.0}, {0.5, 0.5, 0.5}, {0.5, -0.5, 0.5}, {0.0, 0.0, 1.0}};
  double u = 0.0;
#pragma unroll
  for (int a = 0; a < 3; ++a)
#pragma unroll
    for (int b = 0; b < 3; ++b) u += G[i][a] * (double)g[a * 3 + b] * G[j][b];
  return u;
}
inline size_t packed_wino2d_frags(int cin, int cout) { return (size_t)((cout + 127) / 128) * (cin / 16) * 16 * 2 * 4 * 64; }
inline size_t packed_wino2d_bytes(int cin, int cout) { return packed_wino2d_frags(cin, cout) * 16 + (size_t)((cout + 127) / 128) * 128 * 4; }

__global__ __launch_bounds__(256) void wino2d_co_scale_kernel(const float* src, int cin, int cout, int cout_pad, float* inv_scale, float* scale) {
  const int co = blockIdx.x * 256 + threadIdx.x;
  if (co >= cout_pad) return;
  float m = 0.f;
  if (co < cout) {
    for (int c = 0; c < cin; ++c) {
      const float* g = src + ((size_t)co * cin + c) * 9;
#pragma unroll
      for (int i = 0; i < 4; ++i)
#pragma unroll
        for (int j = 0; j < 4; ++j) m = fmaxf(m, fabsf((float)wino2d_u(g, i, j)) * 1.0000002f);
    }
  }
  const float s = co < cout ? h2_weight_scale(m) : 1.f;
  scale[co] = s; inv_scale[co] = 1.f / s;
}
__global__ __launch_bounds__(256) void pack_weights_wino2d_kernel(PackWinoArgs p, const float* co_scale) {
  const size_t e = (size_t)blockIdx.x * 256 + threadIdx.x;
  if (e >= p.total) return;
  const int lane = (int)(e & 63);
  size_t r = e >> 6;
  const int cf = (int)(r & 3); r >>= 2;
  const int split = (int)(r & 1); r >>= 1;
  const int comp = (int)(r & 15); r >>= 4;
  const int nst = p.cin / 16;
  const int st = (int)(r % nst);
  const int blk = (int)(r / nst);
  const int co = blk * 128 + cf * 32 + (lane & 31);
  const int c0 = st * 16 + 8 * (lane >> 5);
  const double ws = co < p.cout ? (double)co_scale[co] : 1.0;
  u32x4 o;
#pragma unroll
  for (int q = 0; q < 4; ++q) {
    uint32_t part[2];
#pragma unroll
    for (int h = 0; h < 2; ++h) {
      const int c = c0 + 2 * q + h;
      double u = 0.0;
      if (co < p.cout) u = wino2d_u(p.src + ((size_t)co * p.cin + c) * 9, comp >> 2, comp & 3);
      u *= ws;
      const uint32_t hi = drt_f32_to_f16((float)u);
      const uint32_t lo = drt_f32_to_f16((float)(u - (double)drt_f16_to_f32(hi)));
      part[h] = split ? lo : hi;
    }
    o[q] = part[0] | (part[1] << 16);
  }
  reinterpret_cast<u32x4*>(p.dst)[e] = o;
}

template <int ACT, int ABL = 0>
__global__ __launch_bounds__(512, 1) void conv3x3_wino2d_kernel(ConvArgs p) {
  using G = Wino2Geom;
  using T = Wino2Tile;
  using S = SplitH2;
  constexpr int PV = G::PV, NS = 2, ROWS = 4;
  __shared__ u32x4 s_all[G::LDS_V];
  u32x4* const s_st0 = s_all;
  u32x4* const s_st1 = s_all + G::STAGE_V;
  float* const s_scr0 = reinterpret_cast<float*>(s_all + 2 * G::STAGE_V);
  float* const s_scr1 = s_scr0 + G::SCR_F;
  f32x4* const s_co = reinterpret_cast<f32x4*>(s_all + 2 * G::STAGE_V + 2 * G::SCR_V);

  const int tid = threadIdx.x;
  const int wave = drt_uniform(tid >> 6), lane = tid & 63, l31 = lane & 31, kg = lane >> 5;
  const int cf = wave & 3, kh = wave >> 2;
  const int Cin = p.C1 + p.C2;
  const int tiles_xg = (p.W + 31) >> 5;
  const int tiles_y = (p.H + ROWS - 1) / ROWS;
  int b, ty, tx;
  conv_tile_of(p, (int)blockIdx.x, (int)gridDim.x, tiles_xg, tiles_y, b, ty, tx);
  if (p.rag_w) { if (!conv_ragged_adjust(p, b, tx)) return; }
  const int H = p.H, W = p.W;
  const int tiles_x = (W + 31) >> 5;
  const int co_blk = blockIdx.y;
  const int x0 = tx * 32, y0 = ty * ROWS;
  const unsigned HW = (unsigned)H * (unsigned)W;

  float xb_raw = 0.f;
  if (p.xbound) xb_raw = p.xbound[b * kAmaxSpread + (tid & (kAmaxSpread - 1))];
  const bool cld = p.in_scale != nullptr && tid < Cin;
  const float csc = cld ? p.in_scale[b * Cin + (tid < Cin ? tid : 0)] : 1.f;
  const float csh = cld ? p.in_shift[b * Cin + (tid < Cin ? tid : 0)] : 0.f;

  const int sub1 = lane / 18, j1 = lane - 18 * sub1;
  const int rr1 = 3 * wave + sub1;
  const bool live1 = sub1 < 3;
  const int q1 = rr1 & 3, r1 = live1 ? rr1 >> 2 : 0;
  const int gy1 = y0 - 1 + r1, gx1 = x0 - 2 + 2 * j1;
  const bool ok1 = live1 && gy1 >= 0 && gy1 < H && gx1 >= 0 && gx1 < W;
  const unsigned boff1 = ((unsigned)(4 * q1) * HW + (ok1 ? (unsigned)(gy1 * W + gx1) : 0u)) * 4u;
  const bool wr1 = live1 && j1 >= 1 && j1 <= 16;
  const int soff1 = (r1 * 16 + (wr1 ? j1 - 1 : 0)) * G::SCR_E + q1 * 4;
  float rin[8];
  auto load_raw = [&](int c0) {
    const bool first = c0 < p.C1;
    const float* base = first ? p.src1 + ((size_t)b * p.C1 + c0) * HW : p.src2 + ((size_t)b * p.C2 + (c0 - p.C1)) * HW;
#pragma unroll
    for (int c = 0; c < 4; ++c) {
      const float2 v = *reinterpret_cast<const float2*>(reinterpret_cast<const char*>(base + (size_t)c * HW) + boff1);
      rin[2 * c] = v.x; rin[2 * c + 1] = v.y;
    }
  };
  auto produce_co = [&](float x, const f32x4& co, bool ok) -> float {
    float o = x * co[0] + co[1];
    if constexpr (ACT == 1) {
      const float u = x * co[2] + co[3];
      o = o * __builtin_amdgcn_rcpf(1.0f + drt_exp2(u));
    }
    return ok ? o : 0.f;
  };
  float Hh[4][4];
  auto phase1_chan = [&](int c, const f32x4& co) {
    const float e = produce_co(rin[2 * c], co, ok1), o = produce_co(rin[2 * c + 1], co, ok1);
    const float ol = drt_wave_shr1(o), er = drt_wave_shl1(e);
    Hh[0][c] = ol - o; Hh[1][c] = e + o; Hh[2][c] = o - e; Hh[3][c] = e - er;
  };
  auto phase1_store = [&](float* scr) {
    if (wr1) {
#pragma unroll
      for (int hc = 0; hc < 4; ++hc) {
        f32x4 v = {Hh[hc][0], Hh[hc][1], Hh[hc][2], Hh[hc][3]};
        *reinterpret_cast<f32x4*>(scr + soff1 + hc * 16) = v;
      }
    }
  };
  auto phase1 = [&](int c0, float* scr) {
    f32x4 co4[4];
#pragma unroll
    for (int c = 0; c < 4; ++c) co4[c] = s_co[c0 + 4 * q1 + c];
#pragma unroll
    for (int c = 0; c < 4; ++c) phase1_chan(c, co4[c]);
    phase1_store(scr);
  };
  const int q2 = tid & 3, hc2 = (tid >> 2) & 3, tc2 = (tid >> 4) & 15, tr2 = tid >> 8;
  const int roff2 = ((2 * tr2) * 16 + tc2) * G::SCR_E + hc2 * 16 + q2 * 4;
  const int woff2 = (((tr2 * 16 + tc2) * PV + hc2 * 4 + (q2 >> 1) * NS) * 2) + (q2 & 1);
  f32x4 Vv[4];
  auto phase2_load = [&](const float* scr) {
    f32x4 R[4];
#pragma unroll
    for (int k = 0; k < 4; ++k) R[k] = *reinterpret_cast<const f32x4*>(scr + roff2 + k * 16 * G::SCR_E);
#pragma unroll
    for (int c = 0; c < 4; ++c) { Vv[0][c] = R[0][c] - R[2][c]; Vv[1][c] = R[1][c] + R[2][c]; Vv[2][c] = R[2][c] - R[1][c]; Vv[3][c] = R[1][c] - R[3][c]; }
  };
  auto phase2_store = [&](int i, u32x4* stg) {
    uint2* w = reinterpret_cast<uint2*>(stg) + woff2 + i * 32;
    uint32_t d01[2], d23[2];
    S::split2(Vv[i][0], Vv[i][1], d01);
    S::split2(Vv[i][2], Vv[i][3], d23);
    w[0] = make_uint2(d01[0], d23[0]);
    w[2] = make_uint2(d01[1], d23[1]);
  };
  auto phase2 = [&](const float* scr, u32x4* stg) {
    phase2_load(scr);
#pragma unroll
    for (int i = 0; i < 4; ++i) phase2_store(i, stg);
  };
// ... 198 lines not shown
```

sgmse_amd/csrc/kernels_conv_wino43.h:

```cpp
#pragma once
#include "kernels_conv_wino.h"

namespace sgmse {

template <int ROWS_>
struct Wino43Geom {
  static constexpr int KC = 16, ROWS = ROWS_, TROWS = ROWS_ + 2, NF = ROWS_ / 4, NK = 6;
  static constexpr int PV = 25;
  static constexpr int ROW_V = 8 * PV;
  static constexpr int STAGE_V = TROWS * ROW_V;
  static constexpr int NSROW = 4 * TROWS;
  static constexpr int NPASS = (NSROW + 5) / 6;
  static constexpr int CO_V = 512;
  static constexpr int NDIR = ROWS_ == 4 ? 1 : 2;
  static constexpr int XCH_V = 4 * NDIR * 16 * 64;
  static constexpr int LDS_V = (2 * STAGE_V + CO_V) > XCH_V ? (2 * STAGE_V + CO_V) : XCH_V;
  static_assert(NPASS <= 8, "one staging pass per wave");
};

inline size_t packed_wino43_frags(int cin, int cout) { return (size_t)((cout + 127) / 128) * (cin / 16) * 18 * 2 * 4 * 64; }
inline size_t packed_wino43_bytes(int cin, int cout) { return packed_wino43_frags(cin, cout) * 16 + (size_t)((cout + 127) / 128) * 128 * 4; }

__device__ __forceinline__ double wino43_u(double g0, double g1, double g2, int k) {
  return k == 0 ? 0.25 * g0 : k == 1 ? -(g0 + g1 + g2) / 6.0 : k == 2 ? -(g0 - g1 + g2) / 6.0
       : k == 3 ? g0 / 24.0 + g1 / 12.0 + g2 / 6.0 : k == 4 ? g0 / 24.0 - g1 / 12.0 + g2 / 6.0 : g2;
}
__global__ __launch_bounds__(64) void wino43_co_scale_kernel(const float* src, int cin, int cout, int cout_pad, float* inv_scale, float* scale) {
  const int co = blockIdx.x;
  if (co >= cout_pad) return;
  float m = 0.f;
  if (co < cout) {
    for (int i = threadIdx.x; i < cin * 3; i += 64) {
      const float* g = src + ((size_t)co * cin * 3 + i) * 3;
      m = fmaxf(m, fmaxf(0.25f * fabsf(g[0]), fabsf(g[2])));
      for (int k = 1; k < 5; ++k) m = fmaxf(m, fabsf((float)wino43_u(g[0], g[1], g[2], k)));
    }
  }
#pragma unroll
  for (int o = 32; o >= 1; o >>= 1) m = fmaxf(m, __shfl_xor(m, o));
  if (threadIdx.x == 0) {
    const float s = co < cout ? h2_weight_scale(m) : 1.f;
    scale[co] = s; inv_scale[co] = 1.f / s;
  }
}
__global__ __launch_bounds__(256) void pack_weights_wino43_kernel(PackWinoArgs p, const float* co_scale) {
  const size_t e = (size_t)blockIdx.x * 256 + threadIdx.x;
  if (e >= p.total) return;
  const int lane = (int)(e & 63);
  size_t r = e >> 6;
  const int cf = (int)(r & 3); r >>= 2;
  const int split = (int)(r & 1); r >>= 1;
  const int k = (int)(r % 6); r /= 6;
  const int dy = (int)(r % 3); r /= 3;
  const int nst = p.cin / 16;
  const int st = (int)(r % nst);
  const int blk = (int)(r / nst);
  const int co = blk * 128 + cf * 32 + (lane & 31);
  const int c0 = st * 16 + 8 * (lane >> 5);
  const double ws = co < p.cout ? (double)co_scale[co] : 1.0;
  u32x4 o;
#pragma unroll
  for (int q = 0; q < 4; ++q) {
    uint32_t part[2];
#pragma unroll
    for (int h = 0; h < 2; ++h) {
      const int c = c0 + 2 * q + h;
      double u = 0.0;
      if (co < p.cout) {
        const float* g = p.src + (((size_t)co * p.cin + c) * 3 + dy) * 3;
        u = wino43_u(g[0], g[1], g[2], k);
      }
      u *= ws;
      const uint32_t hi = drt_f32_to_f16((float)u);
      const uint32_t lo = drt_f32_to_f16((float)(u - (double)drt_f16_to_f32(hi)));
      part[h] = split ? lo : hi;
    }
    o[q] = part[0] | (part[1] << 16);
  }
  reinterpret_cast<u32x4*>(p.dst)[e] = o;
}

template <int ROWS, int ACT, int TRACE = 0>
__global__ __launch_bounds__(512, 1) void conv3x3_wino43_kernel(ConvArgs p) {
  using G = Wino43Geom<ROWS>;
  using T = WinoTile<ROWS>;
  using S = SplitH2;
  constexpr int NF = G::NF, PV = G::PV, NS = 2;
  __shared__ u32x4 s_all[G::LDS_V];
  u32x4* const s_in0 = s_all;
  u32x4* const s_in1 = s_all + G::STAGE_V;
  f32x4* const s_co = reinterpret_cast<f32x4*>(s_all + 2 * G::STAGE_V);

  const int tid = threadIdx.x;
  const int wave = drt_uniform(tid >> 6), lane = tid & 63, l31 = lane & 31, kg = lane >> 5;
  const int cf = wave & 3, kh = wave >> 2;
  unsigned long long* trace = nullptr;
  if constexpr (TRACE) {
    if (tid == 0 && p.trace) {
      trace = p.trace + 32 * (size_t)(blockIdx.y * gridDim.x + blockIdx.x);
      trace[0] = (unsigned long long)drt_hw_id() | ((unsigned long long)drt_xcc_id() << 32);
      trace[1] = drt_clock();
    }
  }
  const int Cin = p.C1 + p.C2;
  const int tiles_xg = (p.W + 31) >> 5;
  const int tiles_y = (p.H + ROWS - 1) / ROWS;
  int b, ty, tx;
  conv_tile_of(p, (int)blockIdx.x, (int)gridDim.x, tiles_xg, tiles_y, b, ty, tx);
  if (p.rag_w) { if (!conv_ragged_adjust(p, b, tx)) return; }
  const int H = p.H, W = p.W;
  const int tiles_x = (W + 31) >> 5;
  const int co_blk = blockIdx.y;
  const int x0 = tx * 32, y0 = ty * ROWS;
  const unsigned HW = (unsigned)H * (unsigned)W;

  float xb_raw = 0.f;
  if (p.xbound) xb_raw = p.xbound[b * kAmaxSpread + (tid & (kAmaxSpread - 1))];
  const bool cld = p.in_scale != nullptr && tid < Cin;
  const float csc = cld ? p.in_scale[b * Cin + (tid < Cin ? tid : 0)] : 1.f;
  const float csh = cld ? p.in_shift[b * Cin + (tid < Cin ? tid : 0)] : 0.f;

  const int it_sub = lane / 10, it_j = lane - 10 * it_sub;
  const int it_rr = 6 * wave + it_sub;
  const bool it_live = it_sub < 6 && it_rr < G::NSROW;
  const int it_q = it_rr & 3, it_r = it_live ? it_rr >> 2 : 0;
  const int it_gy = y0 - 1 + it_r, it_gx = x0 - 4 + 4 * it_j;
  const bool it_ok = it_live && it_gy >= 0 && it_gy < H && it_gx >= 0 && it_gx < W;
  const unsigned it_boff = ((unsigned)(4 * it_q) * HW + (it_ok ? (unsigned)(it_gy * W + it_gx) : 0u)) * 4u;
  const int it_woff = ((it_r * 8 + (it_j - 1)) * PV + (it_q >> 1) * NS) * 2 + (it_q & 1);
  const bool it_wr = it_live && it_j >= 1 && it_j <= 8;
  const bool it_run = 6 * wave < G::NSROW;
  float rin[16];
  auto load_item = [&](int c0) {
    const bool first = c0 < p.C1;
    const float* base = first ? p.src1 + ((size_t)b * p.C1 + c0) * HW : p.src2 + ((size_t)b * p.C2 + (c0 - p.C1)) * HW;
#pragma unroll
    for (int c = 0; c < 4; ++c) {
      const float4 v = *reinterpret_cast<const float4*>(reinterpret_cast<const char*>(base + (size_t)c * HW) + it_boff);
      rin[4 * c] = v.x; rin[4 * c + 1] = v.y; rin[4 * c + 2] = v.z; rin[4 * c + 3] = v.w;
    }
  };
  float V[6][4];
  auto produce_co = [&](float x, const f32x4& co) -> float {
    float o = x * co[0] + co[1];
    if constexpr (ACT == 1) {
      const float u = x * co[2] + co[3];
      o = o * __builtin_amdgcn_rcpf(1.0f + drt_exp2(u));
    }
    return it_ok ? o : 0.f;
  };
  auto stage_chan_co = [&](int c, const f32x4& co) {
    const float d1 = produce_co(rin[4 * c], co), d2 = produce_co(rin[4 * c + 1], co);
    const float d3 = produce_co(rin[4 * c + 2], co), d4 = produce_co(rin[4 * c + 3], co);
    const float d0 = drt_wave_shr1(d4), d5 = drt_wave_shl1(d1);
    const float a = d4 - d2, bb = d3 - d1;
    const float c4 = d4 - 4.f * d2, c3 = d3 - 4.f * d1;
    V[0][c] = 4.f * (d0 - d2) + a;
    V[1][c] = c4 + c3;
    V[2][c] = c4 - c3;
    V[3][c] = a + 2.f * bb;
    V[4][c] = a - 2.f * bb;
    V[5][c] = (d5 - d3) - 4.f * bb;
  };
  auto flush_item = [&](u32x4* sbuf) {
    if (it_wr) {
      uint2* w = reinterpret_cast<uint2*>(sbuf) + it_woff;
#pragma unroll
      for (int k = 0; k < 6; ++k) {
        uint32_t d01[2], d23[2];
        S::split2(V[k][0], V[k][1], d01);
        S::split2(V[k][2], V[k][3], d23);
        w[k * 8] = make_uint2(d01[0], d23[0]);
        w[k * 8 + 2] = make_uint2(d01[1], d23[1]);
      }
    }
  };

  const int nst = Cin / G::KC;
  const float* cs_tab = p.co_scale + (size_t)co_blk * 128;
  float acc_raw[16];
  conv_acc_raw<T>(p, b, co_blk, cf, kg, acc_raw);
  auto load_cs = [&](float (&cs)[16]) {
#pragma unroll
    for (int r = 0; r < 16; ++r) cs[r] = cs_tab[cf * 32 + 4 * kg + (r & 3) + 8 * (r >> 2)];
  };
  if (it_run) load_item(0);
  float kx = 1.f;
  if (p.xbound) {
#pragma unroll
    for (int o = 32; o >= 1; o >>= 1) xb_raw = fmaxf(xb_raw, __shfl_xor(xb_raw, o));
    kx = h2_weight_scale(xb_raw) * 0.125f;
  }
  const float inv_kx = 1.f / kx;
  if (tid < Cin) {
    constexpr float nl2e = -1.4426950408889634f;
// ... 244 lines not shown
```

sgmse_amd/ops.py:

```python
from __future__ import annotations

from typing import Dict, Optional, Tuple

import torch

from . import _lib

_ctx: Dict[str, "_lib.Context"] = {}


def default_context(device: "torch.device | str | None" = None) -> "_lib.Context":
    if device is None:
        device = "cpu" if _lib.is_emulator() else torch.device("cuda", torch.cuda.current_device())
    key = str(torch.device(device))
    if key not in _ctx:
        _ctx[key] = _lib.Context(device)
    return _ctx[key]


def _f32(t: Optional[torch.Tensor], name: str, dev) -> Optional[torch.Tensor]:
    return None if t is None else _lib.check_tensor(t, name, torch.float32, dev)


def conv2d(x: torch.Tensor, weight: torch.Tensor, bias: Optional[torch.Tensor] = None, *,
           residual: Optional[torch.Tensor] = None, out_scale: float = 1.0, x2: Optional[torch.Tensor] = None,
           in_scale: Optional[torch.Tensor] = None, in_shift: Optional[torch.Tensor] = None, in_act: bool = False,
           force_direct: bool = False, force_split: Optional[str] = None) -> torch.Tensor:
    ctx = default_context(x.device)
    dev = ctx.device
    x = _f32(x, "x", dev); weight = _f32(weight, "weight", dev)
    B, C1, H, W = x.shape
    C2 = 0 if x2 is None else x2.shape[1]
    Cout, Cin, kh, kw = weight.shape
    if kh != kw or kh not in (1, 3):
        raise ValueError("kernel must be 1x1 or 3x3")
    if Cin != C1 + C2:
        raise ValueError(f"weight expects {Cin} input channels, got {C1}+{C2}")
    out = torch.empty((B, Cout, H, W), dtype=torch.float32, device=dev)
    ctx.use_current_stream()
    ctx.check(ctx.lib.sgmse_op_conv2d(ctx.h, x.data_ptr(), weight.data_ptr(), _lib.ptr(_f32(bias, "bias", dev)),
                                      _lib.ptr(_f32(residual, "residual", dev)), out.data_ptr(), B, Cin, Cout, H, W, kh,
                                      float(out_scale), {None: int(force_direct), 'bf16x3': 2, 'fp16x2': 3, 'wino': 4, 'wino4': 5, 'thin': 6, 'wino2d': 7, 'wino43': 8, 'wino43_4': 9}[force_split], _lib.ptr(_f32(in_scale, "in_scale", dev)),
                                      _lib.ptr(_f32(in_shift, "in_shift", dev)), int(in_act),
                                      _lib.ptr(_f32(x2, "x2", dev)), C2))
    return out


def group_norm(x: torch.Tensor, weight: torch.Tensor, bias: torch.Tensor, *, act: bool = False,
               x2: Optional[torch.Tensor] = None) -> torch.Tensor:
    ctx = default_context(x.device)
    dev = ctx.device
    x = _f32(x, "x", dev)
    B, C1, H, W = x.shape
    C2 = 0 if x2 is None else x2.shape[1]
    C = C1 + C2
    out = torch.empty((B, C, H, W), dtype=torch.float32, device=dev)
    ctx.use_current_stream()
    ctx.check(ctx.lib.sgmse_op_groupnorm(ctx.h, x.data_ptr(), _f32(weight, "weight", dev).data_ptr(),
                                         _f32(bias, "bias", dev).data_ptr(), out.data_ptr(), B, C, H, W, int(act),
                                         _lib.ptr(_f32(x2, "x2", dev)), C2))
    return out


def fir_resample(x: torch.Tensor, up: bool, in_scale: Optional[torch.Tensor] = None, in_shift: Optional[torch.Tensor] = None,
                 in_act: bool = False, return_raw: bool = False):
    ctx = default_context(x.device)
    x = _f32(x, "x", ctx.device)
    B, Cc, H, W = x.shape
    shape = (B, Cc, 2 * H, 2 * W) if up else (B, Cc, H // 2, W // 2)
    out = torch.empty(shape, dtype=torch.float32, device=ctx.device)
    raw = torch.empty(shape, dtype=torch.float32, device=ctx.device) if return_raw else None
    sc = _f32(in_scale, "in_scale", ctx.device)
    sh = _f32(in_shift, "in_shift", ctx.device)
    if (sc is None) != (sh is None) or (sc is not None and (tuple(sc.shape) != (B, Cc) or tuple(sh.shape) != (B, Cc))):
        raise ValueError("in_scale and in_shift must both be given, with shape [B, C]")
    ctx.use_current_stream()
    ctx.check(ctx.lib.sgmse_op_fir(ctx.h, x.data_ptr(), out.data_ptr(), B * Cc, H, W, int(up), _lib.ptr(sc), _lib.ptr(sh),
                                   int(bool(in_act)), _lib.ptr(raw)))
    return (out, raw) if return_raw else out


def upfirdn2d(x: torch.Tensor, kernel: torch.Tensor, up: int = 1, down: int = 1, pad: Tuple[int, int] = (0, 0)) -> torch.Tensor:
    ctx = default_context(x.device)
    code = {torch.float32: 0, torch.float64: 1, torch.float16: 2}.get(x.dtype)
    if code is None:
        raise ValueError(f"upfirdn2d: input dtype {x.dtype} is not supported (float32, float64, float16 -- op/upfirdn2d_kernel.cu:311)")
    if not kernel.dtype.is_floating_point:
        raise ValueError(f"upfirdn2d: kernel dtype {kernel.dtype} is not a floating-point type")
    if kernel.device != x.device:
        raise ValueError(f"upfirdn2d: kernel on {kernel.device}, input on {x.device} (the reference op checks both tensors, upfirdn2d.cpp:15-16)")
    dt = x.dtype
    x = _lib.check_tensor(x, "input", dt, ctx.device); kernel = kernel.to(dtype=dt).contiguous()
    N, Cc, H, W = x.shape
    kh, kw = kernel.shape
    Ho = (H * up + pad[0] + pad[1] - kh) // down + 1
    Wo = (W * up + pad[0] + pad[1] - kw) // down + 1
    out = torch.empty((N, Cc, Ho, Wo), dtype=dt, device=ctx.device)
    ctx.use_current_stream()
    ctx.check(ctx.lib.sgmse_upfirdn2d_dtype(ctx.h, code, x.data_ptr(), kernel.data_ptr(), out.data_ptr(), N * Cc, H, W, kh, kw, up, up,
                                            down, down, pad[0], pad[1], pad[0], pad[1]))
    return out


def attention(qkv: torch.Tensor) -> torch.Tensor:
    ctx = default_context(qkv.device)
    qkv = _f32(qkv, "qkv", ctx.device)
    B, C3, S = qkv.shape
    out = torch.empty((B, C3 // 3, S), dtype=torch.float32, device=ctx.device)
    ctx.use_current_stream()
    ctx.check(ctx.lib.sgmse_op_attention(ctx.h, qkv.data_ptr(), out.data_ptr(), B, C3 // 3, S))
    return out


def stft(sig: torch.Tensor, n_fft: int, hop_length: int, window: torch.Tensor) -> torch.Tensor:
    ctx = default_context(sig.device)
    squeeze = sig.dim() == 1
    s = _f32(sig.reshape(-1, sig.shape[-1]), "sig", ctx.device)
    B, L = s.shape
    K = L // hop_length + 1 if n_fft % 2 == 0 else (L - 1) // hop_length + 1
    out = torch.empty((B, n_fft // 2 + 1, K), dtype=torch.complex64, device=ctx.device)
    ctx.use_current_stream()
    ctx.check(ctx.lib.sgmse_stft(ctx.h, s.data_ptr(), _f32(window, "window", ctx.device).data_ptr(), out.data_ptr(), B, L,
                                 n_fft, hop_length))
    return out[0] if squeeze else out.reshape(*sig.shape[:-1], n_fft // 2 + 1, K)

# ... 56 lines not shown
```

Baseline: 6.167 utterances/s.

## Fold Cout blocks into grid x for large convs and read entry input unpadded

Adds a co_fold mode that flattens the output-channel grid dimension into blockIdx.x so consecutive blocks share the same spatial tile across output-channel blocks. The mode applies only when input is at least 256 MiB unless overridden, and it aims to improve L2/MALL reuse of input tiles. Separately, the entry convolution now reads the 4-channel input directly and treats the padded channels 4..7 as dead planes, instead of materialising a zero-padded 8-channel copy. This removes extra writes and reads in the entry kernel, at the cost of more index arithmetic in the conv kernels.

```diff
diff --git a/sgmse_amd/csrc/conv_launch.h b/sgmse_amd/csrc/conv_launch.h
--- a/sgmse_amd/csrc/conv_launch.h
+++ b/sgmse_amd/csrc/conv_launch.h
@@ -12,6 +12,9 @@
 #ifndef SGMSE_CONV_SPLIT_DEFAULT
 #define SGMSE_CONV_SPLIT_DEFAULT 2
 #endif
+#ifndef SGMSE_CONV_CO_PAIR_DEFAULT
+#define SGMSE_CONV_CO_PAIR_DEFAULT 15
+#endif
 #ifndef SGMSE_CONV_PIPE_DEFAULT
 #define SGMSE_CONV_PIPE_DEFAULT 1
 #endif
@@ -21,6 +24,20 @@
 inline int conv_variant() {
   static int v = [] { const char* e = getenv("SGMSE_CONV_VARIANT"); return e ? atoi(e) : 0; }();
   return v;
+}
+
+enum ConvPairFamily { kPairConv1x1 = 1, kPairWino43 = 2, kPairWino23 = 4, kPairSplit3x3 = 8, kPairAnySize = 16 };
+constexpr double kPairMinInputBytes = 256.0 * 1024 * 1024;
+inline ConvArgs conv_fold_grid(const ConvArgs& a, dim3& grid, int family) {
+  ConvArgs f = a;
+  f.co_fold = 0;
+  const double in_bytes = 4.0 * (a.C1 + a.C2) * a.B * a.H * a.W;
+  if ((a.co_pair & family) && grid.y > 1 && grid.z == 1 && (unsigned long long)grid.x * grid.y < (1ull << 31) &&
+      ((a.co_pair & kPairAnySize) || in_bytes >= kPairMinInputBytes)) {
+    f.co_fold = (int)grid.y;
+    grid.x *= grid.y; grid.y = 1;
+  }
+  return f;
 }
 
 inline int conv_grid_tiles(const ConvArgs& a, int rows) {
@@ -89,7 +106,8 @@
 static_assert(ConvThinGeom::KC == kConvThinKC, "conv_thin_eligible (conv_route.h) assumes the thin kernel's stage depth");
 
 template <class S, int SHAPE>
-inline void launch_conv3x3_split_t(const ConvArgs& a, dim3 grid, drt::stream_t st) {
+inline void launch_conv3x3_split_t(const ConvArgs& a0, dim3 grid, drt::stream_t st) {
+  const ConvArgs a = conv_fold_grid(a0, grid, kPairSplit3x3);
   const bool act = a.in_scale && a.in_act;
   if constexpr (SHAPE != 1 && S::SCALED) {
     if (a.sc_w) {
@@ -104,7 +122,8 @@
 #define SGMSE_CONV1X1_RAW_VEC 1
 #endif
 template <class S>
-inline void launch_conv1x1_split_t(const ConvArgs& a, dim3 grid, drt::stream_t st) {
+inline void launch_conv1x1_split_t(const ConvArgs& a0, dim3 grid, drt::stream_t st) {
+  const ConvArgs a = conv_fold_grid(a0, grid, kPairConv1x1);
   if (a.in_scale) { DRT_LAUNCH((conv1x1_split_kernel<S, 1, 0>), grid, dim3(256), st, a); return; }
   const bool vec = SGMSE_CONV1X1_RAW_VEC && (a.rag_w ? a.rag_vec_ok != 0 : a.W % 4 == 0) && reinterpret_cast<uintptr_t>(a.src1) % 16 == 0 &&
                    (a.src2 == nullptr || reinterpret_cast<uintptr_t>(a.src2) % 16 == 0);
@@ -115,8 +134,10 @@
   const int tiles = conv_grid_tiles(a, 8);
   if (ks == 3 && a.Cout > 32 && rows4 && a.kchunk_stages > 0 && mode == 2) {
     const dim3 grid(conv_grid_tiles(a, 4), a.Cout / 128, ksplit);
-    if (a.in_scale && a.in_act) DRT_LAUNCH((conv3x3_split_kernel<SplitH2, 2, 1, 0, 0, 1>), grid, dim3(256), st, a);
-    else DRT_LAUNCH((conv3x3_split_kernel<SplitH2, 2, 0, 0, 0, 1>), grid, dim3(256), st, a);
+    dim3 fgrid = grid;
+    const ConvArgs f = conv_fold_grid(a, fgrid, kPairSplit3x3);
+    if (a.in_scale && a.in_act) DRT_LAUNCH((conv3x3_split_kernel<SplitH2, 2, 1, 0, 0, 1>), fgrid, dim3(256), st, f);
+    else DRT_LAUNCH((conv3x3_split_kernel<SplitH2, 2, 0, 0, 0, 1>), fgrid, dim3(256), st, f);
     if (ksplit > 1) DRT_LAUNCH((conv_splitk_reduce_kernel<3, 4, 1, 4, true>), dim3(grid.x, grid.y, 1), dim3(256), st, a, ksplit);
     return;
   }
@@ -151,8 +172,9 @@
   return reinterpret_cast<uintptr_t>(a.src1) % 16 == 0 && (a.src2 == nullptr || reinterpret_cast<uintptr_t>(a.src2) % 16 == 0);
 }
 template <int ROWS>
-inline void launch_conv_wino_rows(WinoForm form, const ConvArgs& a, drt::stream_t st) {
-  const dim3 grid(conv_grid_tiles(a, ROWS), a.Cout / 128, 1);
+inline void launch_conv_wino_rows(WinoForm form, const ConvArgs& a0, drt::stream_t st) {
+  dim3 grid(conv_grid_tiles(a0, ROWS), a0.Cout / 128, 1);
+  const ConvArgs a = conv_fold_grid(a0, grid, form == WinoForm::F43 ? kPairWino43 : kPairWino23);
   const bool act = a.in_scale && a.in_act;
   if (form == WinoForm::F43) {
     if (act) DRT_LAUNCH((conv3x3_wino43_kernel<ROWS, 1>), grid, dim3(512), st, a);
diff --git a/sgmse_amd/csrc/engine.h b/sgmse_amd/csrc/engine.h
--- a/sgmse_amd/csrc/engine.h
+++ b/sgmse_amd/csrc/engine.h
@@ -767,17 +767,29 @@
   }
 
   enum ForceConv { FC_AUTO = 0, FC_DIRECT = 1, FC_SPLIT_B3 = 2, FC_SPLIT_H2 = 3, FC_WINO = 4, FC_WINO_4ROW = 5, FC_THIN = 6, FC_WINO2D = 7,
-                   FC_WINO43 = 8, FC_WINO43_4ROW = 9 };
+                   FC_WINO43 = 8, FC_WINO43_4ROW = 9, FC_ENTRY = 10, FC_ENTRY_SMALL = 11 };
   void op_conv2d(const float* x, const float* w_oihw, const float* bias, const float* res, float* out, int B, int Cin,
                  int Cout, int H, int W, int ks, float out_scale, int force_direct, const float* in_scale,
                  const float* in_shift, int in_act, const float* x2, int C2) {
     ConvArgs a{};
     a.src1 = x; a.src2 = x2; a.C1 = Cin - C2; a.C2 = C2; a.bias = bias; a.res = res; a.out_scale = out_scale; a.out = out;
     a.Cout = Cout; a.B = B; a.H = H; a.W = W; a.in_scale = in_scale; a.in_shift = in_shift; a.in_act = in_act;
+    a.xcd_map = conv_xcd_map_ ? 1 : 0; a.co_pair = conv_co_pair_;
     ConvPlan pl = choose_conv_plan(ks, Cin, Cout, H, W);
     const bool wino = force_direct == FC_WINO || force_direct == FC_WINO_4ROW || force_direct == FC_WINO2D || force_direct == FC_WINO43 || force_direct == FC_WINO43_4ROW;
     StandaloneConv s;
-    if (force_direct == FC_THIN) {
+    if (force_direct == FC_ENTRY || force_direct == FC_ENTRY_SMALL) {
+      SG_REQUIRE(ks == 3 && Cin == 4 && C2 == 0 && Cout % 128 == 0 && H >= 8, "op_conv2d: shape is not the entry convolution's");
+      constexpr int cp = 8;
+      const DevBuf w8_buf = fresh((size_t)Cout * cp * 9 * 4);
+      float* w8 = w8_buf.as<float>();
+      DRT_LAUNCH(pad_cin_kernel, dim3((unsigned)(((size_t)Cout * cp * 9 + 255) / 256)), dim3(256), stream_, w_oihw, w8, Cout, 4, cp, 9);
+      a.C1 = cp; a.cin_live = 4;
+      pl = force_direct == FC_ENTRY ? ConvPlan{128, 8, true} : ConvPlan{32, 4, true};
+      s = standalone_conv(a, ConvPack{ConvPack::Mfma, 0, WinoForm::F23, pl.co_t}, w8, ks);
+      launch_conv_mfma(s.a, ks, pl, stream_);
+      SG_CHECK(drt::stream_sync(stream_));
+    } else if (force_direct == FC_THIN) {
       SG_REQUIRE(conv_thin_eligible(ks, a.C1, C2, Cout), "op_conv2d: shape is not eligible for the thin-output kernel");
       s = standalone_conv(a, ConvPack{ConvPack::Thin}, w_oihw, ks);
       launch_conv_thin(s.a, stream_);
@@ -931,6 +943,7 @@
     ConvArgs a0{};
     a0.src1 = x; a0.C1 = Cin; a0.out = o; a0.Cout = Cout; a0.B = B; a0.H = H; a0.W = W; a0.out_scale = 1.f;
     a0.ablate = ablate;
+    a0.xcd_map = conv_xcd_map_ ? 1 : 0; a0.co_pair = conv_co_pair_;
     if (fused) { a0.in_scale = sc; a0.in_shift = sc + (size_t)B * Cin; a0.in_act = 1; a0.res = r; a0.bias = w; a0.out_scale = 0.70710678f; }
     if (b3 && smode == 2 && ks == 1) { a0.in_scale = nullptr; a0.in_shift = nullptr; a0.in_act = 0; }
     EventTimer timer;
@@ -1430,10 +1443,12 @@
 
   Tensor conv(const ConvW& w, const Tensor& a, const Tensor* b, const Xform& xf, const float* bias, const float* bias2,
               const float* res, float out_scale, const FwdCtl& ctl, bool emit_stats = false, const Shortcut* sc = nullptr) {
-    const int C2 = b ? b->C : 0, Cin = a.C + C2;
+    const int live = (!b && a.C < w.cin && entry8_.packed && &w == &entry8_) ? a.C : 0;
+    const int C1 = live ? w.cin : a.C, C2 = b ? b->C : 0, Cin = C1 + C2;
     SG_REQUIRE(Cin == w.cin, "conv: channel mismatch");
+    SG_REQUIRE(!live || (w.ks == 3 && w.cin == 8 && live == 4), "conv: padded input channels outside the entry convolution");
     Tensor o = new_tensor(w.cout, a.H, a.W);
-    const ConvRoute rt = route_of(w, a.C, C2, a.H, a.W, ConvCall{xf.bound != nullptr, a.amax && (!b || b->amax), xf.scale != nullptr, emit_stats,
+    const ConvRoute rt = route_of(w, C1, C2, a.H, a.W, ConvCall{xf.bound != nullptr, a.amax && (!b || b->amax), xf.scale != nullptr, emit_stats,
                                                                  bias2 != nullptr, sc != nullptr});
     const ConvFamily fam = rt.family;
     SG_REQUIRE(fam != ConvFamily::Wino23 || (a.W % 2 == 0 && rag_all_mult(a.H, 2)), "conv: odd width on a Winograd level");
@@ -1453,9 +1468,10 @@
     if (dry_) { if (partial) arena_.release(partial); return o; }
     ConvArgs ca{};
     ca.xcd_map = conv_xcd_map_ ? 1 : 0;
+    ca.co_pair = conv_co_pair_;
     ca.stats_out = o.st; ca.stats_nsub = o.nsub; ca.stats_rows = o.srows;
     ca.amax_out = o.amax;
-    ca.src1 = a.p; ca.src2 = b ? b->p : nullptr; ca.C1 = a.C; ca.C2 = C2;
+    ca.src1 = a.p; ca.src2 = b ? b->p : nullptr; ca.C1 = C1; ca.C2 = C2; ca.cin_live = live;
     ca.bias = bias; ca.bias2 = bias2; ca.bias2_bstride = ctl.bias_bstride; ca.bias2_sstride = ctl.bias_sstride;
     ca.step_ptr = bias2 ? ctl.bias_step : nullptr;
     ca.in_scale = xf.scale; ca.in_shift = xf.shift; ca.in_act = xf.act;
@@ -1721,17 +1737,13 @@
     std::vector<Tensor> hs;
     Tensor xr = new_tensor(4, F, T);
     const bool entry8 = entry_mfma_ && entry8_.packed && layout_[mi].idx == entry8_idx_;
-    Tensor xr8{};
-    if (entry8) xr8 = new_tensor(entry8_.cin, F, T);
     if (!dry_) { tock(); const WrapCoef wc{ctl.coef, ctl.coef_bstride, ctl.coef_sstride, ctl.step_ptr, ctl.sign};
-      DRT_LAUNCH(entry_kernel, dim3((FT + 255) / 256, B), dim3(256), stream_, x, xbs, y, ybs, xr.p, entry8 ? xr8.p : (float*)nullptr,
-                 entry8 ? entry8_.cin : 0, FT, wc, rag_of(F), F, ctl.y_plane);
-      tick(TC_MISC, (32.0 + (entry8 ? 4.0 * entry8_.cin : 0.0)) * B * FT); }
+      DRT_LAUNCH(entry_kernel, dim3((FT + 255) / 256, B), dim3(256), stream_, x, xbs, y, ybs, xr.p, FT, wc, rag_of(F), F, ctl.y_plane);
+      tick(TC_MISC, 32.0 * B * FT); }
     {
       const Mod& m = next();
       const ConvW& w = entry8 ? entry8_ : conv_.at(m.idx);
-      hs.push_back(conv(w, entry8 ? xr8 : xr, nullptr, Xform{}, w.bias, nullptr, nullptr, 1.f, ctl, true));
-      if (entry8) drop(xr8);
+      hs.push_back(conv(w, xr, nullptr, Xform{}, w.bias, nullptr, nullptr, 1.f, ctl, true));
     }
     Tensor pyr_in = xr;
     bool pyr_in_is_xr = true;
@@ -1910,6 +1922,8 @@
     wino43_ = flag("SGMSE_WINO43", true);
     rag_prefix_ = flag("SGMSE_RAGGED_PREFIX", true);
     conv_xcd_map_ = flag("SGMSE_CONV_XCD_MAP", true);
+    e = getenv("SGMSE_CONV_CO_PAIR");
+    conv_co_pair_ = e ? atoi(e) : SGMSE_CONV_CO_PAIR_DEFAULT;
     debug_sync_ = flag("SGMSE_DEBUG_SYNC", false);
     prof_dump_ = flag("SGMSE_PROFILE_DUMP", false);
     e = getenv("SGMSE_TILE_MIN_BLOCKS");
@@ -1942,6 +1956,7 @@
   ConvW entry8_{}; int entry8_idx_ = -1;
   bool poison_ = false, debug_sync_ = false, conv_xcd_map_ = true, rag_prefix_ = true, wino_ = true, wino43_ = true;
   long wino_min_tiles_ = 32;
+  int conv_co_pair_ = SGMSE_CONV_CO_PAIR_DEFAULT;
   int nofold_levels_ = 0;
   bool lds_poison_ = false, lds_poison_upto_ = false; int lds_poison_at_ = -1, lds_poison_count_ = 0; DevArray<unsigned> lds_sink_;
   static constexpr long coarse_splitk_div_ = 4, chunk_max_tiles_ = 8;
diff --git a/sgmse_amd/csrc/kernels_attn_misc.h b/sgmse_amd/csrc/kernels_attn_misc.h
--- a/sgmse_amd/csrc/kernels_attn_misc.h
+++ b/sgmse_amd/csrc/kernels_attn_misc.h
@@ -252,7 +252,7 @@
 }
 
 __global__ __launch_bounds__(256) void entry_kernel(const float2* x, long long xbs, const float2* y, long long ybs,
-                                                    float* xr, float* xr8, int C8, int FT, WrapCoef w, Rag rag, int F, int y_plane) {
+                                                    float* xr, int FT, WrapCoef w, Rag rag, int F, int y_plane) {
   const int i = blockIdx.x * 256 + threadIdx.x;
   const int b = blockIdx.y;
   size_t xo = (size_t)b * xbs, yo = (size_t)b * ybs, po = (size_t)b * FT;
@@ -267,11 +267,6 @@
   float* o = xr + po * 4 + i;
   const float v0 = g * xv.x, v1 = g * xv.y, v2 = g * yv.x, v3 = g * yv.y;
   o[0] = v0; o[FT] = v1; o[2 * (size_t)FT] = v2; o[3 * (size_t)FT] = v3;
-  if (xr8) {
-    float* q = xr8 + po * C8 + i;
-    q[0] = v0; q[FT] = v1; q[2 * (size_t)FT] = v2; q[3 * (size_t)FT] = v3;
-    for (int k = 4; k < C8; ++k) q[(size_t)k * FT] = 0.f;
-  }
 }
 
 struct ExitArgs {
diff --git a/sgmse_amd/csrc/kernels_conv.h b/sgmse_amd/csrc/kernels_conv.h
--- a/sgmse_amd/csrc/kernels_conv.h
+++ b/sgmse_amd/csrc/kernels_conv.h
@@ -38,10 +38,15 @@
   unsigned long long* trace;
   int xcd_map;
   const int* rag_cols; int rag_ncols;
+  int co_fold;
+  int co_pair;
+  int cin_live;
 };
 __device__ __forceinline__ int conv_xcd_tile(int t, int nt, int on) { return (on && (nt & 7) == 0) ? (t & 7) * (nt >> 3) + (t >> 3) : t; }
-__device__ __forceinline__ void conv_tile_of(const ConvArgs& p, int t, int nt, int tiles_xg, int tiles_y, int& b, int& ty, int& tx) {
+__device__ __forceinline__ int conv_tile_of(const ConvArgs& p, int t, int nt, int tiles_xg, int tiles_y, int& b, int& ty, int& tx) {
   int bid = conv_xcd_tile(t, nt, p.xcd_map);
+  int co_blk = (int)blockIdx.y;
+  if (p.co_fold > 1) { co_blk = bid % p.co_fold; bid /= p.co_fold; }
   if (p.rag_cols) {
     int lo = 0, hi = p.B;
     while (hi - lo > 1) { const int mid = (lo + hi) >> 1; if (p.rag_cols[mid] * tiles_y <= bid) lo = mid; else hi = mid; }
@@ -52,7 +57,9 @@
     ty = bid % tiles_y;
     b = bid / tiles_y;
   }
-}
+  return co_blk;
+}
+__device__ __forceinline__ int conv_src1_planes(const ConvArgs& p) { return p.cin_live ? p.cin_live : p.C1; }
 
 #ifndef SGMSE_SPLITK_FRAGMENT_MAJOR
 #define SGMSE_SPLITK_FRAGMENT_MAJOR 1
@@ -64,7 +71,7 @@
   if (tx * 32 >= Wb) return false;
   const long long d = p.rag_off[b] - (long long)b * p.H * Wb;
   p.W = Wb;
-  p.src1 += d * p.C1;
+  p.src1 += d * conv_src1_planes(p);
   if (p.src2) p.src2 += d * p.C2;
   p.out += d * p.Cout;
   if (p.res) p.res += d * p.Cout;
@@ -473,11 +480,10 @@
   const int tiles_xg = (p.W + 31) >> 5;
   const int tiles_y = (p.H + ROWS - 1) / ROWS;
   int b, ty, tx;
-  conv_tile_of(p, (int)blockIdx.x, (int)gridDim.x, tiles_xg, tiles_y, b, ty, tx);
+  const int co_blk = conv_tile_of(p, (int)blockIdx.x, (int)gridDim.x, tiles_xg, tiles_y, b, ty, tx);
   if (p.rag_w) { if (!conv_ragged_adjust(p, b, tx)) return; }
   const int tiles_x = (p.W + 31) >> 5;
   const int x0 = tx * 32, y0 = ty * ROWS;
-  const int co_blk = blockIdx.y;
   const int H = p.H, W = p.W;
   const bool xform = p.in_scale != nullptr;
 
@@ -511,6 +517,9 @@
 
   const float* wbase = p.w + (size_t)co_blk * Cin * TAPS * CO_T;
   const size_t HW = (size_t)H * W;
+  const int live = (KS == 3 && p.cin_live) ? p.cin_live : KC;
+  const int c1p = KS == 3 ? conv_src1_planes(p) : p.C1;
+  auto dead_planes = [&](int c) -> int { return c >= live ? c - (live - 1) : 0; };
 
   if constexpr (!VEC) {
 #pragma unroll
@@ -522,9 +531,9 @@
       const int r = rem / RS;
       const int x = rem - r * RS;
       const int gy = y0 - HALO + r, gx = x0 - HALO + x;
-      const bool ok = gy >= 0 && gy < H && gx >= 0 && gx < W;
+      const bool ok = gy >= 0 && gy < H && gx >= 0 && gx < W && c < live;
       okmask |= (ok ? 1u : 0u) << i;
-      goff[i] = ok ? gy * W + gx : 0;
+      goff[i] = (ok ? gy * W + gx : 0) - dead_planes(c) * (int)HW;
     }
   } else {
 #pragma unroll
@@ -535,9 +544,9 @@
       const int rem = it - c * (TROWS * 8);
       const int r = rem >> 3, q = rem & 7;
       const int gy = y0 - HALO + r, gx = x0 + 4 * q;
-      const bool ok = gy >= 0 && gy < H && gx < W;
+      const bool ok = gy >= 0 && gy < H && gx < W && c < live;
       okmask |= (ok ? 1u : 0u) << i;
-      goff_v[i] = ok ? gy * W + gx : 0;
+      goff_v[i] = (ok ? gy * W + gx : 0) - dead_planes(c) * (int)HW;
       loff_v[i] = c * PLANE + r * RS + (HALO ? 4 : 0) + 4 * q;
     }
     if (HALO) {
@@ -546,15 +555,15 @@
       const int rem = it - c * (TROWS * 2);
       const int r = rem >> 1, side = rem & 1;
       const int gy = y0 - HALO + r, gx = side ? x0 + 32 : x0 - 1;
-      const bool ok = gy >= 0 && gy < H && gx >= 0 && gx < W;
+      const bool ok = gy >= 0 && gy < H && gx >= 0 && gx < W && c < live;
       okmask |= (ok ? 1u : 0u) << 31;
-      goff[0] = ok ? gy * W + gx : 0;
+      goff[0] = (ok ? gy * W + gx : 0) - dead_planes(c) * (int)HW;
       loff_h = c * PLANE + r * RS + (side ? 36 : 3);
     }
   }
 
   auto plane_of = [&](int cg) -> const float* {
-    return (cg < p.C1) ? p.src1 + (size_t)(b * p.C1 + cg) * HW : p.src2 + (size_t)(b * p.C2 + (cg - p.C1)) * HW;
+    return (cg < p.C1) ? p.src1 + (size_t)(b * c1p + cg) * HW : p.src2 + (size_t)(b * p.C2 + (cg - p.C1)) * HW;
   };
 
   auto load_stage = [&](int c0) {
@@ -743,11 +752,10 @@
   const int tiles_xg = (p.W + 31) >> 5;
   const int tiles_y = (p.H + ROWS - 1) / ROWS;
   int b, ty, tx;
-  conv_tile_of(p, (int)blockIdx.x, (int)gridDim.x, tiles_xg, tiles_y, b, ty, tx);
+  const int co_blk = conv_tile_of(p, (int)blockIdx.x, (int)gridDim.x, tiles_xg, tiles_y, b, ty, tx);
   if (p.rag_w) { if (!conv_ragged_adjust(p, b, tx)) return; }
   const int H = p.H, W = p.W;
   const int tiles_x = (W + 31) >> 5;
-  const int co_blk = blockIdx.y;
   const int wave = tid >> 6, lane = tid & 63, l31 = lane & 31, kh = lane >> 5;
   const int wc = wave % WC, wp = wave / WC;
   f32x16 acc[FC][FP];
diff --git a/sgmse_amd/csrc/kernels_conv1x1.h b/sgmse_amd/csrc/kernels_conv1x1.h
--- a/sgmse_amd/csrc/kernels_conv1x1.h
+++ b/sgmse_amd/csrc/kernels_conv1x1.h
@@ -18,11 +18,10 @@
   const int tiles_xg = (p.W + 31) >> 5;
   const int tiles_y = (p.H + T::ROWS - 1) / T::ROWS;
   int b, ty, tx;
-  conv_tile_of(p, (int)blockIdx.x, (int)gridDim.x, tiles_xg, tiles_y, b, ty, tx);
+  const int co_blk = conv_tile_of(p, (int)blockIdx.x, (int)gridDim.x, tiles_xg, tiles_y, b, ty, tx);
   if (p.rag_w) { if (!conv_ragged_adjust(p, b, tx)) return; }
   const int H = p.H, W = p.W;
   const int tiles_x = (W + 31) >> 5;
-  const int co_blk = blockIdx.y;
   const bool xform = p.in_scale != nullptr;
   for (int c = tid; c < Cin; c += 256) {
     s_sc[c] = xform ? p.in_scale[b * Cin + c] : 1.f;
diff --git a/sgmse_amd/csrc/kernels_conv_pipe.h b/sgmse_amd/csrc/kernels_conv_pipe.h
--- a/sgmse_amd/csrc/kernels_conv_pipe.h
+++ b/sgmse_amd/csrc/kernels_conv_pipe.h
@@ -29,11 +29,10 @@
   const int tiles_xg = (p.W + 31) >> 5;
   const int tiles_y = (p.H + ROWS - 1) / ROWS;
   int b, ty, tx;
-  conv_tile_of(p, (int)blockIdx.x, (int)gridDim.x, tiles_xg, tiles_y, b, ty, tx);
+  const int co_blk = conv_tile_of(p, (int)blockIdx.x, (int)gridDim.x, tiles_xg, tiles_y, b, ty, tx);
   if (p.rag_w) { if (!conv_ragged_adjust(p, b, tx)) return; }
   const int tiles_x = (p.W + 31) >> 5;
   const int x0 = tx * 32, y0 = ty * ROWS;
-  const int co_blk = blockIdx.y;
   const int H = p.H, W = p.W;
   const bool xform = p.in_scale != nullptr;
   for (int c = tid; c < Cin; c += 256) {
@@ -89,10 +88,11 @@
   }
   const float* wbase = p.w + (size_t)co_blk * Cin * TAPS * CO_T;
   const size_t HW = (size_t)H * W;
-  const int nst = Cin / KH;
+  const int nst = (p.cin_live ? p.cin_live : Cin) / KH;
+  const int c1p = conv_src1_planes(p);
 
   auto plane_of = [&](int cg) -> const float* {
-    return (cg < p.C1) ? p.src1 + (size_t)(b * p.C1 + cg) * HW : p.src2 + (size_t)(b * p.C2 + (cg - p.C1)) * HW;
+    return (cg < p.C1) ? p.src1 + (size_t)(b * c1p + cg) * HW : p.src2 + (size_t)(b * p.C2 + (cg - p.C1)) * HW;
   };
   auto xf1 = [&](float v, float sc, float sh, bool ok) -> float {
     v = v * sc + sh;
diff --git a/sgmse_amd/csrc/kernels_conv_split.h b/sgmse_amd/csrc/kernels_conv_split.h
--- a/sgmse_amd/csrc/kernels_conv_split.h
+++ b/sgmse_amd/csrc/kernels_conv_split.h
@@ -152,11 +152,10 @@
   const int tiles_xg = (p.W + 31) >> 5;
   const int tiles_y = (p.H + ROWS - 1) / ROWS;
   int b, ty, tx;
-  conv_tile_of(p, (int)blockIdx.x, (int)gridDim.x, tiles_xg, tiles_y, b, ty, tx);
+  const int co_blk = conv_tile_of(p, (int)blockIdx.x, (int)gridDim.x, tiles_xg, tiles_y, b, ty, tx);
   if (p.rag_w) { if (!conv_ragged_adjust(p, b, tx)) return; }
   const int H = p.H, W = p.W;
   const int tiles_x = (W + 31) >> 5;
-  const int co_blk = blockIdx.y;
   const int x0 = tx * 32, y0 = ty * ROWS;
   float xb_raw = 0.f;
   if constexpr (S::SCALED) { if (p.xbound) xb_raw = p.xbound[b * kAmaxSpread + (tid & (kAmaxSpread - 1))]; }
@@ -578,11 +577,10 @@
   const int tiles_xg = (p.W + 31) >> 5;
   const int tiles_y = (p.H + 7) >> 3;
   int b, ty, tx;
-  conv_tile_of(p, (int)blockIdx.x, (int)gridDim.x, tiles_xg, tiles_y, b, ty, tx);
+  const int co_blk = conv_tile_of(p, (int)blockIdx.x, (int)gridDim.x, tiles_xg, tiles_y, b, ty, tx);
   if (p.rag_w) { if (!conv_ragged_adjust(p, b, tx)) return; }
   const int H = p.H, W = p.W;
   const int tiles_x = (W + 31) >> 5;
-  const int co_blk = blockIdx.y;
   const int x0 = tx * 32, y0 = ty * 8;
   float actf = 0.f;
   if constexpr (XF) {
diff --git a/sgmse_amd/csrc/kernels_conv_wino.h b/sgmse_amd/csrc/kernels_conv_wino.h
--- a/sgmse_amd/csrc/kernels_conv_wino.h
+++ b/sgmse_amd/csrc/kernels_conv_wino.h
@@ -107,11 +107,10 @@
   const int tiles_xg = (p.W + 31) >> 5;
   const int tiles_y = (p.H + ROWS - 1) / ROWS;
   int b, ty, tx;
-  conv_tile_of(p, (int)blockIdx.x, (int)gridDim.x, tiles_xg, tiles_y, b, ty, tx);
+  const int co_blk = conv_tile_of(p, (int)blockIdx.x, (int)gridDim.x, tiles_xg, tiles_y, b, ty, tx);
   if (p.rag_w) { if (!conv_ragged_adjust(p, b, tx)) return; }
   const int H = p.H, W = p.W;
   const int tiles_x = (W + 31) >> 5;
-  const int co_blk = blockIdx.y;
   const int x0 = tx * 32, y0 = ty * ROWS;
   const unsigned HW = (unsigned)H * (unsigned)W;
 
diff --git a/sgmse_amd/csrc/kernels_conv_wino2d.h b/sgmse_amd/csrc/kernels_conv_wino2d.h
--- a/sgmse_amd/csrc/kernels_conv_wino2d.h
+++ b/sgmse_amd/csrc/kernels_conv_wino2d.h
@@ -98,11 +98,10 @@
   const int tiles_xg = (p.W + 31) >> 5;
   const int tiles_y = (p.H + ROWS - 1) / ROWS;
   int b, ty, tx;
-  conv_tile_of(p, (int)blockIdx.x, (int)gridDim.x, tiles_xg, tiles_y, b, ty, tx);
+  const int co_blk = conv_tile_of(p, (int)blockIdx.x, (int)gridDim.x, tiles_xg, tiles_y, b, ty, tx);
   if (p.rag_w) { if (!conv_ragged_adjust(p, b, tx)) return; }
   const int H = p.H, W = p.W;
   const int tiles_x = (W + 31) >> 5;
-  const int co_blk = blockIdx.y;
   const int x0 = tx * 32, y0 = ty * ROWS;
   const unsigned HW = (unsigned)H * (unsigned)W;
 
diff --git a/sgmse_amd/csrc/kernels_conv_wino43.h b/sgmse_amd/csrc/kernels_conv_wino43.h
--- a/sgmse_amd/csrc/kernels_conv_wino43.h
+++ b/sgmse_amd/csrc/kernels_conv_wino43.h
@@ -106,11 +106,10 @@
   const int tiles_xg = (p.W + 31) >> 5;
   const int tiles_y = (p.H + ROWS - 1) / ROWS;
   int b, ty, tx;
-  conv_tile_of(p, (int)blockIdx.x, (int)gridDim.x, tiles_xg, tiles_y, b, ty, tx);
+  const int co_blk = conv_tile_of(p, (int)blockIdx.x, (int)gridDim.x, tiles_xg, tiles_y, b, ty, tx);
   if (p.rag_w) { if (!conv_ragged_adjust(p, b, tx)) return; }
   const int H = p.H, W = p.W;
   const int tiles_x = (W + 31) >> 5;
-  const int co_blk = blockIdx.y;
   const int x0 = tx * 32, y0 = ty * ROWS;
   const unsigned HW = (unsigned)H * (unsigned)W;
 
diff --git a/sgmse_amd/ops.py b/sgmse_amd/ops.py
--- a/sgmse_amd/ops.py
+++ b/sgmse_amd/ops.py
@@ -40,7 +40,7 @@
     ctx.use_current_stream()
     ctx.check(ctx.lib.sgmse_op_conv2d(ctx.h, x.data_ptr(), weight.data_ptr(), _lib.ptr(_f32(bias, "bias", dev)),
                                       _lib.ptr(_f32(residual, "residual", dev)), out.data_ptr(), B, Cin, Cout, H, W, kh,
-                                      float(out_scale), {None: int(force_direct), 'bf16x3': 2, 'fp16x2': 3, 'wino': 4, 'wino4': 5, 'thin': 6, 'wino2d': 7, 'wino43': 8, 'wino43_4': 9}[force_split], _lib.ptr(_f32(in_scale, "in_scale", dev)),
+                                      float(out_scale), {None: int(force_direct), 'bf16x3': 2, 'fp16x2': 3, 'wino': 4, 'wino4': 5, 'thin': 6, 'wino2d': 7, 'wino43': 8, 'wino43_4': 9, 'entry': 10, 'entry_small': 11}[force_split], _lib.ptr(_f32(in_scale, "in_scale", dev)),
                                       _lib.ptr(_f32(in_shift, "in_shift", dev)), int(in_act),
                                       _lib.ptr(_f32(x2, "x2", dev)), C2))
     return out
```

Result: no change. 6.222 utterances/s, median of 6 (+0.9%).
